# BachiLi/redner

Hardware: AMD Instinct MI355X
Metric: Msamples/s fwd+bwd (higher is better)
Workload: dtype f64; 1 GPU; bunny_box 1024x1024, max_bounces 4, Sobol, 256 spp fwd+bwd per step (vertex gradients, primary+secondary edge sampling), sharded by sample index over 1 GPU(s): 256 spp per GPU; spp=256, spp_per_gpu=256, max_bounces=4, parallelism=sample-sharded x1, world_size=1, pool_cap_mb=32768, samples_per_launch=8, sample_workers=2, schedule=library default: two sample workers, batches as large as the buffer cache holds

## Files before the change

### include/redner_amd.h

```cpp
#ifndef REDNER_AMD_H
#define REDNER_AMD_H

#include <stddef.h>
#include <stdint.h>

#ifdef __cplusplus
extern "C" {
#endif

#define RDR_MAX_MIP_LEVELS 8

enum rdr_camera_type { RDR_CAMERA_PERSPECTIVE = 0, RDR_CAMERA_ORTHOGRAPHIC = 1, RDR_CAMERA_FISHEYE = 2,
                       RDR_CAMERA_PANORAMA = 3 };
enum rdr_sampler_type { RDR_SAMPLER_INDEPENDENT = 0, RDR_SAMPLER_SOBOL = 1 };
enum rdr_channel {
    RDR_CH_RADIANCE = 0, RDR_CH_ALPHA, RDR_CH_DEPTH, RDR_CH_POSITION, RDR_CH_GEOMETRY_NORMAL,
    RDR_CH_SHADING_NORMAL, RDR_CH_UV, RDR_CH_BARYCENTRIC_COORDINATES, RDR_CH_DIFFUSE_REFLECTANCE,
    RDR_CH_SPECULAR_REFLECTANCE, RDR_CH_ROUGHNESS, RDR_CH_GENERIC_TEXTURE, RDR_CH_VERTEX_COLOR,
    RDR_CH_SHAPE_ID, RDR_CH_TRIANGLE_ID, RDR_CH_MATERIAL_ID
};

typedef struct rdr_camera_desc {
    int width, height;
    const float *position, *look, *up;
// ... 38 lines not shown
} rdr_material_desc;

typedef struct rdr_dtexture_desc {
    float *texels[RDR_MAX_MIP_LEVELS];
    int num_levels;
    float *uv_scale;
} rdr_dtexture_desc;
typedef struct rdr_dmaterial_desc {
    rdr_dtexture_desc diffuse_reflectance, specular_reflectance, roughness, generic_texture, normal_map;
} rdr_dmaterial_desc;

typedef struct rdr_area_light_desc {
    int shape_id;
    float intensity[3];
    int two_sided, directly_visible;
} rdr_area_light_desc;
typedef struct rdr_darea_light_desc { float *intensity; } rdr_darea_light_desc;

typedef struct rdr_envmap_desc {
    rdr_texture_desc values;
    const float *env_to_world, *world_to_env;
    const float *sample_cdf_ys, *sample_cdf_xs;
    float pdf_norm;
    int directly_visible;
} rdr_envmap_desc;
typedef struct rdr_denvmap_desc { rdr_dtexture_desc values; float *world_to_env; } rdr_denvmap_desc;

typedef struct rdr_tuning rdr_tuning;
typedef struct rdr_render_options {
    uint64_t seed;
    int num_samples, max_bounces;
    const int *channels; int num_channels;
    int sampler_type;
    int sample_pixel_center;
    int sample_offset, total_samples;
    const rdr_tuning *tuning;
} rdr_render_options;

enum rdr_tune_flags {
    RDR_TUNE_NO_OVERLAP       = 1 << 0,
    RDR_TUNE_FORCE_GENERAL    = 1 << 1,
    RDR_TUNE_PICKN_WALK       = 1 << 2,
    RDR_TUNE_PICKH_FUSED      = 1 << 3,
    RDR_TUNE_PICKH_LAZY       = 1 << 4,
    RDR_TUNE_NO_HOIST         = 1 << 5,
    RDR_TUNE_REFILL_OFF       = 1 << 6,
    RDR_TUNE_REFILL_ALL       = 1 << 7,
    RDR_TUNE_TRACE_BINARY     = 1 << 8,
    RDR_TUNE_TRACE_NO_LDS_TOP = 1 << 9,
    RDR_TUNE_NO_FUSED_BOUNCE  = 1 << 10,
    RDR_TUNE_PICKH_ONE_LAUNCH = 1 << 11,
    RDR_TUNE_NO_NEE_COMPACT   = 1 << 12,
    RDR_TUNE_LARGE_FORMS      = 1 << 13,
    RDR_TUNE_TRACE_EVERY_CONTINUATION = 1 << 14
};
struct rdr_tuning {
    unsigned flags;
    int batch_samples;
    int64_t batch_lanes;
    int workers;
    int refill_rays_per_lane, refill_idle_lanes, refill_steps;
    int wide_max_rays;
    int gather_budget;
    int gather_heavy_cap_plus1, gather_work_cap_plus1;
    int mem_available_mb;
    int refill_order;
    int pickh_slots_per_lane, pickh_idle_lanes, pickh_steps;
    int stale_event_cap_plus1;
};

void rdr_set_stream(void *hip_stream);
void rdr_set_pool_cap_mb(int64_t megabytes);
int64_t rdr_get_pool_cap_mb(void);
enum rdr_build_flags {
    RDR_BUILD_NO_REFIT        = 1 << 0,
    RDR_BUILD_NO_EDGE_CACHE   = 1 << 1,
    RDR_BUILD_SYNC_EDGES      = 1 << 2,
    RDR_BUILD_EDGE_HOST_BUILD = 1 << 3
};
void rdr_set_build_flags(unsigned flags);

typedef struct rdr_dscene_desc {
    rdr_dcamera_desc camera;
    const rdr_dshape_desc *shapes; int num_shapes;
    const rdr_dmaterial_desc *materials; int num_materials;
    const rdr_darea_light_desc *area_lights; int num_area_lights;
    const rdr_denvmap_desc *envmap;
} rdr_dscene_desc;

typedef struct rdr_scene rdr_scene;

rdr_scene *rdr_scene_create(const rdr_camera_desc *camera,
                            const rdr_shape_desc *shapes, int num_shapes,
                            const rdr_material_desc *materials, int num_materials,
                            const rdr_area_light_desc *area_lights, int num_area_lights,
                            const rdr_envmap_desc *envmap,
                            int use_gpu, int gpu_index,
                            int use_primary_edge_sampling, int use_secondary_edge_sampling);
void rdr_scene_destroy(rdr_scene *scene);
int rdr_scene_max_generic_texture_dimension(const rdr_scene *scene);

int rdr_render(const rdr_scene *scene, const rdr_render_options *options,
               float *rendered_image, const float *d_rendered_image,
               const rdr_dscene_desc *d_scene,
               float *screen_gradient_image, float *debug_image);

int rdr_compute_num_channels(const int *channels, int num_channels, int max_generic_texture_dimension);
// ... 109 lines not shown
```

### redner_amd/_capi.py

```python
import ctypes as C
import os

MAX_MIP = 8
_HERE = os.path.dirname(os.path.abspath(__file__))
DEFAULT_LIBRARY = os.path.join(_HERE, 'lib', 'libredner_amd.so')
EXACT_LIBRARY = os.path.join(_HERE, 'lib', 'libredner_amd_exact.so')

c_float_p = C.POINTER(C.c_float)
c_int_p = C.POINTER(C.c_int32)


class CameraDesc(C.Structure):
    _fields_ = [('width', C.c_int), ('height', C.c_int),
                ('position', C.c_void_p), ('look', C.c_void_p), ('up', C.c_void_p),
                ('cam_to_world', C.c_void_p), ('world_to_cam', C.c_void_p),
                ('intrinsic_mat_inv', C.c_void_p), ('intrinsic_mat', C.c_void_p),
                ('distortion_params', C.c_void_p),
                ('clip_near', C.c_float), ('camera_type', C.c_int),
                ('viewport_beg', C.c_int * 2), ('viewport_end', C.c_int * 2)]


class DCameraDesc(C.Structure):
    _fields_ = [(n, C.c_void_p) for n in ('position', 'look', 'up', 'cam_to_world', 'world_to_cam',
                                          'intrinsic_mat_inv', 'intrinsic_mat', 'distortion_params')]
# ... 11 lines not shown
    _fields_ = [(n, C.c_void_p) for n in ('vertices', 'uvs', 'normals', 'colors')]


class TextureDesc(C.Structure):
    _fields_ = [('texels', C.c_void_p * MAX_MIP), ('width', C.c_int * MAX_MIP), ('height', C.c_int * MAX_MIP),
                ('channels', C.c_int), ('num_levels', C.c_int), ('uv_scale', C.c_void_p)]


class MaterialDesc(C.Structure):
    _fields_ = [('diffuse_reflectance', TextureDesc), ('specular_reflectance', TextureDesc),
                ('roughness', TextureDesc), ('generic_texture', TextureDesc), ('normal_map', TextureDesc),
                ('compute_specular_lighting', C.c_int), ('two_sided', C.c_int), ('use_vertex_color', C.c_int)]


class DTextureDesc(C.Structure):
    _fields_ = [('texels', C.c_void_p * MAX_MIP), ('num_levels', C.c_int), ('uv_scale', C.c_void_p)]


class DMaterialDesc(C.Structure):
    _fields_ = [(n, DTextureDesc) for n in ('diffuse_reflectance', 'specular_reflectance', 'roughness',
                                            'generic_texture', 'normal_map')]


class AreaLightDesc(C.Structure):
    _fields_ = [('shape_id', C.c_int), ('intensity', C.c_float * 3), ('two_sided', C.c_int),
                ('directly_visible', C.c_int)]


class DAreaLightDesc(C.Structure):
    _fields_ = [('intensity', C.c_void_p)]


class EnvmapDesc(C.Structure):
    _fields_ = [('values', TextureDesc), ('env_to_world', C.c_void_p), ('world_to_env', C.c_void_p),
                ('sample_cdf_ys', C.c_void_p), ('sample_cdf_xs', C.c_void_p),
                ('pdf_norm', C.c_float), ('directly_visible', C.c_int)]


class DEnvmapDesc(C.Structure):
    _fields_ = [('values', DTextureDesc), ('world_to_env', C.c_void_p)]


class Tuning(C.Structure):
    _fields_ = [('flags', C.c_uint), ('batch_samples', C.c_int), ('batch_lanes', C.c_int64), ('workers', C.c_int),
                ('refill_rays_per_lane', C.c_int), ('refill_idle_lanes', C.c_int), ('refill_steps', C.c_int),
                ('wide_max_rays', C.c_int), ('gather_budget', C.c_int),
                ('gather_heavy_cap_plus1', C.c_int), ('gather_work_cap_plus1', C.c_int), ('mem_available_mb', C.c_int),
                ('refill_order', C.c_int), ('pickh_slots_per_lane', C.c_int), ('pickh_idle_lanes', C.c_int), ('pickh_steps', C.c_int),
                ('stale_event_cap_plus1', C.c_int)]


TUNE_NO_OVERLAP, TUNE_FORCE_GENERAL, TUNE_PICKN_WALK, TUNE_PICKH_FUSED, TUNE_PICKH_LAZY, TUNE_NO_HOIST, TUNE_REFILL_OFF, \
    TUNE_REFILL_ALL, TUNE_TRACE_BINARY, TUNE_TRACE_NO_LDS_TOP, TUNE_NO_FUSED_BOUNCE, TUNE_PICKH_ONE_LAUNCH, TUNE_NO_NEE_COMPACT, \
    TUNE_LARGE_FORMS, TUNE_TRACE_EVERY_CONTINUATION = [1 << k for k in range(15)]
BUILD_NO_REFIT, BUILD_NO_EDGE_CACHE, BUILD_SYNC_EDGES, BUILD_EDGE_HOST_BUILD = [1 << k for k in range(4)]


class RenderOptionsDesc(C.Structure):
    _fields_ = [('seed', C.c_uint64), ('num_samples', C.c_int), ('max_bounces', C.c_int),
                ('channels', C.POINTER(C.c_int)), ('num_channels', C.c_int),
                ('sampler_type', C.c_int), ('sample_pixel_center', C.c_int),
                ('sample_offset', C.c_int), ('total_samples', C.c_int),
                ('tuning', C.POINTER(Tuning))]


class DSceneDesc(C.Structure):
    _fields_ = [('camera', DCameraDesc),
                ('shapes', C.POINTER(DShapeDesc)), ('num_shapes', C.c_int),
                ('materials', C.POINTER(DMaterialDesc)), ('num_materials', C.c_int),
                ('area_lights', C.POINTER(DAreaLightDesc)), ('num_area_lights', C.c_int),
                ('envmap', C.POINTER(DEnvmapDesc))]


class TraceStats(C.Structure):
    _fields_ = [('closest_ms', C.c_double), ('any_ms', C.c_double),
                ('closest_launches', C.c_uint64), ('any_launches', C.c_uint64),
                ('closest_rays', C.c_uint64), ('any_rays', C.c_uint64),
                ('closest_nodes', C.c_uint64), ('closest_tris', C.c_uint64),
                ('any_nodes', C.c_uint64), ('any_tris', C.c_uint64),
                ('closest_wide_nodes', C.c_uint64), ('any_wide_nodes', C.c_uint64),
                ('closest_union_ms', C.c_double), ('any_union_ms', C.c_double)]


class DebugCounters(C.Structure):
    _fields_ = [('device_mallocs', C.c_uint64), ('host_count_reads', C.c_uint64),
                ('last_batch_samples', C.c_uint64), ('last_workers', C.c_uint64)]


class DeferredDesc(C.Structure):
    _fields_ = [('num_images', C.c_int), ('height', C.c_int), ('width', C.c_int),
                ('aa_samples', C.c_int), ('alpha', C.c_int), ('num_lights', C.c_int),
                ('light_type', c_int_p), ('image_light_range', c_int_p), ('gpu_index', C.c_int),
                ('occluders', C.POINTER(C.c_void_p)), ('visibility', C.c_void_p),
                ('ao_occluders', C.POINTER(C.c_void_p)), ('ao_words', C.c_void_p),
                ('ao_rays', C.c_int), ('ao_radius', C.c_float)]


DL_AMBIENT, DL_POINT, DL_DIRECTIONAL, DL_SPOT, DL_SH_R, DL_SH_G, DL_SH_B = range(7)

_p, _i, _i64 = C.c_void_p, C.c_int, C.c_int64
HEADERS = {
    'redner_amd.h': {
        'rdr_last_error': (C.c_char_p, []),
        'rdr_scene_create': (_p, [C.POINTER(CameraDesc), C.POINTER(ShapeDesc), _i, C.POINTER(MaterialDesc), _i,
                                  C.POINTER(AreaLightDesc), _i, C.POINTER(EnvmapDesc), _i, _i, _i, _i]),
        'rdr_scene_destroy': (None, [_p]),
        'rdr_scene_max_generic_texture_dimension': (_i, [_p]),
# ... 124 lines not shown
```

### redner_amd/csrc/bsdf.h

```cpp
#pragma once
#include "surface.h"

namespace rdr {

RDR_FN int imod(int a, int b) { int r = a % b; return r < 0 ? r + b : r; }

struct Bilerp { int i00, i10, i01, i11; double u, v; };
RDR_FN Bilerp bilerp_setup(const TexD &tex, int li, V2 uv) {
    Bilerp b;
    int W = tex.width[li], H = tex.height[li];
    double x = uv.x * W - 0.5f, y = uv.y * H - 0.5f;
    int xf = (int)floor(x), yf = (int)floor(y);
    b.u = x - xf; b.v = y - yf;
    int x0 = imod(xf, W), y0 = imod(yf, H), x1 = imod(xf + 1, W), y1 = imod(yf + 1, H);
    b.i00 = y0 * W + x0; b.i10 = y0 * W + x1; b.i01 = y1 * W + x0; b.i11 = y1 * W + x1;
    return b;
}
RDR_FN double bilerp_eval(const float *texels, int ch, int c, const Bilerp &b) {
    double f00 = texels[ch * b.i00 + c], f10 = texels[ch * b.i10 + c];
    double f01 = texels[ch * b.i01 + c], f11 = texels[ch * b.i11 + c];
    return f00 * (1.f - b.u) * (1.f - b.v) + f01 * (1.f - b.u) * b.v +
           f10 * b.u * (1.f - b.v) + f11 * b.u * b.v;
}

template <class F> RDR_FN void trilinear_each(const TexD &tex, V2 uv, double level, const F &f) {
    int ch = tex.channels;
    if (level <= 0 || level >= tex.num_levels - 1) {
        int li = level <= 0 ? 0 : tex.num_levels - 1;
        Bilerp b = bilerp_setup(tex, li, uv);
        for (int c = 0; c < ch; ++c) f(c, bilerp_eval(tex.texels[li], ch, c, b));
    } else {
        int li = (int)floor(level);
        double ld = level - li;
        Bilerp b0 = bilerp_setup(tex, li, uv), b1 = bilerp_setup(tex, li + 1, uv);
        for (int c = 0; c < ch; ++c) {
            double a0 = bilerp_eval(tex.texels[li], ch, c, b0);
            double a1 = bilerp_eval(tex.texels[li + 1], ch, c, b1);
            f(c, a0 * (1 - ld) + a1 * ld);
        }
    }
}
RDR_FN void trilinear(const TexD &tex, V2 uv, double level, double *out) {
    trilinear_each(tex, uv, level, [out](int c, double x) { out[c] = x; });
}

RDR_FN double tex_level(const TexD &tex, V2 du, V2 dv) {
    double fp = dmax(len(du) * tex.width[0], len(dv) * tex.height[0]);
    return log(dmax(fp, double(1e-8f))) / log(2.0);
}

template <class F> RDR_FN void tex_fetch_each(const TexD &tex, V2 uv_, V2 du_, V2 dv_, const F &f) {
    if (tex.width[0] <= 0 && tex.height[0] <= 0) {
        for (int c = 0; c < tex.channels; ++c) f(c, (double)tex.texels[0][c]);
        return;
// ... 338 lines not shown
}

RDR_FN V3 cos_hemisphere(V2 s) {
    double phi = 2.f * float(M_PI) * s.x;
    double tmp = sqrt(dmax(1.f - s.y, 0.0));
    return V3{cos(phi) * tmp, sin(phi) * tmp, sqrt(s.y)};
}

RDR_FN V3 bsdf_sample_dir(const MaterialD &m, const Surf &sp, V3 wi, V2 s_uv, double s_w, double min_rough,
                          const RayDiff &wi_rd, RayDiff &wo_rd, double &next_min_rough, bool diffs = true) {
    next_min_rough = min_rough;
    ShadeCtx c = shade_ctx(m, sp);
    double gwi = dot(c.gn, wi);
    if (!m.two_sided && gwi < 0) return v3(0);
    LobePmf p = lobe_pmf(m, sp);
    if (s_w <= p.diffuse) {
        next_min_rough = 1.0;
        V3 ld = cos_hemisphere(s_uv);
        if (diffs) {
            wo_rd.org_dx = wi_rd.org_dx; wo_rd.org_dy = wi_rd.org_dy;
            wo_rd.dir_dx = V3{0.03f, 0.03f, 0.03f};
            wo_rd.dir_dy = V3{0.03f, 0.03f, 0.03f};
        }
        V3 d = to_world(c.fr, ld);
        if (dot(c.gn, d) * gwi < 0) d = to_world(c.fr, -ld);
        return d;
    }
    double rough = dmax(dmax(tex1(m.roughness, sp), min_rough), 1e-6);
    next_min_rough = dmax(rough, min_rough);
    double e = roughness_to_phong(rough);
    double phi = 2.f * double(M_PI) * s_uv.y;
    double sphi = sin(phi), cphi = cos(phi);
    double ct = pow(s_uv.x, 1.0 / (e + 2.0));
    double st = sqrt(dmax(1.f - ct * ct, 0.0));
    V3 hl = V3{st * cphi, st * sphi, ct};
    V3 h = to_world(c.fr, hl);
    V3 d = 2.f * dot(wi, h) * h - wi;
    if (dot(c.gn, d) * gwi < 0) {
        hl = -hl;
        h = to_world(c.fr, hl);
        d = 2.f * dot(wi, h) * h - wi;
    }
    if (!diffs) return d;
    V3 dmdx = sp.dn_dx * hl.z, dmdy = sp.dn_dy * hl.z;
    V3 wi_dx = -wi_rd.dir_dx, wi_dy = -wi_rd.dir_dy;
    double wdm_dx = sum(wi_dx * h) + sum(wi * dmdx);
    double wdm_dy = sum(wi_dy * h) + sum(wi * dmdy);
    wo_rd.org_dx = wi_rd.org_dx; wo_rd.org_dy = wi_rd.org_dy;
    wo_rd.dir_dx = 2 * (dot(wi, h) * dmdx + wdm_dx * h) - wi_dx;
    wo_rd.dir_dy = 2 * (dot(wi, h) * dmdy + wdm_dy * h) - wi_dy;
    return d;
}

}
```

### redner_amd/csrc/hip/exec.h

```cpp
#pragma once
#include <hip/hip_runtime.h>
#include "../per_device.h"
#include <stdint.h>
#include <stdio.h>
#include <atomic>
#include <condition_variable>
#include <cstdlib>
#include <exception>
#include <functional>
#include <mutex>
#include <stdexcept>
#include <string>
#include <thread>

#define RDR_FN __host__ __device__ inline
#define RDR_INLINE_CALL [[clang::always_inline]]
#define RDR_DEV_FN __device__ inline
#define RDR_STACK_DECL(T, name, N) __shared__ T name##_lds[(N) * 256]; T *name = name##_lds + threadIdx.x
#define RDR_STACK_AT(name, k) name[(k) * 256]
#define RDR_WALK_STACK_MEMBER(T, name, N)
#define RDR_WALK_STACK(st, T, name, N, TAG) (rdr::lds_column<T, N, TAG>())
#define RDR_WALK_AT(stk, k) stk[(k) * 256]

namespace rdr {
// ... 231 lines not shown
                    if (low && hipDeviceGetStreamPriorityRange(&least, &greatest) == hipSuccess && least != greatest)
                        check(hipStreamCreateWithPriority(&s, hipStreamNonBlocking, least), "hipStreamCreateWithPriority");
                    else check(hipStreamCreateWithFlags(&s, hipStreamNonBlocking), "hipStreamCreate");
                }
                ctx().stream = s;
                job();
                check(hipStreamSynchronize(s), "second stream sync");
            } catch (...) { failure = std::current_exception(); }
            { std::unique_lock<std::mutex> lk(m_); failure_ = failure; state_ = 0; }
            cv_.notify_all();
        }
    }
    std::mutex m_; std::condition_variable cv_;
    std::function<void()> job_; int device_ = 0; int state_ = 0;
    std::exception_ptr failure_;
};

struct Fence {
    hipEvent_t e = nullptr;
    Fence() { check(hipEventCreateWithFlags(&e, hipEventDisableTiming), "hipEventCreate"); }
    ~Fence() { if (e) (void)hipEventDestroy(e); }
    Fence(const Fence &) = delete;
    void after(hipStream_t producer) { check(hipEventRecord(e, producer), "hipEventRecord"); }
    void gate(hipStream_t consumer) { check(hipStreamWaitEvent(consumer, e, 0), "hipStreamWaitEvent"); }
};

inline int choose_replicas(size_t replica_bytes, size_t budget) {
    int r = 256;
    while (r > 1 && replica_bytes * (size_t)r > budget) r >>= 1;
    return r;
}
inline size_t replica_budget(size_t job_samples) {
    static const size_t mb = [] { const char *e = std::getenv("RDR_REPLICA_MB"); return e ? (size_t)std::atoi(e) : (size_t)0; }();
    if (mb) return mb << 20;
    const size_t lo = (size_t)256 << 20, hi = (size_t)1 << 30, want = job_samples * 64;
    return want < lo ? lo : (want > hi ? hi : want);
}
inline void set_replicas(const rdr::ReplicaLayout &layout) {
    check(hipMemcpyToSymbolAsync(HIP_SYMBOL(rdr::g_rep), &layout, sizeof(layout), 0, hipMemcpyHostToDevice, ctx().stream), "set_replicas");
    static const int texel_rounds = [] { const char *e = std::getenv("RDR_TEXEL_ROUNDS"); return e ? std::atoi(e) : 0; }();
    if (texel_rounds > 0) check(hipMemcpyToSymbolAsync(HIP_SYMBOL(rdr::g_texel_rounds), &texel_rounds, sizeof(int), 0, hipMemcpyHostToDevice, ctx().stream), "set_replicas");
    check(hipStreamSynchronize(ctx().stream), "set_replicas sync");
}

struct Count {
    const int *dev; int upper;
    Count(int n) : dev(nullptr), upper(n) {}
    Count(const int *d, int u) : dev(d), upper(u) {}
};

template <class F, class = void> struct MinBlocks { static constexpr int value = 1; };
template <class F> struct MinBlocks<F, decltype((void)F::kMinBlocksPerCU)> { static constexpr int value = F::kMinBlocksPerCU; };

template <class F>
__global__ void __launch_bounds__(256, MinBlocks<F>::value) stage_kernel(F f, int n, const int *count) {
    int i = blockIdx.x * 256 + threadIdx.x;
    if (count) { const int c = *count; n = c < n ? c : n; }
    if (i < n) { RDR_INLINE_CALL f(i); }
}

constexpr int kRefillIdle = 16;
constexpr int kWalkSteps = 16;
template <class W, class = void> struct WalkGate { __device__ static bool closed(const W &) { return false; } };
template <class W> struct WalkGate<W, decltype((void)&W::gate_closed)> { __device__ static bool closed(const W &w) { return w.gate_closed(); } };
template <class W>
__global__ void __launch_bounds__(256) persistent_kernel(W w, int n, const int *count, int *next_item) {
    if (WalkGate<W>::closed(w)) return;
    if (count) { const int c = *count; n = c < n ? c : n; }
    typename W::State st;
    bool busy = false;
    const int lane = threadIdx.x & 63;
    for (;;) {
        const unsigned long long idle = __ballot(!busy);
        const int nidle = __popcll(idle);
        if (nidle >= kRefillIdle) {
            const int leader = __ffsll((long long)idle) - 1;
            int base = 0;
            if (lane == leader) base = atomicAdd(next_item, nidle);
            base = __shfl(base, leader);
            if (!busy) {
                const int item = base + __popcll(idle & ((1ull << lane) - 1ull));
                if (item < n) {
                    if (w.begin(item, st)) busy = true;
                    else w.finish(st);
                }
            }
            if (__ballot(busy) == 0ull && base + nidle >= n) break;
        }
#pragma unroll 1
        for (int it = 0; it < kWalkSteps; ++it) {
            if (busy && w.step(st)) { w.finish(st); busy = false; }
        }
    }
}
#ifndef RDR_CHUNKED_MIN_BLOCKS
#define RDR_CHUNKED_MIN_BLOCKS 1
#endif
template <class W>
__global__ void __launch_bounds__(256, RDR_CHUNKED_MIN_BLOCKS) chunked_kernel(W w, int n, const int *count, int items_per_lane, int idle_min, int steps, int *next_chunk) {
    if (count) { const int c = *count; n = c < n ? c : n; }
    const int chunk = 64 * items_per_lane;
    const int lane = threadIdx.x & 63;
    int next = 0, end = 0;
    bool more = true;
    typename W::State st;
    bool busy = false;
    for (;;) {
        const unsigned long long idle = __ballot(!busy);
        const int nidle = __popcll(idle);
        if (nidle >= idle_min || nidle == 64) {
// ... 221 lines not shown
```

### redner_amd/csrc/render.cpp

```cpp
#include "render.h"
#include "tuning.h"
#include <atomic>
#include <exception>
#include <cstdio>
#include <cstdlib>
#include "stages_fwd.h"
#include "stages_bwd.h"
#include "stages_edge.h"
#include "grad_store.h"
#include <algorithm>
#include <memory>
#include <stdexcept>
#include <type_traits>
#include <vector>

namespace rdr {

namespace {

inline bool overlap_on() { return !tuning().has(RDR_TUNE_NO_OVERLAP); }


VSlice make_slice(Arena &a, int n, bool with_occl, bool with_rdiff = true) {
    VSlice v;
// ... 11 lines not shown
struct Queues {
    rt::RayRec *nee, *bsdf;
    rt::HitRec *h_nee, *h_bsdf;
    int *pos[2];
};

struct BounceChain {
    bool fused = false;
    bool have_rays = false;
    const int *qpos = nullptr;
    exec::Count queue_n{0};
    int flip = 0;
};

struct ChannelLayout { int nd, radiance_dim; ChannelsD ch; };
ChannelLayout layout_of(const rdr_render_options &o, int max_generic) {
    ChannelLayout l;
    l.nd = 0; l.radiance_dim = -1;
    if (o.num_channels > kMaxChannels) throw std::runtime_error("render: too many channels");
    l.ch.n = o.num_channels; l.ch.max_generic = max_generic; l.ch.radiance_off = -1;
    l.ch.id = nullptr;
    l.ch.radiance_only = o.num_channels == 1 && o.channels[0] == RDR_CH_RADIANCE;
    int d = 0;
    for (int i = 0; i < o.num_channels; ++i) {
        if (o.channels[i] == RDR_CH_RADIANCE) {
            if (l.radiance_dim != -1) throw std::runtime_error("Duplicated radiance channel");
            l.radiance_dim = i;
            l.ch.radiance_off = d;
        }
        int one = o.channels[i];
        int w = compute_num_channels(&one, 1, max_generic);
        if (w < 0) throw std::runtime_error("render: unknown channel id");
        d += w;
    }
    l.nd = d;
    l.ch.nd = d; l.ch.radiance_dim = l.radiance_dim;
    return l;
}

void debug_dump(const char *tag, int sample, int depth, const void *dev_ptr, size_t bytes) {
    static const char *dir = std::getenv("RDR_DEBUG_DUMP");
    if (!dir || !dev_ptr) return;
    std::vector<char> host(bytes);
    exec::download(host.data(), dev_ptr, bytes);
    char path[1024];
    std::snprintf(path, sizeof(path), "%s/%s_s%d_d%d.bin", dir, tag, sample, depth);
    if (FILE *f = std::fopen(path, "wb")) { std::fwrite(host.data(), 1, bytes, f); std::fclose(f); }
}

uint64_t pcg_stream_seed(const rdr_render_options &o) {
    return (uint64_t)o.seed + (uint64_t)o.sample_offset * 0x9E3779B97F4A7C15ULL;
}

bool scene_is_lean(const Scene &scene, const ChannelsD &ch) {
    const CameraD &c = scene.d.cam;
    return scene.d.envmap == nullptr && c.kind == kCamPerspective && !c.distortion.defined && ch.radiance_only &&
           !scene.has_mipmaps && !scene.has_textures && !scene.has_vertex_colors;
}

constexpr int kGeneral = 0, kLean = 1, kMid = 2;
int scene_kind(const Scene &scene, const ChannelsD &ch) {
    if (tuning().has(RDR_TUNE_FORCE_GENERAL)) return kGeneral;
    if (scene_is_lean(scene, ch)) return kLean;
    const CameraD &c = scene.d.cam;
    if (scene.d.envmap == nullptr && c.kind == kCamPerspective && !c.distortion.defined && ch.radiance_only) return kMid;
    return kGeneral;
}
template <class F, class Go> void with_kind(int kind, const F &f, Go &&go) {
    if (kind == kLean) go(LeanStage<F>{f});
    else if (kind == kMid) go(MidStage<F>{f});
    else go(f);
}
template <class W, class Go> void with_walk_kind(int kind, const W &w, Go &&go) {
    if (kind == kLean) go(LeanWalk<W>{w});
    else if (kind == kMid) go(MidWalk<W>{w});
    else go(w);
}
template <class F> void launch_v(int kind, exec::Count n, const F &f) {
    with_kind(kind, f, [&](const auto &k) { exec::launch(n, k); });
}

inline int side_index(int k, int lanes) { return lanes >= (1 << 19) ? k + 2 : k; }
struct Fork {
    exec::Fence from, done;
    bool marked = false, pending = false;
    void mark() { from.after(exec::ctx().stream); marked = true; }
    void join() { if (pending) done.gate(exec::ctx().stream); pending = false; }
    template <class Work> void run(hipStream_t side, Work &&work) {
        if (!marked) mark();
        marked = false;
        from.gate(side);
        exec::StreamScope on(side);
        work();
        done.after(side);
        pending = true;
    }
};
template <class Work> void beside(Fork &fork, bool aside, int k, int lanes, Work &&work) {
    if (aside) fork.run(exec::side_stream(side_index(k, lanes)), work);
    else work();
}

inline bool fuse_bounces(bool pcg, int kind, int chain_lanes) {
    return !pcg && kind == kLean && chain_lanes <= (1 << 19) && !tuning().has(RDR_TUNE_NO_FUSED_BOUNCE);
}
constexpr int kEmitterTestMax = 8;
struct Bounce {
    SamplerD rng{}; int dim = 0, rng_shift = 0;
    const int *active = nullptr; exec::Count num_active{0};
    int *next_active = nullptr;
    const VSlice *v = nullptr, *vn = nullptr, *vnn = nullptr;
    const Queues *q = nullptr;
    Sink sink{};
    int *dyn = nullptr; int dyn_inc = 0;
    bool shadow_rays_coherent = false, last_bounce = false, next_is_last = false;
    BounceChain *chain = nullptr;
    Fork *shadow_fork = nullptr;
};
exec::Count run_bounce(const Scene &scene, const SceneD &sd, const Bounce &b) {
    const VSlice &v = *b.v, &vn = *b.vn;
    const Queues &q = *b.q;
    BounceChain *chain = b.chain;
    const int lean = scene_kind(scene, b.sink.ch);
    const bool fused = chain && chain->fused;
    const bool drawn = fused && chain->have_rays;
    const exec::Count queue_n = drawn ? chain->queue_n : b.num_active;
    const int *qpos = drawn ? chain->qpos : nullptr;
    const bool emitter_test = lean == kLean && scene.emitter_triangles > 0 && scene.emitter_triangles <= kEmitterTestMax &&
                              !tuning().has(RDR_TUNE_TRACE_EVERY_CONTINUATION);
    if (!drawn) {
        BounceSample bs{sd, b.rng, b.dim, b.rng_shift, b.active, v, vn, q.nee, q.bsdf};
        bs.last_bounce_emitters = b.last_bounce && emitter_test;
        launch_v(lean, b.num_active, bs);
    }
    beside(*b.shadow_fork, overlap_on(), 1, b.num_active.upper, [&] {
        exec::trace(scene.bvh, q.nee, q.h_nee, queue_n, true, b.shadow_rays_coherent);
    });
    exec::trace(scene.bvh, q.bsdf, q.h_bsdf, queue_n, false);
    b.shadow_fork->join();
    const BounceContrib contrib{sd, b.rng, b.dim, b.rng_shift, b.active, v, vn, q.h_nee, q.h_bsdf, b.sink};
    if (!fused) {
        launch_v(lean, b.num_active, contrib);
        return exec::compact_dev(b.active, b.num_active, b.next_active, KeepHit{vn.shape}, nullptr, b.dyn, b.dyn_inc);
    }
    if (b.vnn) {
        BounceSample next{sd, b.rng, b.dim + 7, b.rng_shift, b.active, vn, *b.vnn, q.nee, q.bsdf};
        next.last_bounce_emitters = b.next_is_last && emitter_test;
        launch_v(lean, b.num_active, BounceContribSample{contrib, next, qpos});
    } else if (qpos) {
        launch_v(lean, b.num_active, BounceContribSample{contrib, BounceSample{sd, b.rng, b.dim + 7, b.rng_shift, b.active, vn, vn, nullptr, nullptr}, qpos, 1});
    } else {
        launch_v(lean, b.num_active, contrib);
    }
    int *pos_out = q.pos[chain->flip];
    chain->flip ^= 1;
    const exec::Count next = exec::compact_dev(b.active, b.num_active, b.next_active, KeepHit{vn.shape}, nullptr, b.dyn, b.dyn_inc, pos_out);
    chain->have_rays = b.vnn != nullptr;
    chain->qpos = pos_out;
    chain->queue_n = b.num_active;
    return next;
}

struct BatchView { int S = 1, P0 = 0, rows = 0; bool on = false; };

struct Worker {
    Arena arena;
    std::vector<VSlice> vs;
    int *active = nullptr;
    Queues q;
    std::vector<exec::Count> num_active;
    int *main_dyn = nullptr;
    int *seg = nullptr;
    float *stage = nullptr;
    Fork shadow_fork;
};

struct Backward {
    const Scene &scene; const rdr_render_options &opt;
    Worker &w;
    int stride, B;
    const float *d_image; float *screen_grad; double weight; int nd, radiance_dim;
// ... 10 lines not shown
    int *edge_dyn = nullptr;
    int *hoist_dyn = nullptr;
    double *multipliers = nullptr;

    VSlice ea, eb;
    int chain_n = 0;
    double *erd_chain = nullptr;
    int *deferred = nullptr, *deferred_seg = nullptr, *deferred_count = nullptr, *prim_dyn = nullptr;
    int *elist[3] = {nullptr, nullptr, nullptr};
    HEntry *h_leaves = nullptr, *h_spill = nullptr;
    int *nee_act = nullptr;
    HDescent *h_descent = nullptr;
    GatherShared gshared{nullptr, nullptr, nullptr, nullptr, 0, 0};
    GatherCand *gather_cands = nullptr;
    int *nee_slots = nullptr;
    double *edge_contrib = nullptr, *edge_tmin = nullptr, *hit_pos = nullptr;
    unsigned char *hp_written = nullptr; int *hp_violations = nullptr;
    HitEvent *hp_events = nullptr; int *hp_event_count = nullptr; int hp_event_cap = 0;
    double *hp_carry = nullptr;
    unsigned char *replay_live = nullptr;
    PrimaryEdgeRec *prim_recs = nullptr;
    SecondaryEdgeRec *sec_recs = nullptr;
    SecPick *sec_picks = nullptr;
    unsigned char *sec_mode = nullptr;
    Sink esink{}, psink{};

    Fork walk_fork;
    Fork pickh_fork;
    Fork adjoint_fork;
    const bool overlap = overlap_on();
    const bool has_lights = sd.num_lights > 0;
    const int dim0 = opt.sample_pixel_center ? 0 : 2;
    bool edges_on() const { return prim_recs != nullptr; }
    bool secondary_on() const { return edges_on() && scene.use_secondary_edges; }

    int sample_id = 0;
    int lanes = 0;
    int cur_S = 1;
    SamplerD rng{}, rng_edge{};
    int edim = 0;
    bool hoisted = false;
    SecEdgeArgs early_sa{};

    Backward(const Scene &scene_, const rdr_render_options &opt_, GradStore &grads_, Worker &w_, int P, int B_,
             const float *d_image_, float *screen_grad_, double weight_, int nd_, int radiance_dim_, const ChannelsD &ch_,
             const BatchView &batch_)
        : scene(scene_), opt(opt_), w(w_), stride(P), B(B_), d_image(d_image_), screen_grad(screen_grad_), weight(weight_),
          nd(nd_), radiance_dim(radiance_dim_), batch(batch_), sd(scene_.d), grads(grads_), ch(ch_) {
        if (batch.on) sd.cam.batch_rows = batch.rows;
        lean = scene_kind(scene, ch);
        adj.n = P; adj.plain = 0;
        adj.thr = arena.get<double>((size_t)3 * P);
        adj.ray_dir = arena.get<double>((size_t)3 * P);
        adj_point_doubles = lean == kLean ? kAdjPointDoublesLean : kAdjPointDoubles;
        adj.point = arena.get<double>((size_t)adj_point_doubles * P);
        adj.carries = scene.d.envmap == nullptr ? arena.get<unsigned char>((size_t)P) : nullptr;
        nee_act = arena.get<int>((size_t)P);
        const bool use_edges = scene.edges && scene.edges->d.num_edges > 0 &&
                              (scene.use_primary_edges || scene.use_secondary_edges);
        if (use_edges) {
            edge_dyn = arena.get<int>(kMaxBatch);
            hoist_dyn = arena.get<int>(kMaxBatch);
            const int L = 2 * P;
            ea = make_slice(arena, L, false, lean != kLean);
            eb = make_slice(arena, L, false, lean != kLean);
            if (scene.has_mipmaps) {
                ea.erd = eb.erd = arena.get<double>((size_t)12 * L);
                exec::zero(ea.erd, sizeof(double) * 12 * L);
                if (batch.on) {
                    chain_n = 2 * batch.P0;
                    ea.erd_touched = eb.erd_touched = arena.get<unsigned char>(L);
                    erd_chain = arena.get<double>((size_t)12 * chain_n);
                    exec::zero(erd_chain, sizeof(double) * 12 * chain_n);
                    deferred = arena.get<int>(L);
                    deferred_seg = arena.get<int>(kMaxBatch + 1);
                    deferred_count = arena.get<int>(kMaxBatch);
                    prim_dyn = arena.get<int>(kMaxBatch);
                }
            }
            for (int k = 0; k < 3; ++k) elist[k] = arena.get<int>(L);
            nee_slots = arena.get<int>(P);
            gather_cands = arena.get<GatherCand>((size_t)kGatherCands * P);
            gshared.book = arena.get<GatherBook>(1);
            gshared.heavy_cap = (int)std::min<long long>(std::max<long long>((long long)P / 256, kGatherHeavyCap), kGatherHeavyMax);
            gshared.work_cap = (int)std::min<long long>(std::max<long long>((long long)P / 32, kGatherWorkCap), kGatherWorkMax);
            gshared.heavy_slot = arena.get<int>(gshared.heavy_cap);
            gshared.work = arena.get<GatherWork>(gshared.work_cap);
            gshared.cands_big = arena.get<GatherCand>((size_t)kGatherCandsBig * gshared.heavy_cap);
            if (tuning().gather_heavy_cap >= 0) gshared.heavy_cap = std::min(tuning().gather_heavy_cap, gshared.heavy_cap);
            if (tuning().gather_work_cap >= 0) gshared.work_cap = std::min(tuning().gather_work_cap, gshared.work_cap);
            h_leaves = arena.get<HEntry>((size_t)kHSamples * P);
            h_spill = arena.get<HEntry>((size_t)(kHSamples - kHStackLds) * P);
            h_descent = arena.get<HDescent>((size_t)P);
            edge_contrib = arena.get<double>(L);
            edge_tmin = arena.get<double>(L);
            hit_pos = arena.get<double>((size_t)3 * L);
            exec::zero(hit_pos, sizeof(double) * 3 * L);
            if (batch.on && scene.d.envmap != nullptr) {
                hp_written = arena.get<unsigned char>(L);
                hp_violations = arena.get<int>(1);
                exec::zero(hp_violations, sizeof(int));
                hp_event_cap = L;
                hp_events = arena.get<HitEvent>((size_t)hp_event_cap);
                if (tuning().stale_event_cap >= 0) hp_event_cap = std::min(tuning().stale_event_cap, hp_event_cap);
                hp_event_count = arena.get<int>(1);
                exec::zero(hp_event_count, sizeof(int));
                hp_carry = arena.get<double>((size_t)3 * 2 * batch.P0);
                exec::zero(hp_carry, sizeof(double) * 3 * 2 * batch.P0);
                replay_live = arena.get<unsigned char>(P);
            }
            prim_recs = arena.get<PrimaryEdgeRec>(P);
            sec_recs = arena.get<SecondaryEdgeRec>(P);
            sec_picks = arena.get<SecPick>(P);
            sec_mode = arena.get<unsigned char>(P);
            if (!ch.radiance_only) multipliers = arena.get<double>((size_t)L * nd);
            if (opt.sampler_type == RDR_SAMPLER_INDEPENDENT) {
                pcg_edge = arena.get<uint64_t>(P);
                exec::launch(P, PcgInit{pcg_edge, pcg_stream_seed(opt) + 131071U});
// ... 300 lines not shown
        for (int d = B - 1; d >= 0; --d) {
            if (w.num_active[d].upper <= 0) continue;
            const AdjBounceArgs ba{sd, grads.g, rng, dim0 + 7 * d, active_of(d), w.vs[d], w.vs[d + 1], d_image, nd, radiance_dim, 0.0, adj};
            launch_v(lean, w.num_active[d], AdjBounceScatterLive{AdjBounceScatter{ba}, replay_live});
            exec::launch(n_events, InjectHitEvents{sd, grads.g, hp_events, d, hit_pos, ea.n, hp_written, hp_carry, 2 * batch.P0, adj, replay_live});
        }
        launch_v(lean, lanes, AdjPrimaryLive{AdjPrimary{sd, grads.g, rng, opt.sample_pixel_center, w.vs[0], d_image, nd, radiance_dim, 0.0,
                                                        adj, screen_grad, ch}, replay_live});
        exec::launch(2 * batch.P0, HitPosCarryAdvance{hp_carry, 2 * batch.P0, cur_S, hit_pos, ea.n, hp_written});
        exec::zero(hp_event_count, sizeof(int));
    }

    void run_sample(int sample_id_, const SamplerD &main_rng, int n_lanes, int S_now) {
        begin_sample(sample_id_, main_rng, n_lanes, S_now);
        hoist_first_vertex_picks();
        for (int d = B - 1; d >= 0 && has_lights; --d) sweep_depth(d);
        camera_vertex_adjoint();
        if (edges_on() && scene.use_primary_edges) primary_edge_pass();
        adjoint_fork.join();
        if (hp_events) replay_stale_hits();
    }
};

struct RestartUnbatched {};
std::atomic<uint64_t> g_unbatchable{0};
uint64_t scene_shape_key(const Scene &scene) {
    uint64_t h = 1469598103934665603ULL;
    auto mix = [&](uint64_t v) { h = (h ^ v) * 1099511628211ULL; };
    mix(scene.shapes.size());
    for (const ShapeD &sh : scene.shapes) { mix((uint64_t)sh.num_vertices); mix((uint64_t)sh.num_triangles); }
    mix(scene.materials.size()); mix(scene.lights.size());
    mix((uint64_t)scene.h_envmap.values.width[0]); mix((uint64_t)scene.h_envmap.values.height[0]);
    return h | 1;
}
BatchView choose_batch(const rdr_render_options &opt, const Tuning &tune, int P, int rows, int lean, int nd,
                       bool samples_independent, bool forward_batches, bool gradient) {
    const int B = opt.max_bounces;
    BatchView batch;
    batch.P0 = P; batch.rows = rows;
    if (!samples_independent && !forward_batches) return batch;
    const int batch_cap = std::min(kMaxBatch, tune.batch_samples);
    const long long total = (long long)opt.num_samples * P;
    int want = opt.num_samples;
    if (total > (1 << 17) && samples_independent) want = (opt.num_samples + 1) / 2;
    long long lane_cap = tune.batch_lanes;
    if (lane_cap == 0) {
        lane_cap = 1LL << 24;
        if (total > (1LL << 22) && exec::memory_held_by_others() > 0.10) lane_cap = 1LL << 22;
    }
    batch.S = std::max(1, std::min(std::min(batch_cap, want), (int)std::max(1LL, lane_cap / P)));
    auto bytes_needed = [&](int S_try) {
        const double lanes = (double)S_try * P;
        const int wk = !samples_independent ? 1 : (tune.workers > 0 ? tune.workers : 2);
        double per_lane = (lean == kLean ? 260.0 * (B + 1) + 660.0 : 400.0 * (B + 1) + 1200.0) * wk;
        if (forward_batches) per_lane += 4.0 * nd * (B + 1);
        if (gradient) per_lane += 4.0 * nd;
        return per_lane * lanes;
    };
    if (tune.batch_lanes == 0 && tune.mem_available_mb < 0) {
        const double cap = (double)exec::pool_cap_bytes();
        while (batch.S > 1 && bytes_needed(batch.S) > cap) --batch.S;
    }
    if (tune.mem_available_mb >= 0 || bytes_needed(batch.S) > 1073741824.0) {
        const double room = 0.8 * (tune.mem_available_mb >= 0 ? tune.mem_available_mb * 1048576.0 : (double)exec::memory_available());
        while (batch.S > 1 && bytes_needed(batch.S) > room) batch.S = (batch.S + 1) / 2;
    }
    batch.on = batch.S > 1;
    return batch;
}

const int *upload_assign_flags(Arena &arena, const rdr_render_options &opt, int max_generic, int nd) {
    std::vector<int> flags((size_t)nd, 0);
    int at = 0;
    bool any_id = false;
    for (int k = 0; k < opt.num_channels; ++k) {
        int one = opt.channels[k];
        const int w = compute_num_channels(&one, 1, max_generic);
        if (one >= RDR_CH_SHAPE_ID) { for (int j = 0; j < w; ++j) flags[at + j] = 1; any_id = true; }
        at += w;
    }
    if (!any_id) return nullptr;
    int *d_flags = arena.get<int>(flags.size());
    exec::upload(d_flags, flags.data(), sizeof(int) * flags.size());
    return d_flags;
}

void render_once(const Scene &scene, const rdr_render_options &opt, float *image, const float *d_image,
                 const rdr_dscene_desc *d_scene, float *screen_gradient_image, const Tuning &tune, bool envmap_batches) {
    if (opt.sampler_type != RDR_SAMPLER_SOBOL && opt.sampler_type != RDR_SAMPLER_INDEPENDENT)
        throw std::runtime_error("render: unknown sampler type");
    if (d_image && !d_scene) throw std::runtime_error("render: d_rendered_image given without d_scene");
    const CameraD &cam = scene.d.cam;
    const int P = (cam.vp_x1 - cam.vp_x0) * (cam.vp_y1 - cam.vp_y0);
    if (P <= 0) return;
    const int B = opt.max_bounces;
    if (B < 0) throw std::runtime_error("render: max_bounces must be >= 0");
    ChannelLayout lay = layout_of(opt, scene.max_generic_texture_dimension);
    if (lay.radiance_dim < 0 && B > 0)
        throw std::runtime_error("render: max_bounces > 0 needs the radiance channel (the reference writes path "
                                 "contributions at the radiance offset, src/path_contribution.cpp:127-129)");
    const int total_spp = opt.total_samples > 0 ? opt.total_samples : opt.num_samples;
    const double weight = 1.0 / total_spp;
    const bool has_lights = scene.d.num_lights > 0;
    if (2 + 7 * B > kSamplerDims) throw std::runtime_error("render: max_bounces exceeds the Sobol' table");

    PhaseTimer timer(d_image ? "render (backward)" : "render (forward)");
    Arena arena;
    {
        int *ids = arena.get<int>(kMaxChannels);
        exec::upload(ids, opt.channels, sizeof(int) * opt.num_channels);
        lay.ch.id = ids;
    }
    std::unique_ptr<GradStore> grads;
    if (d_image) grads.reset(new GradStore(scene, *d_scene, (size_t)P * (size_t)opt.num_samples));

    uint64_t *pcg_main = nullptr;
    if (opt.sampler_type == RDR_SAMPLER_INDEPENDENT) {
        pcg_main = arena.get<uint64_t>(P);
        exec::launch(P, PcgInit{pcg_main, pcg_stream_seed(opt)});
    }
    const int lean = scene_kind(scene, lay.ch);

    const bool sobol_plain = screen_gradient_image == nullptr && opt.sampler_type == RDR_SAMPLER_SOBOL && !timer.on;
    const bool no_edge_passes = !scene.use_primary_edges && !scene.use_secondary_edges;
    const bool chain = (scene.has_mipmaps || scene.d.envmap != nullptr) && !no_edge_passes;
    const bool batchable = sobol_plain && (lean == kLean || no_edge_passes || scene.d.envmap == nullptr || envmap_batches);
    const bool samples_independent = batchable && d_image != nullptr && image == nullptr;
    const bool forward_batches = sobol_plain && d_image == nullptr && image != nullptr;
    const BatchView batch = choose_batch(opt, tune, P, cam.vp_y1 - cam.vp_y0, lean, lay.nd, samples_independent, forward_batches, d_image != nullptr);
    const int S = batch.S;
    const int PL = S * P;
    static const bool tell = std::getenv("RDR_DEBUG_BATCH") != nullptr;
    if (tell) std::fprintf(stderr, "[render] %s: %d samples of %d lanes in batches of %d\n", d_image ? "backward" : "forward", opt.num_samples, P, S);
    const int num_batches = (opt.num_samples + S - 1) / S;
    const float *d_image_lanes = d_image;
    if (batch.on && d_image) {
        float *rep = arena.get<float>((size_t)PL * lay.nd);
        for (int k = 0; k < S; ++k)
            exec::copy_dev(rep + (size_t)k * P * lay.nd, d_image, sizeof(float) * (size_t)P * lay.nd);
        d_image_lanes = rep;
    }
    const int *assign_flags = batch.on && forward_batches && !lay.ch.radiance_only ? upload_assign_flags(arena, opt, scene.max_generic_texture_dimension, lay.nd) : nullptr;
    int workers = 1;
    if (samples_independent) workers = std::max(1, std::min(tune.workers > 0 ? tune.workers : exec::sample_workers(PL, num_batches, batch.on), num_batches));
    if (chain) workers = 1;
    if (d_image != nullptr) { last_schedule()[0].store(S); last_schedule()[1].store(workers); }

    struct SampleWorker : Worker { std::unique_ptr<Backward> bwd; };
    auto make_worker = [&](SampleWorker &w) {
        w.vs.resize(B + 1);
        for (int d = 0; d <= B; ++d) w.vs[d] = make_slice(w.arena, PL, d < B && d_image_lanes != nullptr, lean != kLean);
        w.active = w.arena.get<int>((size_t)(B + 1) * PL);
        w.q.nee = w.arena.get<rt::RayRec>((size_t)2 * PL); w.q.bsdf = w.arena.get<rt::RayRec>((size_t)2 * PL);
        w.q.h_nee = w.arena.get<rt::HitRec>((size_t)2 * PL); w.q.h_bsdf = w.arena.get<rt::HitRec>((size_t)2 * PL);
        w.q.pos[0] = w.arena.get<int>((size_t)2 * PL); w.q.pos[1] = w.arena.get<int>((size_t)2 * PL);
        w.num_active.assign(B + 2, exec::Count(0));
        if (pcg_main) w.main_dyn = w.arena.get<int>(1);
        if (batch.on) w.seg = w.arena.get<int>((size_t)(B + 1) * (kMaxBatch + 1));
        if (batch.on && forward_batches) w.stage = w.arena.get<float>((size_t)(B + 1) * PL * lay.nd);
    };
    auto run_samples = [&](SampleWorker &w, int first, int stride) {
        std::vector<VSlice> &vs = w.vs;
        int *active = w.active;
        const Queues &q = w.q;
        std::vector<exec::Count> &num_active = w.num_active;
        SceneD sd = scene.d;
        if (batch.on) sd.cam.batch_rows = batch.rows;
        for (int b = first; b < num_batches; b += stride) {
            const int s = b * S;
            const int S_now = std::min(S, opt.num_samples - s);
            const int lanes = S_now * P;
            const int sample_id = opt.sample_offset + s;
            SamplerD rng{scene.sobol_table, opt.seed, sample_id, pcg_main, 0};
            if (batch.on) { rng.batch = S_now; rng.batch_lanes = P; }
            Sink sink{image, nullptr, lay.nd, lay.radiance_dim, weight, lay.ch, nullptr};
            const size_t plane = (size_t)PL * lay.nd;
            auto sink_of = [&](int launch) { Sink k = sink; if (w.stage) k.image = w.stage + (size_t)launch * plane; return k; };
            if (w.stage) exec::zero(w.stage, sizeof(float) * plane * (B + 1));
            auto segments = [&](int d) {
                if (batch.on) exec::launch(S_now + 1, SegOffsets{active + (size_t)d * PL, num_active[d].dev, num_active[d].upper, P, S_now,
                                                                 w.seg + (size_t)d * (kMaxBatch + 1)});
            };

            launch_v(lean, lanes, GenPrimary{sd, rng, opt.sample_pixel_center, vs[0], q.bsdf});
            exec::trace(scene.bvh, q.bsdf, q.h_bsdf, lanes, false, true);
            launch_v(lean, lanes, ShadePrimary{sd, nullptr, vs[0], q.h_bsdf, sink_of(0)});
            std::fill(num_active.begin(), num_active.end(), exec::Count(0));
            num_active[0] = exec::compact_dev((const int *)nullptr, lanes, active, KeepHit{vs[0].shape});
            if (d_image) segments(0);
            if (w.main_dyn) exec::zero(w.main_dyn, sizeof(int));

            int dim = opt.sample_pixel_center ? 0 : 2;
            const int dim_first = dim;
            BounceChain chain;
            chain.fused = fuse_bounces(pcg_main != nullptr, lean, 2 * lanes);
            for (int d = 0; d < B && num_active[d].upper > 0 && has_lights; ++d) {
                Bounce bounce;
                bounce.rng = rng; bounce.dim = dim;
                bounce.active = active + (size_t)d * PL; bounce.num_active = num_active[d]; bounce.next_active = active + (size_t)(d + 1) * PL;
                bounce.v = &vs[d]; bounce.vn = &vs[d + 1]; bounce.vnn = d + 1 < B ? &vs[d + 2] : nullptr;
                bounce.q = &q; bounce.sink = sink_of(d + 1);
                bounce.dyn = w.main_dyn; bounce.dyn_inc = 7;
                bounce.shadow_rays_coherent = d == 0;
                bounce.last_bounce = d == B - 1; bounce.next_is_last = d + 2 == B;
// ... 263 lines not shown
```

### redner_amd/csrc/stages_bwd.h

```cpp
#pragma once
#include "stages_fwd.h"

namespace rdr {

constexpr int kAdjPointDoubles = 24;
constexpr int kAdjPointDoublesLean = 6;

struct AdjState {
    double *thr;
    double *ray_dir;
    double *point;
    int n;
    int plain;
    unsigned char *carries;
};

RDR_FN Surf load_adj_point(const AdjState &a, int p) {
    Surf s = surf_zero();
    s.position = ld3(a.point, a.n, p, 0);
    if (a.plain) { s.frame.n = ld3(a.point, a.n, p, 3); return s; }
    s.frame.x = ld3(a.point, a.n, p, 3); s.frame.y = ld3(a.point, a.n, p, 6); s.frame.n = ld3(a.point, a.n, p, 9);
    s.dpdu = ld3(a.point, a.n, p, 12);
    s.uv = v2(a.point[(size_t)15 * a.n + p], a.point[(size_t)16 * a.n + p]);
    s.du_dxy = v2(a.point[(size_t)17 * a.n + p], a.point[(size_t)18 * a.n + p]);
    s.dv_dxy = v2(a.point[(size_t)19 * a.n + p], a.point[(size_t)20 * a.n + p]);
    s.color = ld3(a.point, a.n, p, 21);
    return s;
}
RDR_FN void store_adj_point(const AdjState &a, int p, const Surf &s, bool with_position = true) {
    if (with_position) st3(a.point, a.n, p, 0, s.position);
    if (a.plain) { st3(a.point, a.n, p, 3, s.frame.n); return; }
    st3(a.point, a.n, p, 3, s.frame.x); st3(a.point, a.n, p, 6, s.frame.y); st3(a.point, a.n, p, 9, s.frame.n);
    st3(a.point, a.n, p, 12, s.dpdu);
    a.point[(size_t)15 * a.n + p] = s.uv.x; a.point[(size_t)16 * a.n + p] = s.uv.y;
    a.point[(size_t)17 * a.n + p] = s.du_dxy.x; a.point[(size_t)18 * a.n + p] = s.du_dxy.y;
    a.point[(size_t)19 * a.n + p] = s.dv_dxy.x; a.point[(size_t)20 * a.n + p] = s.dv_dxy.y;
    st3(a.point, a.n, p, 21, s.color);
}

RDR_FN V3 image_grad(const float *d_image, int nd, int radiance_dim, int pixel) {
    if (radiance_dim < 0) return v3(0);
    const float *g = d_image + (size_t)nd * pixel + radiance_dim;
    return V3{(double)g[0], (double)g[1], (double)g[2]};
}

struct AdjBounceArgs {
    SceneD sc; GScene g; SamplerD rng; int dim;
    const int *active; VSlice v, vn;
    const float *d_image; int nd, radiance_dim; double weight;
    AdjState adj;
};

struct AdjBounceScatter {
    AdjBounceArgs a;
    static constexpr int kMidBlocksPerCU = 2;
    static constexpr int kMinBlocksPerCU = 2;
#ifndef RDR_ADJ_SCATTER_LEAN_BLOCKS
#define RDR_ADJ_SCATTER_LEAN_BLOCKS 3
#endif
    static constexpr int kLeanBlocksPerCU = RDR_ADJ_SCATTER_LEAN_BLOCKS;
#ifndef RDR_PARK_ADJ_SCATTER
#define RDR_PARK_ADJ_SCATTER 0
#endif
    static constexpr int kParkDoubles = kSurfParkDoubles + 4;
    static_assert(kParkDoubles <= kMaxParkDoubles, "kMaxParkDoubles must cover every stage");
    RDR_FN void make_lean() { lean_scene(a.sc); lean_slice(a.v); lean_slice(a.vn); a.nd = 3; a.radiance_dim = 0; a.adj.plain = 1; }
    RDR_FN void make_mid() { mid_scene(a.sc); a.nd = 3; a.radiance_dim = 0; }
    RDR_FN void operator()(int idx) const {
        const SceneD &sc = a.sc; const GScene &g = a.g; const VSlice &v = a.v, &vn = a.vn; const AdjState &adj = a.adj;
        int p = a.active[idx];
        VertexCtx c = load_vertex(sc, v, p);
        const GMaterial &gm = g.materials[c.shape->material_id];
        V3 thr = ld3(v.thr, v.n, p, 0);
        V3 pc_bar = a.weight * image_grad(a.d_image, a.nd, a.radiance_dim, p);
        V3 thr_bar = v3(0), in_dir_bar = v3(0);
        Surf sp_bar = surf_zero();
        V3 pos = c.sp.position;
        int bshape = vn.shape[p];
        TriGrad tg = trigrad_zero();
        int tg_shape = -1, tg_tri = -1;
        V3 dir_bar = v3(0);
        bool through_hit = false;
        double d2 = 0;
        V3 wo = v3(0);
        if (bshape >= 0) {
            const ShapeD &bsh = sc.shapes[bshape];
            int btri = vn.tri[p];
            RayDiff wo_rd = load_rdiff(vn, p);
            RayDiff tmp;
            Surf bp = surf_at(bsh, btri, load_ray(vn, p), wo_rd, tmp, !sc.no_diffs);
            V3 next_thr_bar = ld3(adj.thr, adj.n, p, 0);
            V3 next_dir_bar = ld3(adj.ray_dir, adj.n, p, 0);
            V3 dir = bp.position - pos;
            d2 = len_sq(dir);
            wo = dir / sqrt(d2);
            double pdf_b = bsdf_pdf(*c.mat, c.sp, c.wi, wo, c.mrough);
            if (pdf_b > 0) {
                V3 f = bsdf_eval(*c.mat, c.sp, c.wi, wo, c.mrough);
                V3 sb = f / pdf_b;
                thr_bar += next_thr_bar * sb;
                V3 sb_bar = next_thr_bar * thr;
                V3 f_bar = sb_bar / pdf_b;
                if (bsh.light_id >= 0) {
                    const LightD &l = sc.lights[bsh.light_id];
                    if (l.two_sided || dot(-wo, bp.frame.n) > 0) {
                        double geo = fabs(dot(wo, bp.geom_normal)) / d2;
                        V3 Le = v3f(l.intensity);
                        double pdf_nee = (sc.light_pmf[bsh.light_id] * (1 / sc.light_areas[bsh.light_id])) / geo;
                        double mis = 1 / (1 + sq(pdf_nee / pdf_b));
                        V3 sc_contrib = (mis / pdf_b) * f * Le;
                        V3 scb = pc_bar * thr;
                        thr_bar += pc_bar * sc_contrib;
                        double w = mis / pdf_b;
                        f_bar += w * scb * Le;
                        if (g.light_intensity) accum3(g.light_intensity + 3 * bsh.light_id, w * scb * f);
                    }
                }
                V3 wi_bar = v3(0);
                V3 wo_bar = next_dir_bar;
                adj_bsdf_eval(*c.mat, c.sp, c.wi, wo, c.mrough, f_bar, gm, sp_bar, wi_bar, wo_bar);
                dir_bar = wo_bar / sqrt(d2);
                double sd_bar = -sum(wo_bar * dir) / d2;
                double d2_bar = 0.5f * sd_bar / sqrt(d2);
                dir_bar += adj_len_sq(dir, d2_bar);
                in_dir_bar -= wi_bar;
                through_hit = true;
            }
        } else if (sc.envmap != nullptr) {
            V3 wo_e = load_ray(vn, p).dir;
            double pdf_b = bsdf_pdf(*c.mat, c.sp, c.wi, wo_e, c.mrough);
            if (len_sq(wo_e) > 0 && pdf_b > 0) {
                V3 f = bsdf_eval(*c.mat, c.sp, c.wi, wo_e, c.mrough);
                V3 Le = envmap_eval(*sc.envmap, wo_e, raydiff_zero());
                double pdf_nee = envmap_pdf(*sc.envmap, wo_e) * sc.light_pmf[sc.num_lights - 1];
                double mis = 1 / (1 + sq(pdf_nee / pdf_b));
                V3 sc_contrib = (mis / pdf_b) * f * Le;
                V3 scb = pc_bar * thr;
                thr_bar += pc_bar * sc_contrib;
                double w = mis / pdf_b;
                V3 f_bar = w * scb * Le, Le_bar = w * scb * f;
                V3 wo_bar = v3(0), wi_bar = v3(0);
                RayDiff rd_bar = raydiff_zero();
                adj_envmap_eval(*sc.envmap, wo_e, raydiff_zero(), Le_bar, g.envmap, wo_bar, rd_bar);
                adj_bsdf_eval(*c.mat, c.sp, c.wi, wo_e, c.mrough, f_bar, gm, sp_bar, wi_bar, wo_bar);
                in_dir_bar -= wi_bar;
            }
        }
        st3(adj.thr, adj.n, p, 0, thr_bar);
        st3(adj.ray_dir, adj.n, p, 0, in_dir_bar);
        V3 pos_bar = sp_bar.position;
        Surf next_pt_bar = surf_zero();
        if (through_hit) next_pt_bar = load_adj_point(adj, p);
        store_adj_point(adj, p, sp_bar, false);
        if (through_hit) {
            const ShapeD &bsh = sc.shapes[bshape];
            const int btri = vn.tri[p];
            Surf bp_bar = next_pt_bar;
            bp_bar.position += dir_bar;
            DRay r_bar = dray_zero();
            RayDiff rd_bar = raydiff_zero();
            Ray br = make_ray(pos, wo);
#if RDR_PARK_ADJ_SCATTER
            RDR_PARK_DECL(park, kParkDoubles);
            park.put3(kSurfParkDoubles, dir_bar); park.put(kSurfParkDoubles + 3, c.mrough);
            adj_surf_at(bsh, btri, br, load_rdiff(vn, p), bp_bar, raydiff_zero(), r_bar, rd_bar, tg, !sc.no_diffs, sc.plain_materials != 0, park);
            dir_bar = park.get3<V3>(kSurfParkDoubles); c.mrough = park.get(kSurfParkDoubles + 3);
#else
            adj_surf_at(bsh, btri, br, load_rdiff(vn, p), bp_bar, raydiff_zero(), r_bar, rd_bar, tg, !sc.no_diffs, sc.plain_materials != 0);
#endif
            tg_shape = bshape; tg_tri = btri;
            if (c.mrough > 0.01f) {
                pos_bar -= dir_bar;
                pos_bar += r_bar.org;
            }
        }
        st3(adj.point, adj.n, p, 0, pos_bar);
        if (adj.carries) adj.carries[p] = 1;
        scatter_trigrad_wave(sc.shapes, g.shapes, tg_shape, tg_tri, tg, sc.plain_materials != 0);
    }
};

RDR_FN void adj_record_add(const AdjState &adj, int p, V3 thr_bar, V3 in_dir_bar, const Surf &sp_bar) {
    st3(adj.thr, adj.n, p, 0, ld3(adj.thr, adj.n, p, 0) + thr_bar);
    st3(adj.ray_dir, adj.n, p, 0, ld3(adj.ray_dir, adj.n, p, 0) + in_dir_bar);
    Surf cur = load_adj_point(adj, p);
    cur.position += sp_bar.position;
    cur.frame.n += sp_bar.frame.n;
    if (!adj.plain) {
        cur.frame.x += sp_bar.frame.x; cur.frame.y += sp_bar.frame.y;
        cur.dpdu += sp_bar.dpdu; cur.uv += sp_bar.uv; cur.du_dxy += sp_bar.du_dxy; cur.dv_dxy += sp_bar.dv_dxy;
        cur.color += sp_bar.color;
    }
    store_adj_point(adj, p, cur);
    if (adj.carries) adj.carries[p] = 1;
}

struct AdjBounceNee {
    static constexpr int kMinBlocksPerCU = 2;
    static constexpr int kMidBlocksPerCU = 2;
#ifdef RDR_ADJ_NEE_LEAN_BLOCKS
    static constexpr int kLeanBlocksPerCU = RDR_ADJ_NEE_LEAN_BLOCKS;
#endif
#ifndef RDR_PARK_ADJ_NEE
#define RDR_PARK_ADJ_NEE 1
#endif
    static constexpr int kParkDoubles = 22;
    static_assert(kParkDoubles <= kMaxParkDoubles, "kMaxParkDoubles must cover every stage");
    AdjBounceArgs a;
    RDR_FN void make_lean() { lean_scene(a.sc); lean_slice(a.v); lean_slice(a.vn); a.nd = 3; a.radiance_dim = 0; a.adj.plain = 1; }
    RDR_FN void make_mid() { mid_scene(a.sc); a.nd = 3; a.radiance_dim = 0; }
    RDR_FN void envmap_nee(int p, const LightDraw &ld) const {
        const SceneD &sc = a.sc; const GScene &g = a.g; const VSlice &v = a.v;
        V3 wo = envmap_sample(*sc.envmap, ld.uv);
        double pdf_nee = envmap_pdf(*sc.envmap, wo) * sc.light_pmf[sc.num_lights - 1];
        if (!(pdf_nee > 0)) return;
        VertexCtx c = load_vertex(sc, v, p);
        const GMaterial &gm = g.materials[c.shape->material_id];
        V3 thr = ld3(v.thr, v.n, p, 0);
        V3 pc_bar = a.weight * image_grad(a.d_image, a.nd, a.radiance_dim, p);
        V3 f = bsdf_eval(*c.mat, c.sp, c.wi, wo, c.mrough);
        V3 Le = envmap_eval(*sc.envmap, wo, raydiff_zero());
        double pdf_b = bsdf_pdf(*c.mat, c.sp, c.wi, wo, c.mrough);
        double mis = 1 / (1 + sq(pdf_b / pdf_nee));
        V3 nee = (mis / pdf_nee) * f * Le;
        V3 nee_bar = pc_bar * thr;
        V3 thr_bar = pc_bar * nee;
        double w = mis / pdf_nee;
        V3 f_bar = w * nee_bar * Le, Le_bar = w * nee_bar * f;
        V3 wo_bar = v3(0), wi_bar = v3(0);
        RayDiff rd_bar = raydiff_zero();
        adj_envmap_eval(*sc.envmap, wo, raydiff_zero(), Le_bar, g.envmap, wo_bar, rd_bar);
        Surf sp_bar = surf_zero();
        adj_bsdf_eval(*c.mat, c.sp, c.wi, wo, c.mrough, f_bar, gm, sp_bar, wi_bar, wo_bar);
        adj_record_add(a.adj, p, thr_bar, -wi_bar, sp_bar);
    }
    RDR_FN void operator()(int idx) const {
        V3 lv_bar[3] = {v3(0), v3(0), v3(0)};
        int l_shape = -1, l_tri = -1;
        RDR_INLINE_CALL light_vertex(idx, lv_bar, l_shape, l_tri);
        scatter_positions_wave(a.sc.shapes, a.g.shapes, l_shape, l_tri, lv_bar);
    }
    RDR_FN void light_vertex(int idx, V3 (&lv_bar)[3], int &l_shape, int &l_tri) const {
        const SceneD &sc = a.sc; const GScene &g = a.g; const VSlice &v = a.v; const AdjState &adj = a.adj;
        int p = a.active[idx];
        if (v.occl[p]) return;
        LightDraw ld = draw_light(a.rng, p, a.dim);
        LightPick pk = pick_light(sc, ld.light_sel, ld.tri_sel);
        if (pk.shape_id < 0) {
            if (sc.envmap != nullptr) envmap_nee(p, ld);
            return;
        }
        const ShapeD &lsh = sc.shapes[pk.shape_id];
        if (lsh.light_id < 0) return;
        VertexCtx c = load_vertex(sc, v, p);
        V3 pos = c.sp.position;
        Surf lp = sample_tri(lsh, pk.tri_id, ld.uv);
        V3 dir = lp.position - pos;
        double d2 = len_sq(dir);
        V3 wo = dir / sqrt(d2);
        const LightD &l = sc.lights[lsh.light_id];
        if (nee_is_geometrically_zero(sc, c, pk, lp)) return;
        const GMaterial &gm = g.materials[c.shape->material_id];
        V3 thr = ld3(v.thr, v.n, p, 0);
        V3 pc_bar = a.weight * image_grad(a.d_image, a.nd, a.radiance_dim, p);
        V3 thr_bar = v3(0), in_dir_bar = v3(0);
        Surf sp_bar = surf_zero();
        V3 f = bsdf_eval(*c.mat, c.sp, c.wi, wo, c.mrough);
        double cl = dot(wo, lp.geom_normal);
        double geo = fabs(cl) / d2;
        V3 Le = v3f(l.intensity);
        double pdf_nee = sc.light_pmf[lsh.light_id] * (1 / sc.light_areas[lsh.light_id]);
        double pdf_b = bsdf_pdf(*c.mat, c.sp, c.wi, wo, c.mrough) * geo;
        double mis = 1 / (1 + sq(pdf_b / pdf_nee));
        V3 nee = (mis * geo / pdf_nee) * f * Le;
        V3 nee_bar = pc_bar * thr;
        thr_bar += pc_bar * nee;
        double w = mis / pdf_nee;
        double w_bar = geo * sum(nee_bar * f * Le);
        double pdfnee_bar = -w_bar * w / pdf_nee;
        double geo_bar = w * sum(nee_bar * f * Le);
        V3 f_bar = w * nee_bar * geo * Le;
        V3 Le_bar = w * nee_bar * geo * f;
        double area_bar = -pdfnee_bar * pdf_nee / tri_area(lsh, pk.tri_id);
        adj_tri_area(lsh, pk.tri_id, area_bar, lv_bar);
        if (g.light_intensity) accum3(g.light_intensity + 3 * lsh.light_id, Le_bar);
        double cl_bar = cl > 0 ? geo_bar / d2 : -geo_bar / d2;
        double d2_bar = -geo_bar * geo / d2;
        V3 wo_bar = cl_bar * lp.geom_normal;
        Surf lp_bar = surf_zero();
        lp_bar.geom_normal = cl_bar * wo;
        V3 wi_bar = v3(0);
#if RDR_PARK_ADJ_NEE
        RDR_PARK_DECL(park, kParkDoubles);
        park.put3(0, lv_bar[0]); park.put3(3, lv_bar[1]); park.put3(6, lv_bar[2]);
        park.put3(9, thr_bar); park.put3(12, dir); park.put(15, d2); park.put(16, d2_bar);
        park.put3(17, lp_bar.geom_normal); park.put2(20, ld.uv);
#endif
        adj_bsdf_eval(*c.mat, c.sp, c.wi, wo, c.mrough, f_bar, gm, sp_bar, wi_bar, wo_bar);
#if RDR_PARK_ADJ_NEE
        lv_bar[0] = park.get3<V3>(0); lv_bar[1] = park.get3<V3>(3); lv_bar[2] = park.get3<V3>(6);
        thr_bar = park.get3<V3>(9); dir = park.get3<V3>(12); d2 = park.get(15); d2_bar = park.get(16);
        lp_bar.geom_normal = park.get3<V3>(17); ld.uv = park.get2<V2>(20);
#endif
        V3 dir_bar = wo_bar / sqrt(d2);
        double sd_bar = -sum(wo_bar * dir) / d2;
        d2_bar += (0.5f * sd_bar / sqrt(d2));
        dir_bar += adj_len_sq(dir, d2_bar);
        lp_bar.position += dir_bar;
        sp_bar.position -= dir_bar;
        in_dir_bar -= wi_bar;
        adj_sample_tri(lsh, pk.tri_id, ld.uv, lp_bar, lv_bar);
        l_shape = pk.shape_id; l_tri = pk.tri_id;
        adj_record_add(adj, p, thr_bar, in_dir_bar, sp_bar);
    }
};

struct ImageBar {
    const float *gi; double weight;
    RDR_FN double operator()(int c) const { return weight * (double)gi[c]; }
    RDR_FN const double *triple(double *o) const { o[0] = (*this)(0); o[1] = (*this)(1); o[2] = (*this)(2); return o; }
};
RDR_FN void adj_first_hit_channels(const SceneD &sc, const GScene &g, const ChannelsD &ch, const float *d_image,
                                   double weight, int p, int shape, const Surf &sp, const Ray &ray,
                                   Surf &pt_bar, V3 &org_bar) {
    const ShapeD &sh = sc.shapes[shape];
    const MaterialD &m = sc.materials[sh.material_id];
    const GMaterial &gm = g.materials[sh.material_id];
    const float *gi = d_image + (size_t)ch.nd * p;
    int d = 0;
    for (int k = 0; k < ch.n; ++k) {
        int id = ch.id[k];
        int width = channel_width(id, ch.max_generic);
        switch (id) {
            case 2: {
                double dist_bar = (double)gi[d] * weight;
                V3 diff_bar = adj_len(sp.position - ray.org, dist_bar);
                org_bar -= diff_bar; pt_bar.position += diff_bar;
            } break;
            case 3: pt_bar.position += weight * V3{(double)gi[d], (double)gi[d + 1], (double)gi[d + 2]}; break;
            case 4: pt_bar.geom_normal += weight * V3{(double)gi[d], (double)gi[d + 1], (double)gi[d + 2]}; break;
            case 5: pt_bar.frame.n += weight * V3{(double)gi[d], (double)gi[d + 1], (double)gi[d + 2]}; break;
            case 6: pt_bar.uv += weight * V2{(double)gi[d], (double)gi[d + 1]}; break;
            case 7: pt_bar.bary += weight * V2{(double)gi[d], (double)gi[d + 1]}; break;
            case 8: {
                V3 r_bar = weight * V3{(double)gi[d], (double)gi[d + 1], (double)gi[d + 2]};
                if (m.use_vertex_color) pt_bar.color += r_bar; else adj_tex3(m.diffuse, sp, r_bar, gm.diffuse, pt_bar);
            } break;
            case 9: adj_tex3(m.specular, sp, weight * V3{(double)gi[d], (double)gi[d + 1], (double)gi[d + 2]}, gm.specular, pt_bar); break;
            case 10: adj_tex1(m.roughness, sp, weight * (double)gi[d], gm.roughness, pt_bar); break;
            case 11: {
                if (m.generic.num_levels > 0)
// ... 57 lines not shown
            RayDiff mrd_bar = raydiff_zero();
            adj_envmap_eval(*sc.envmap, ray.dir, rd, e_bar, g.envmap, mr_bar.dir, mrd_bar);
            V2 ms = v2(0.5, 0.5);
            if (!sample_center) { const SamplerD::Lane ln = rng.lane(p); ms = v2(rng.draw(ln, 0), rng.draw(ln, 1)); }
            V2 mscr_bar = v2(0, 0);
            RDR_INLINE_CALL adj_primary_ray(sc.cam, pixel_to_screen(sc.cam, p, ms), mr_bar, g.cam, screen_grad != nullptr, mscr_bar);
            if (screen_grad) { screen_grad[2 * p] += (float)mscr_bar.x; screen_grad[2 * p + 1] += (float)mscr_bar.y; }
            return;
        }
        DRay r_bar = dray_zero();
        r_bar.dir = ld3(adj.ray_dir, adj.n, p, 0);
        RayDiff prd_bar = raydiff_zero();
        {
            Surf pt_bar = load_adj_point(adj, p);
            if (!ch.radiance_only) {
                RayDiff tmp;
                Surf sp = surf_at(sc.shapes[shape], v0.tri[p], ray, rd, tmp, !sc.no_diffs);
                adj_first_hit_channels(sc, g, ch, d_image, weight, p, shape, sp, ray, pt_bar, r_bar.org);
            }
            adj_surf_at(sc.shapes[shape], v0.tri[p], ray, rd, pt_bar, raydiff_zero(), r_bar, prd_bar, tg, !sc.no_diffs, sc.plain_materials != 0, park);
#pragma unroll
            for (int k = 0; k < 3; ++k) { park.put3(3 * k, tg.p[k]); park.put3(9 + 3 * k, tg.n[k]); }
            tg_shape = shape; tg_tri = v0.tri[p];
        }
        V2 s = v2(0.5, 0.5);
        if (!sample_center) { const SamplerD::Lane ln = rng.lane(p); s = v2(rng.draw(ln, 0), rng.draw(ln, 1)); }
        V2 screen = pixel_to_screen(sc.cam, p, s);
        double delta = 1e-3;
        double sx = 0.5 / sc.cam.width, sy = 0.5 / sc.cam.height;
        V2 scr_bar = v2(0, 0);
        const bool sb = screen_grad != nullptr;
        if (!sc.no_diffs) {
            DRay rx_bar{prd_bar.org_dx * sx / delta, prd_bar.dir_dx * sx / delta};
            DRay ry_bar{prd_bar.org_dy * sy / delta, prd_bar.dir_dy * sy / delta};
            r_bar.org += (prd_bar.org_dx * -sx + prd_bar.org_dy * -sy) / delta;
            r_bar.dir += (prd_bar.dir_dx * -sx + prd_bar.dir_dy * -sy) / delta;
            RDR_INLINE_CALL adj_primary_ray(sc.cam, screen + v2(delta, 0), rx_bar, g.cam, sb, scr_bar);
            RDR_INLINE_CALL adj_primary_ray(sc.cam, screen + v2(0, delta), ry_bar, g.cam, sb, scr_bar);
        }
        RDR_INLINE_CALL adj_primary_ray(sc.cam, screen, r_bar, g.cam, sb, scr_bar);
        if (screen_grad) {
            screen_grad[2 * p] += (float)scr_bar.x;
            screen_grad[2 * p + 1] += (float)scr_bar.y;
        }
    }
};

struct AdjBounceScatterLive {
    static constexpr int kMidBlocksPerCU = AdjBounceScatter::kMidBlocksPerCU, kMinBlocksPerCU = AdjBounceScatter::kMinBlocksPerCU,
                         kLeanBlocksPerCU = AdjBounceScatter::kLeanBlocksPerCU;
    AdjBounceScatter f; const unsigned char *live;
    RDR_FN void make_lean() { f.make_lean(); }
    RDR_FN void make_mid() { f.make_mid(); }
    RDR_FN void operator()(int idx) const { if (!live[f.a.active[idx]]) return; RDR_INLINE_CALL f(idx); }
};
struct AdjPrimaryLive {
    static constexpr int kMidBlocksPerCU = AdjPrimary::kMidBlocksPerCU, kMinBlocksPerCU = AdjPrimary::kMinBlocksPerCU;
    AdjPrimary f; const unsigned char *live;
    RDR_FN void make_lean() { f.make_lean(); }
    RDR_FN void make_mid() { f.make_mid(); }
    RDR_FN void operator()(int p) const { if (!live[p]) return; RDR_INLINE_CALL f(p); }
};

struct KeepNeeLive {
    const unsigned char *occl;
    RDR_FN bool operator()(int p) const { return occl[p] == 0; }
};

struct KeepLitContinuation {
    const int *next_shape; const ShapeD *shapes; bool envmap;
    RDR_FN bool operator()(int p) const { const int s = next_shape[p]; return s >= 0 ? shapes[s].light_id >= 0 : envmap; }
};
struct KeepCarryingContinuation {
    const unsigned char *carries; const int *next_shape; const ShapeD *shapes;
    RDR_FN bool operator()(int p) const { return carries[p] != 0 || shapes[next_shape[p]].light_id >= 0; }
};

struct FlushSegment { size_t begin, count; float *out; };
struct FlushGrad {
    const double *block; size_t stride; int replicas;
    const FlushSegment *segments; int num_segments;
    RDR_FN void operator()(int i) const {
        int lo = 0, hi = num_segments;
        while (hi - lo > 1) {
            int mid = (lo + hi) >> 1;
            if (segments[mid].begin <= (size_t)i) lo = mid; else hi = mid;
        }
        const FlushSegment sg = segments[lo];
        if ((size_t)i < sg.begin || (size_t)i >= sg.begin + sg.count) return;
        double s = 0;
        for (int r = 0; r < replicas; ++r) s += block[(size_t)r * stride + i];
        sg.out[(size_t)i - sg.begin] += (float)s;
    }
};

}
```

### redner_amd/csrc/stages_edge.h

```cpp
#pragma once
#include "edges.h"
#include "stages_bwd.h"

namespace rdr {

RDR_FN M3 m3_from_frame(const Frame &f) {
    M3 r;
    r.m[0][0] = f.x.x; r.m[0][1] = f.x.y; r.m[0][2] = f.x.z;
    r.m[1][0] = f.y.x; r.m[1][1] = f.y.y; r.m[1][2] = f.y.z;
    r.m[2][0] = f.n.x; r.m[2][1] = f.n.y; r.m[2][2] = f.n.z;
    return r;
}
RDR_FN M3 m3_inverse(const M3 &a) {
    const double (*m)[3] = a.m;
    double det = m[0][0] * (m[1][1] * m[2][2] - m[2][1] * m[1][2]) - m[0][1] * (m[1][0] * m[2][2] - m[1][2] * m[2][0]) +
                 m[0][2] * (m[1][0] * m[2][1] - m[1][1] * m[2][0]);
    double id = 1 / det;
    M3 r;
    r.m[0][0] = (m[1][1] * m[2][2] - m[2][1] * m[1][2]) * id;
    r.m[0][1] = (m[0][2] * m[2][1] - m[0][1] * m[2][2]) * id;
    r.m[0][2] = (m[0][1] * m[1][2] - m[0][2] * m[1][1]) * id;
    r.m[1][0] = (m[1][2] * m[2][0] - m[1][0] * m[2][2]) * id;
    r.m[1][1] = (m[0][0] * m[2][2] - m[0][2] * m[2][0]) * id;
    r.m[1][2] = (m[1][0] * m[0][2] - m[0][0] * m[1][2]) * id;
// ... 529 lines not shown
RDR_FN int finish_edge_nee(const SceneD &sc, const EdgeSceneD &es, const Ray &nee, bool nee_valid, const Surf &nee_pt, int nee_shape,
                           int selected, double edge_w, double wsum, double &weight, V3 &edge_pt, V3 &mwt) {
    double pmf = edge_w / wsum;
    const EdgeD &e = es.edges[selected];
    V3 a = edge_v0(sc.shapes, e), b = edge_v1(sc.shapes, e);
    V3 pn = nee.dir;
    double t = -(dot(nee.org, pn) - dot(a, pn)) / dot(nee.dir, pn);
    if (t < nee.tmin || t > nee.tmax) return -1;
    V3 ip = nee.org + nee.dir * t;
    double jac = 0, pdf_nee = 0;
    if (nee_valid) {
        V3 ln = nee_pt.geom_normal, lpos = nee_pt.position;
        double tau = dot(lpos - nee.org, ln) / dot(ip - nee.org, ln);
        V3 omega = ip - nee.org;
        jac = len(tau * ((b - a) - omega * (dot(b - a, ln) / dot(omega, ln))));
        const ShapeD &lsh = sc.shapes[nee_shape];
        pdf_nee = sc.light_pmf[lsh.light_id] / sc.light_areas[lsh.light_id];
    } else {
        jac = 1 / len_sq(ip - nee.org);
        pdf_nee = envmap_pdf(*sc.envmap, nee.dir);
    }
    if (pmf <= 0 || jac <= 0 || pdf_nee <= 0) return -1;
    weight = 1 / (2 * es.edge_bounds_expand * pmf * jac * pdf_nee);
    V3 ap = a - ip;
    V3 ab = normalize(b - a);
    edge_pt = ip + ap - (dot(ap, ab)) * ab - nee.org;
    mwt = b - a;
    return selected;
}


RDR_FN M3 ltc_matrix(const float *tab, const Surf &sp, V3 wi, double roughness) {
    double ct = dot(wi, sp.frame.n);
    double theta = acos(ct);
    int rid = iclamp(int(roughness * (128 - 1)), 0, 128 - 1);
    int tid = iclamp(int((theta / (M_PI / 2.f)) * (128 - 1)), 0, 128 - 1);
    const float *p = tab + 9 * (rid + tid * 128);
    M3 r;
    for (int i = 0; i < 3; ++i) for (int j = 0; j < 3; ++j) r.m[i][j] = p[3 * i + j];
    return r;
}

struct SecPick { int eid; double ew; V3 sample_p, mwt; };

struct SecPre {
    bool live;
    VertexCtx c;
    LtcCtx lc;
    double pd, ps, m_pmf, roughness, nee_pmf, edge_sel, resample_sel, bsdf_comp, t_sel;
    bool dg, use_nee, nee_valid;
    Ray nee; Surf nee_pt; int nee_shape;
};

RDR_FN SecPre sec_prepare(const SceneD &sc, const EdgeSceneD &es, const SamplerD &rng_main, int dim_main,
                          const SamplerD &rng_edge, int dim_edge, const VSlice &v, int p, int idx) {
    SecPre s;
    s.live = false;
    s.c = load_vertex(sc, v, p);
    if (s.c.mrough > 1e-2f) return s;
    LightDraw ld = draw_light(rng_main, p, dim_main);
    LightPick pk = pick_light(sc, ld.light_sel, ld.tri_sel);
    s.nee_valid = pk.shape_id >= 0;
    s.nee_shape = pk.shape_id;
    s.nee_pt = surf_zero();
    s.nee = make_ray(s.c.sp.position, v3(0));
    if (s.nee_valid) {
        s.nee_pt = sample_tri(sc.shapes[pk.shape_id], pk.tri_id, ld.uv);
        s.nee = shadow_ray_to(s.c.sp.position, s.nee_pt.position);
        s.nee.tmax = len(s.nee_pt.position - s.nee.org);
    } else if (sc.envmap != nullptr) {
        s.nee = make_ray(s.c.sp.position, envmap_sample(*sc.envmap, ld.uv));
    }
    const SamplerD::Lane eln = rng_edge.lane(idx);
    s.edge_sel = rng_edge.draw(eln, dim_edge); s.resample_sel = rng_edge.draw(eln, dim_edge + 1);
    s.bsdf_comp = rng_edge.draw(eln, dim_edge + 2); s.t_sel = rng_edge.draw(eln, dim_edge + 3);
    const MaterialD &mat = *s.c.mat;
    V3 kd = tex3(mat.diffuse, s.c.sp), ks = tex3(mat.specular, s.c.sp);
    double wd = luminance(kd), ws = luminance(ks), wsum = wd + ws;
    if (wsum <= 0.f) return s;
    s.pd = wd / wsum; s.ps = ws / wsum;
    V3 n = s.c.sp.frame.n;
    V3 wi = s.c.wi;
    if (mat.two_sided && dot(wi, n) < 0.f) n = -n;
    V3 fx = normalize(wi - n * dot(wi, n));
    V3 fy = cross(n, fx);
    if (dot(wi, n) > 1 - 1e-6f) onb(n, fx, fy);
    Frame iso{fx, fy, n};
    s.lc.pos = s.c.sp.position;
    s.roughness = dmax(tex1(mat.roughness, s.c.sp), s.c.mrough);
    if (s.bsdf_comp <= s.pd) {
        s.lc.m_inv = m3_from_frame(iso);
        s.lc.m = m3_inverse(s.lc.m_inv);
        s.m_pmf = s.pd;
    } else {
        s.lc.m_inv = m3_mul(m3_inverse(ltc_matrix(es.ltc, s.c.sp, wi, s.roughness)), m3_from_frame(iso));
        s.lc.m = m3_inverse(s.lc.m_inv);
        s.m_pmf = s.ps;
    }
    s.use_nee = false;
    s.nee_pmf = 1;
    s.dg = s.bsdf_comp <= s.pd || s.roughness > 0.1;
    if (s.dg) {
        s.use_nee = s.edge_sel < 0.5;
        if (s.roughness > 0.1) s.nee_pmf = 0.5f;
        else s.nee_pmf = s.use_nee ? s.pd * 0.5f : 1.f - s.pd * 0.5f;
    }
    if (!s.use_nee && s.dg) s.edge_sel = (s.edge_sel - 0.5) * 2;
    s.live = true;
    return s;
}

struct SecEdgeArgs {
    SceneD sc; EdgeSceneD es;
    SamplerD rng_main; int dim_main;
    SamplerD rng_edge; int dim_edge;
    const int *active; VSlice v;
};
RDR_FN SecPick nee_pick_tail(const SecEdgeArgs &a, int idx, int selected, double edge_w, double wsum) {
    SecPick out{-1, 0.0, v3(0), v3(0)};
    if (selected != -1) {
        SecPre s = sec_prepare(a.sc, a.es, a.rng_main, a.dim_main, a.rng_edge, a.dim_edge, a.v, a.active[idx], idx);
        double ew = 0;
        V3 sample_p = v3(0), mwt = v3(0);
        int eid = finish_edge_nee(a.sc, a.es, s.nee, s.nee_valid, s.nee_pt, s.nee_shape, selected, edge_w, wsum, ew, sample_p, mwt);
        out = SecPick{eid, ew, sample_p, mwt};
    }
    return out;
}

constexpr int kDenseShapeTriangles = 512;
struct HDescent { double pos[3], m_inv[9], sample, resample; int nleaf, pad; };
RDR_FN LtcCtx ltc_of(const HDescent &d) {
    LtcCtx c;
    c.pos = V3{d.pos[0], d.pos[1], d.pos[2]};
    for (int r = 0; r < 3; ++r) for (int k = 0; k < 3; ++k) { c.m_inv.m[r][k] = d.m_inv[3 * r + k]; c.m.m[r][k] = 0; }
    return c;
}
struct SecEdgeSetup {
    SecEdgeArgs a; unsigned char *mode; SecondaryEdgeRec *recs; SecPick *picks; VSlice ev; double *edge_tmin;
    HDescent *hd = nullptr;
    RDR_FN void make_lean() { lean_scene(a.sc); lean_slice(a.v); lean_slice(ev); }
    RDR_FN void make_mid() { mid_scene(a.sc); }
    RDR_FN void operator()(int idx) const {
        int p = a.active[idx];
        int l0 = 2 * idx, l1 = 2 * idx + 1;
        SecPre s = sec_prepare(a.sc, a.es, a.rng_main, a.dim_main, a.rng_edge, a.dim_edge, a.v, p, idx);
        SecondaryEdgeRec rec;
        rec.edge = EdgeD{-1, 0, 0, 0, 0};
        rec.edge_pt = rec.mwt = v3(0); rec.sp_pos = s.c.sp.position;
        rec.use_nee_ray = 0; rec.diffuse_or_glossy = 0;
        recs[idx] = rec;
        picks[idx] = SecPick{-1, 0.0, v3(0), v3(0)};
        for (int l = l0; l <= l1; ++l) {
            st3(ev.thr, ev.n, l, 0, v3(0));
            store_ray(ev, l, v3(0), v3(0));
            ev.shape[l] = -1; ev.tri[l] = -1;
            ev.mrough[l] = s.c.mrough;
            edge_tmin[l] = 1e-3f;
            store_rdiff(ev, l, raydiff_zero());
        }
        const bool dense = s.live && s.c.shape->num_triangles >= kDenseShapeTriangles;
        mode[idx] = !s.live ? 0 : (s.use_nee ? (dense ? 3 : 2) : 1);
        if (hd && s.live && !s.use_nee) {
            HDescent d;
            d.pos[0] = s.lc.pos.x; d.pos[1] = s.lc.pos.y; d.pos[2] = s.lc.pos.z;
            for (int r = 0; r < 3; ++r) for (int k = 0; k < 3; ++k) d.m_inv[3 * r + k] = s.lc.m_inv.m[r][k];
            d.sample = s.edge_sel; d.resample = s.resample_sel; d.nleaf = 0; d.pad = 0;
            hd[idx] = d;
        }
    }
};
struct KeepMode {
    const unsigned char *mode; unsigned char want;
    RDR_FN bool operator()(int idx) const { return mode[idx] == want; }
};

struct SecEdgePickH {
    SecEdgeArgs a; const int *slots; SecPick *picks;
    RDR_FN void make_lean() { lean_scene(a.sc); lean_slice(a.v); }
    RDR_FN void make_mid() { mid_scene(a.sc); }
    RDR_FN void operator()(int i) const {
        int idx = slots[i];
        SecPre s = sec_prepare(a.sc, a.es, a.rng_main, a.dim_main, a.rng_edge, a.dim_edge, a.v, a.active[idx], idx);
        double ew = 0;
        int eid = pick_edge_hierarchical(a.sc, a.es, s.lc, s.edge_sel, s.resample_sel, ew);
        picks[idx] = SecPick{eid, ew, v3(0), v3(0)};
    }
};
template <bool PRELOAD> struct SecEdgePickH2 {
    SecEdgeArgs a; const int *slots; SecPick *picks; HEntry *leaves, *spill; int n;
    RDR_FN void make_lean() { lean_scene(a.sc); lean_slice(a.v); }
    RDR_FN void make_mid() { mid_scene(a.sc); }
    RDR_FN void operator()(int i) const {
        int idx = slots[i];
        SecPre s = sec_prepare(a.sc, a.es, a.rng_main, a.dim_main, a.rng_edge, a.dim_edge, a.v, a.active[idx], idx);
        double ew = 0;
        int eid = pick_edge_hierarchical_deferred<PRELOAD>(a.sc, a.es, s.lc, s.edge_sel, s.resample_sel, ew, leaves + i, spill + i, (size_t)n);
        picks[idx] = SecPick{eid, ew, v3(0), v3(0)};
    }
// ... 292 lines not shown
            for (int k = 0; k < sp && !lost; ++k) {
                const int w = atomic_fetch_add(&sh.book->work_count, 1);
                if (w < sh.work_cap) sh.work[w] = GatherWork{heavy, RDR_STACK_AT(stk, k)};
                else lost = true;
            }
            if (lost && heavy < sh.heavy_cap) atomic_fetch_add(&sh.book->cand_count[heavy], kGatherPoison);
            if (lost) sh.book->walk_needed = 1;
        }
        exec::gather_stats_add(h_nodes, h_edges % 1000000, ncand, (int)(h_edges / 1000000));
        if (heavy >= 0) { picks[idx] = SecPick{kPickOverflow, 0.0, v3(0), v3(0)}; return; }
        picks[idx] = gather_replay(a, idx, mine, ncand, c.resample);
    }
};
template <int NS> struct SecEdgeGatherSub {
    SecEdgeArgs a; const int *slots; GatherShared sh;
    RDR_FN void make_lean() { lean_scene(a.sc); lean_slice(a.v); }
    RDR_FN void make_mid() { mid_scene(a.sc); }
    RDR_FN void operator()(int j) const {
        const int n_work = sh.book->work_count < sh.work_cap ? sh.book->work_count : sh.work_cap;
        if (j >= n_work) return;
        const GatherWork wk = sh.work[j];
        const int idx = slots[sh.heavy_slot[wk.heavy]];
        const GatherCtx c = gather_ctx(a, idx);
        RDR_STACK_DECL(int, stk, NS);
        RDR_STACK_DECL(int, lst, kGatherLeafBatch);
        int sp = 0, nl = 0;
        RDR_STACK_AT(stk, sp) = wk.entry; sp++;
        auto emit = [&](const GatherCand &cd) { gather_append_big(sh, wk.heavy, cd); };
        long pops = 0, h_edges = 0;
        gather_walk<NS>(a.sc, a.es, c, stk, sp, lst, nl, (long)1 << 60, emit, pops, h_edges);
    }
};
struct SecEdgeGatherReplay {
    SecEdgeArgs a; const int *slots; SecPick *picks; GatherShared sh;
    RDR_FN void make_lean() { lean_scene(a.sc); lean_slice(a.v); }
    RDR_FN void make_mid() { mid_scene(a.sc); }
    RDR_FN void operator()(int h) const {
        const int n_heavy = sh.book->heavy_count < sh.heavy_cap ? sh.book->heavy_count : sh.heavy_cap;
        if (h >= n_heavy) return;
        const int n = sh.book->cand_count[h];
        if (n < 0 || n > kGatherCandsBig) { sh.book->walk_needed = 1; return; }
        const int idx = slots[sh.heavy_slot[h]];
        SecPre s = sec_prepare(a.sc, a.es, a.rng_main, a.dim_main, a.rng_edge, a.dim_edge, a.v, a.active[idx], idx);
        picks[idx] = gather_replay(a, idx, sh.cands_big + (size_t)h * kGatherCandsBig, n, s.resample_sel);
    }
};

struct SecEdgeFinish {
    SecEdgeArgs a; const unsigned char *mode; const SecPick *picks;
    const float *d_image; int nd, radiance_dim;
    SecondaryEdgeRec *recs; VSlice ev; double *edge_tmin;
    RDR_FN void make_lean() { lean_scene(a.sc); lean_slice(a.v); lean_slice(ev); nd = 3; radiance_dim = 0; }
    RDR_FN void make_mid() { mid_scene(a.sc); nd = 3; radiance_dim = 0; }
    RDR_FN void operator()(int idx) const {
        if (mode[idx] == 0) return;
        SecPick pkd = picks[idx];
        int eid = pkd.eid;
        double ew = pkd.ew;
        if (eid == -1 || ew <= 0) return;
        int p = a.active[idx];
        int l0 = 2 * idx, l1 = 2 * idx + 1;
        const SceneD &sc = a.sc;
        const EdgeSceneD &es = a.es;
        SecPre s = sec_prepare(sc, es, a.rng_main, a.dim_main, a.rng_edge, a.dim_edge, a.v, p, idx);
        const VertexCtx &c = s.c;
        const LtcCtx &lc = s.lc;
        V3 sample_p = pkd.sample_p, mwt = pkd.mwt;
        if (!s.use_nee) {
            const EdgeD &e = es.edges[eid];
            if (!edge_is_silhouette(sc.shapes, lc.pos, e)) return;
            V3 ea = edge_v0(sc.shapes, e), eb = edge_v1(sc.shapes, e);
            V3 ao = m3_apply(lc.m_inv, ea - lc.pos), bo = m3_apply(lc.m_inv, eb - lc.pos);
            if (ao.z <= 0.f && bo.z <= 0.f) return;
            LineSetup ls = line_setup(ao, bo);
            double Il0 = line_I(ls, ls.l0), Il1 = line_I(ls, ls.l1);
            double norm = Il1 - Il0;
            double lb = ls.l0, ub = ls.l1;
            if (lb > ub) { double tt = lb; lb = ub; ub = tt; }
            double l = 0.5f * (lb + ub);
            for (int it = 0; it < 20; ++it) {
                if (!(l >= lb && l <= ub)) l = 0.5f * (lb + ub);
                double value = (line_I(ls, l) - Il0) / norm - s.t_sel;
                if (fabs(value) < 1e-5f || it == 19) break;
                if (value > 0.f) ub = l; else lb = l;
                double dsq = ls.d * ls.d + l * l;
                double deriv = 2.f * ls.d * (ls.vo + l * ls.wt).z / (norm * dsq * dsq);
                l -= value / deriv;
            }
            double dsq = ls.d * ls.d + l * l;
            double lpdf = 2.f * ls.d * (ls.vo + l * ls.wt).z / (norm * dsq * dsq);
            if (lpdf <= 0.f) return;
            sample_p = m3_apply(lc.m, ls.vo + l * ls.wt);
            ew /= (s.m_pmf * lpdf);
            mwt = m3_apply(lc.m, ls.wt);
        }
        const EdgeD &e = es.edges[eid];
        V3 ea = edge_v0(sc.shapes, e), eb = edge_v1(sc.shapes, e);
        V3 hn = normalize(cross(ea - lc.pos, eb - lc.pos));
        double off = 1e-5f / len(sample_p);
        V3 sdir = normalize(sample_p);
        V3 up = normalize(sdir + off * hn), lo = normalize(sdir - off * hn);
        V3 wi = c.wi;
        V3 f = bsdf_eval(*c.mat, c.sp, wi, sdir, c.mrough);
        if (sum(f) < 1e-6f) return;
        V3 dc = image_grad(d_image, nd, radiance_dim, p);
        SecondaryEdgeRec rec = recs[idx];
        rec.edge = e; rec.edge_pt = sample_p; rec.mwt = mwt;
        rec.use_nee_ray = s.use_nee ? 1 : 0; rec.diffuse_or_glossy = s.dg ? 1 : 0;
        recs[idx] = rec;
        store_ray(ev, l0, lc.pos, up);
        store_ray(ev, l1, lc.pos, lo);
        edge_tmin[l0] = edge_tmin[l1] = 1e-3f * len(sample_p);
        RayDiff brd;
        brd.org_dx = c.rd_surf.org_dx; brd.org_dy = c.rd_surf.org_dy;
        if (s.bsdf_comp <= s.pd) {
            brd.dir_dx = V3{0.03f, 0.03f, 0.03f};
            brd.dir_dy = V3{0.03f, 0.03f, 0.03f};
        } else {
            V3 h = normalize(wi + sdir);
            double hz = dot(h, c.sp.frame.n);
            V3 dmdx = c.sp.dn_dx * hz, dmdy = c.sp.dn_dy * hz;
            V3 ddx = c.rd_surf.dir_dx, ddy = c.rd_surf.dir_dy;
            V3 ddn_dx = ddx * h - wi * dmdx, ddn_dy = ddy * h - wi * dmdy;
            brd.dir_dx = ddx - 2 * (-dot(wi, h) * c.sp.dn_dx + ddn_dx * h);
            brd.dir_dy = ddy - 2 * (-dot(wi, h) * c.sp.dn_dy + ddn_dy * h);
        }
        store_rdiff(ev, l0, brd); store_rdiff(ev, l1, brd);
        if (ev.erd) { st_erd(ev, l0, brd); st_erd(ev, l1, brd); }
        V3 nt = ld3(a.v.thr, a.v.n, p, 0) * f * dc * ew / s.nee_pmf;
        st3(ev.thr, ev.n, l0, 0, nt);
        st3(ev.thr, ev.n, l1, 0, -nt);
    }
};

RDR_FN V3 isect_jacobian(V3 org, V3 dir, V3 p, V3 n, V3 l) {
    double dn = dot(dir, n);
    if (fabs(dn) < 1e-10f) return v3(0);
    double d = -dot(p, n);
    double t = -(dot(org, n) + d) / dn;
    if (t <= 0) return v3(0);
    return t * (l - dir * (dot(l, n) / dot(dir, n)));
}

struct HitEvent { int p, entry, shape_id, v0, v1, depth; double contrib; V3 sp_pos; };
struct HitPosView {
    double *pos; int n;
    const int *seg; int S, P0;
    unsigned char *written; int *violations;
    HitEvent *events; int *event_count; int event_cap, depth;
    RDR_FN int index(int lane) const {
        if (!seg) return lane;
        const int idx = lane >> 1;
        int s = 0;
        while (s + 1 < S && seg[s + 1] <= idx) ++s;
        return lane + 2 * (s * P0 - seg[s]);
    }
// ... 132 lines not shown
```

### redner_amd/csrc/stages_fwd.h

```cpp
#pragma once
#include "bsdf.h"
#include "bvh.h"
#include "camera.h"
#include "lights.h"
#include "envmap.h"
#include "sobol.h"

namespace rdr {

struct VSlice {
    double *ray;
    double *rdiff;
    int *shape, *tri;
    double *thr;
    double *mrough;
    unsigned char *occl;
    int n;
    double *erd;
    unsigned char *erd_touched;
    const int *erd_seg; int erd_S, erd_P0;
};
RDR_FN void st_rdiff(double *b, int n, int i, const RayDiff &r);
RDR_FN RayDiff ld_rdiff(const double *b, int n, int i);
RDR_FN int erd_index(const VSlice &v, int p) {
// ... 10 lines not shown
    if (v.erd_touched) v.erd_touched[i] = 1;
}

RDR_FN V3 ld3(const double *b, int n, int i, int k) { return V3{b[(size_t)(k) * n + i], b[(size_t)(k + 1) * n + i], b[(size_t)(k + 2) * n + i]}; }
RDR_FN void st3(double *b, int n, int i, int k, V3 v) { b[(size_t)(k) * n + i] = v.x; b[(size_t)(k + 1) * n + i] = v.y; b[(size_t)(k + 2) * n + i] = v.z; }

RDR_FN Ray load_ray(const VSlice &v, int i) { return make_ray(ld3(v.ray, v.n, i, 0), ld3(v.ray, v.n, i, 3)); }
RDR_FN void store_ray(const VSlice &v, int i, V3 o, V3 d) { st3(v.ray, v.n, i, 0, o); st3(v.ray, v.n, i, 3, d); }
RDR_FN RayDiff load_rdiff(const VSlice &v, int i) {
    if (!v.rdiff) return raydiff_zero();
    return RayDiff{ld3(v.rdiff, v.n, i, 0), ld3(v.rdiff, v.n, i, 3), ld3(v.rdiff, v.n, i, 6), ld3(v.rdiff, v.n, i, 9)};
}
RDR_FN void st_rdiff(double *b, int n, int i, const RayDiff &r) {
    st3(b, n, i, 0, r.org_dx); st3(b, n, i, 3, r.org_dy);
    st3(b, n, i, 6, r.dir_dx); st3(b, n, i, 9, r.dir_dy);
}
RDR_FN RayDiff ld_rdiff(const double *b, int n, int i) {
    return RayDiff{ld3(b, n, i, 0), ld3(b, n, i, 3), ld3(b, n, i, 6), ld3(b, n, i, 9)};
}
RDR_FN void store_rdiff(const VSlice &v, int i, const RayDiff &r) { if (v.rdiff) st_rdiff(v.rdiff, v.n, i, r); }

RDR_FN rt::RayRec ray_rec(const Ray &r, bool dead) {
    rt::RayRec rec;
    rec.ox = (float)r.org.x; rec.oy = (float)r.org.y; rec.oz = (float)r.org.z; rec.tmin = (float)r.tmin;
    rec.dx = (float)r.dir.x; rec.dy = (float)r.dir.y; rec.dz = (float)r.dir.z;
    rec.tmax = dead ? -1.f : (float)r.tmax;
    return rec;
}
RDR_FN void put_ray(rt::RayRec *q, int slot, const Ray &r, bool dead) { q[slot] = ray_rec(r, dead); }

constexpr int kMaxChannels = 16;

struct ChannelsD { int n; const int *id; int radiance_only; int nd, radiance_dim, radiance_off, max_generic; };

struct Sink {
    float *image;
    double *edge_contrib;
    int nd, radiance_dim;
    double weight;
    ChannelsD ch;
    const double *multipliers;
};

RDR_FN void lean_scene(SceneD &sc) { sc.envmap = nullptr; sc.cam.kind = kCamPerspective; sc.cam.distortion.defined = 0; sc.no_diffs = 1; sc.plain_materials = 1; }
RDR_FN void lean_slice(VSlice &v) { v.rdiff = nullptr; v.erd = nullptr; v.erd_touched = nullptr; v.erd_seg = nullptr; }
RDR_FN void mid_scene(SceneD &sc) { sc.envmap = nullptr; sc.cam.kind = kCamPerspective; sc.cam.distortion.defined = 0; }
RDR_FN void lean_channels(ChannelsD &ch) { ch.n = 1; ch.radiance_only = 1; ch.radiance_dim = 0; ch.radiance_off = 0; ch.nd = 3; }
template <class Stage, class = void> struct LeanBlocks { static constexpr int value = 1; };
template <class Stage> struct LeanBlocks<Stage, decltype((void)Stage::kLeanBlocksPerCU)> { static constexpr int value = Stage::kLeanBlocksPerCU; };
template <class Stage> struct LeanStage {
    static constexpr int kMinBlocksPerCU = LeanBlocks<Stage>::value;
    Stage f;
    RDR_FN void operator()(int i) const { Stage g = f; g.make_lean(); RDR_INLINE_CALL g(i); }
};
template <class Stage, class = void> struct MidBlocks { static constexpr int value = 1; };
template <class Stage> struct MidBlocks<Stage, decltype((void)Stage::kMidBlocksPerCU)> { static constexpr int value = Stage::kMidBlocksPerCU; };
template <class Stage> struct MidStage {
    static constexpr int kMinBlocksPerCU = MidBlocks<Stage>::value;
    Stage f;
    RDR_FN void operator()(int i) const { Stage g = f; g.make_mid(); RDR_INLINE_CALL g(i); }
};
template <class Walk> struct LeanWalk {
    Walk w;
    using State = typename Walk::State;
    RDR_DEV_FN bool begin(int i, State &st) const { Walk g = w; g.make_lean(); return g.begin(i, st); }
    RDR_DEV_FN bool step(State &st) const { Walk g = w; g.make_lean(); return g.step(st); }
    RDR_DEV_FN void finish(State &st) const { Walk g = w; g.make_lean(); g.finish(st); }
    RDR_DEV_FN bool gate_closed() const { return w.gate_closed(); }
};
template <class Walk> struct MidWalk {
    Walk w;
    using State = typename Walk::State;
    RDR_DEV_FN bool begin(int i, State &st) const { Walk g = w; g.make_mid(); return g.begin(i, st); }
    RDR_DEV_FN bool step(State &st) const { Walk g = w; g.make_mid(); return g.step(st); }
    RDR_DEV_FN void finish(State &st) const { Walk g = w; g.make_mid(); g.finish(st); }
    RDR_DEV_FN bool gate_closed() const { return w.gate_closed(); }
};

constexpr int kMaxParkDoubles = 22;

struct LightDraw { double light_sel, tri_sel; V2 uv; };
RDR_FN LightDraw draw_light(const SamplerD &rng, const SamplerD::Lane &ln, int dim) {
    return LightDraw{rng.draw(ln, dim), rng.draw(ln, dim + 1), v2(rng.draw(ln, dim + 2), rng.draw(ln, dim + 3))};
}
RDR_FN LightDraw draw_light(const SamplerD &rng, int slot, int dim) { return draw_light(rng, rng.lane(slot), dim); }

struct GenPrimary {
    SceneD sc; SamplerD rng; int sample_center;
    VSlice v0; rt::RayRec *q;
    RDR_FN void make_lean() { lean_scene(sc); lean_slice(v0); }
    RDR_FN void make_mid() { mid_scene(sc); }
    RDR_FN void operator()(int p) const {
        V2 s = v2(0.5, 0.5);
        if (!sample_center) { const SamplerD::Lane ln = rng.lane(p); s = v2(rng.draw(ln, 0), rng.draw(ln, 1)); }
        RayDiff rd = raydiff_zero();
        Ray r = sc.no_diffs ? primary_ray(sc.cam, pixel_to_screen(sc.cam, p, s))
                            : primary_ray_with_diff(sc.cam, pixel_to_screen(sc.cam, p, s), rd);
        store_ray(v0, p, r.org, r.dir);
        store_rdiff(v0, p, rd);
        st3(v0.thr, v0.n, p, 0, v3(1));
        v0.mrough[p] = 0;
        put_ray(q, p, r, false);
    }
};

RDR_FN V3 direct_emission(const SceneD &sc, int shape, int tri, const Ray &ray, const RayDiff &rd) {
// ... 97 lines not shown
        } else if (shape >= 0) {
            double val[3];
            int nv = channel_value(sc, id, sc.shapes[shape], sp, ray, shape, tri, val);
            bool is_id = id >= 13;
            if (sink.image) {
                float *px = sink.image + (size_t)sink.nd * p + d;
                for (int j = 0; j < nv; ++j) {
                    if (is_id) { px[j] = float(val[j]); continue; }
                    double x = val[j] * sink.weight;
                    if (sink.multipliers) x *= sink.multipliers[(size_t)sink.nd * p + d + j];
                    px[j] += float(x);
                }
            }
            if (sink.edge_contrib && sink.multipliers && !is_id) {
                if (id == 5) { val[0] = sp.frame.n.x; val[1] = sp.frame.n.y; val[2] = sp.frame.n.z; }
                double acc = 0;
                for (int j = 0; j < nv; ++j) acc += (val[j] * sink.weight) * sink.multipliers[(size_t)sink.nd * p + d + j];
                sink.edge_contrib[p] += acc;
            }
        }
        d += width;
    }
}

struct ShadePrimary {
    SceneD sc; const int *active; VSlice v; const rt::HitRec *hits; Sink sink;
    RDR_FN void make_lean() { lean_scene(sc); lean_slice(v); lean_channels(sink.ch); sink.multipliers = nullptr; }
    RDR_FN void make_mid() { mid_scene(sc); lean_channels(sink.ch); sink.multipliers = nullptr; }
    RDR_FN void operator()(int idx) const {
        int p = active ? active[idx] : idx;
        rt::HitRec h = hits[idx];
        v.shape[p] = h.shape; v.tri[p] = h.shape >= 0 ? h.prim : -1;
        shade_first_hit(sc, sink, v, p, h.shape, h.shape >= 0 ? h.prim : -1);
    }
};

struct VertexCtx {
    Ray ray; RayDiff rd_in, rd_surf; Surf sp; V3 wi; double mrough;
    const ShapeD *shape; const MaterialD *mat;
};
RDR_FN VertexCtx load_vertex(const SceneD &sc, const VSlice &v, int p) {
    VertexCtx c;
    c.ray = load_ray(v, p);
    c.rd_in = load_rdiff(v, p);
    c.shape = &sc.shapes[v.shape[p]];
    c.mat = &sc.materials[c.shape->material_id];
    c.sp = surf_at(*c.shape, v.tri[p], c.ray, c.rd_in, c.rd_surf, !sc.no_diffs);
    c.sp.plain = sc.plain_materials;
    c.wi = -c.ray.dir;
    c.mrough = v.mrough[p];
    return c;
}

RDR_FN bool ray_meets_emitter_triangle(const SceneD &sc, const rt::RayRec &r) {
    const float o[3] = {r.ox, r.oy, r.oz}, d[3] = {r.dx, r.dy, r.dz};
    for (int l = 0; l < sc.num_area_lights; ++l) {
        const ShapeD &sh = sc.shapes[sc.lights[l].shape_id];
        for (int t = 0; t < sh.num_triangles; ++t) {
            float a[3], b[3], c[3];
            if (sh.geom) {
                const TriGeomD g = load_dev(sh.geom + t);
                for (int k = 0; k < 3; ++k) { a[k] = g.p[k]; b[k] = g.p[3 + k]; c[k] = g.p[6 + k]; }
            } else {
                const int i0 = sh.indices[3 * t], i1 = sh.indices[3 * t + 1], i2 = sh.indices[3 * t + 2];
                for (int k = 0; k < 3; ++k) { a[k] = sh.vertices[3 * i0 + k]; b[k] = sh.vertices[3 * i1 + k]; c[k] = sh.vertices[3 * i2 + k]; }
            }
            float tt;
            if (rt::ray_triangle(o, d, r.tmin, r.tmax, a, b, c, &tt)) return true;
        }
    }
    return false;
}

struct BounceSample {
    static constexpr int kMidBlocksPerCU = 3;
    static constexpr int kMinBlocksPerCU = 3;
    SceneD sc; SamplerD rng; int dim, rng_shift;
    RDR_FN void make_lean() { lean_scene(sc); lean_slice(v); lean_slice(vn); }
    RDR_FN void make_mid() { mid_scene(sc); }
    const int *active; VSlice v, vn;
    rt::RayRec *q_nee, *q_bsdf;
    int last_bounce_emitters = 0;
    RDR_FN void operator()(int idx) const {
        int p = active[idx];
        VertexCtx c = load_vertex(sc, v, p);
        RDR_INLINE_CALL sample_from(c, p, idx);
    }
    RDR_FN void sample_from(const VertexCtx &c, int p, int idx) const {
        int slot = p >> rng_shift;
        const SamplerD::Lane ln = rng.lane(slot);
        LightDraw ld = draw_light(rng, ln, dim);
        LightPick pk = pick_light(sc, ld.light_sel, ld.tri_sel);
        if (pk.shape_id >= 0) {
            const ShapeD &lsh = sc.shapes[pk.shape_id];
            Surf lp = sample_tri(lsh, pk.tri_id, ld.uv);
            bool moot = false;
            {
                V3 dir = lp.position - c.sp.position;
                double d2 = len_sq(dir);
                if (d2 > 1e-20f && lsh.light_id >= 0) {
                    V3 wo = dir / sqrt(d2);
                    const LightD &l = sc.lights[lsh.light_id];
                    if (!(l.two_sided || dot(-wo, lp.frame.n) > 0)) moot = true;
                    ShadeCtx sx = shade_ctx(*c.mat, c.sp);
                    double gwi = dot(sx.gn, c.wi), gwo = dot(sx.gn, wo);
                    double swi = fabs(dot(sx.fr.n, c.wi)), swo = fabs(dot(sx.fr.n, wo));
                    if (gwi * gwo < 0) moot = true;
                    if (!c.mat->two_sided && gwi < 0 && gwo < 0) moot = true;
                    if (swi == 0 || swo <= 1e-3f || fabs(gwo) <= 1e-3f) moot = true;
                }
            }
            put_ray(q_nee, idx, shadow_ray_to(c.sp.position, lp.position), moot);
        } else if (sc.envmap != nullptr) {
            Ray er = make_ray(c.sp.position, envmap_sample(*sc.envmap, ld.uv));
            put_ray(q_nee, idx, er, false);
        } else {
            Ray dead = make_ray(c.sp.position, v3(0));
            put_ray(q_nee, idx, dead, true);
        }
        V2 buv = v2(rng.draw(ln, dim + 4), rng.draw(ln, dim + 5));
        double bw = rng.draw(ln, dim + 6);
        RayDiff wo_rd = vn.erd ? ld_erd(vn, p) : raydiff_zero();
        double next_mr;
        V3 dir = bsdf_sample_dir(*c.mat, c.sp, c.wi, buv, bw, c.mrough, c.rd_surf, wo_rd, next_mr, !sc.no_diffs);
        store_ray(vn, p, c.sp.position, dir);
        store_rdiff(vn, p, wo_rd);
        if (vn.erd) st_erd(vn, p, wo_rd);
        vn.mrough[p] = next_mr;
        Ray nr = make_ray(c.sp.position, dir);
        bool dead = len_sq(dir) <= 1e-3f;
        if (last_bounce_emitters && !dead) dead = !ray_meets_emitter_triangle(sc, ray_rec(nr, false));
        put_ray(q_bsdf, idx, nr, dead);
    }
};

RDR_FN V3 eval_bounce_nee(const SceneD &sc, const VertexCtx &c, bool nee_visible, const LightPick &pk, const Surf &lp, V2 light_uv) {
    V3 nee = v3(0);
    V3 pos = c.sp.position;
    if (nee_visible && pk.shape_id >= 0) {
        const ShapeD &lsh = sc.shapes[pk.shape_id];
        V3 dir = lp.position - pos;
        double d2 = len_sq(dir);
        V3 wo = dir / sqrt(d2);
        if (d2 > 1e-20f && lsh.light_id >= 0) {
            const LightD &l = sc.lights[lsh.light_id];
            if (l.two_sided || dot(-wo, lp.frame.n) > 0) {
                V3 f = bsdf_eval(*c.mat, c.sp, c.wi, wo, c.mrough);
                double g = fabs(dot(wo, lp.geom_normal)) / d2;
                double pdf_nee = sc.light_pmf[lsh.light_id] / sc.light_areas[lsh.light_id];
                double pdf_b = bsdf_pdf(*c.mat, c.sp, c.wi, wo, c.mrough) * g;
                double mis = 1 / (1 + sq(pdf_b / pdf_nee));
                nee = (mis * g / pdf_nee) * f * v3f(l.intensity);
            }
        }
    } else if (nee_visible && sc.envmap != nullptr) {
        V3 wo = envmap_sample(*sc.envmap, light_uv);
        double pdf_nee = envmap_pdf(*sc.envmap, wo) * sc.light_pmf[sc.num_lights - 1];
        if (pdf_nee > 0) {
            V3 f = bsdf_eval(*c.mat, c.sp, c.wi, wo, c.mrough);
            V3 Le = envmap_eval(*sc.envmap, wo, raydiff_zero());
            double pdf_b = bsdf_pdf(*c.mat, c.sp, c.wi, wo, c.mrough);
            double mis = 1 / (1 + sq(pdf_b / pdf_nee));
            nee = (mis / pdf_nee) * f * Le;
        }
    }
    return nee;
}
struct ScatterEval { V3 scatter, thr_factor; bool next_thr_valid, carries; };
RDR_FN ScatterEval eval_bounce_scatter(const SceneD &sc, const VertexCtx &c, int bshape, const Surf &bp, V3 bsdf_dir) {
    ScatterEval r;
    r.scatter = r.thr_factor = v3(0);
    r.next_thr_valid = r.carries = false;
    V3 pos = c.sp.position;
    if (bshape >= 0) {
        const ShapeD &bsh = sc.shapes[bshape];
        V3 dir = bp.position - pos;
        double d2 = len_sq(dir);
        V3 wo = dir / sqrt(d2);
        double pdf_b = bsdf_pdf(*c.mat, c.sp, c.wi, wo, c.mrough);
        r.next_thr_valid = true;
        if (d2 > 1e-20f && pdf_b > 1e-20f) {
            V3 f = bsdf_eval(*c.mat, c.sp, c.wi, wo, c.mrough);
            if (bsh.light_id >= 0) {
                const LightD &l = sc.lights[bsh.light_id];
                if (l.two_sided || dot(-wo, bp.frame.n) > 0) {
                    double inv_area = 1 / sc.light_areas[bsh.light_id];
                    double g = fabs(dot(wo, bp.geom_normal)) / d2;
                    double pdf_nee = (sc.light_pmf[bsh.light_id] * inv_area) / g;
                    double mis = 1 / (1 + sq(pdf_nee / pdf_b));
                    r.scatter = (mis / pdf_b) * f * v3f(l.intensity);
                }
            }
            r.thr_factor = f / pdf_b;
            r.carries = true;
        }
    } else if (sc.envmap != nullptr) {
        V3 wo = bsdf_dir;
        double pdf_b = bsdf_pdf(*c.mat, c.sp, c.wi, wo, c.mrough);
        if (len_sq(wo) > 0 && pdf_b > 1e-20f) {
            V3 f = bsdf_eval(*c.mat, c.sp, c.wi, wo, c.mrough);
            V3 Le = envmap_eval(*sc.envmap, wo, raydiff_zero());
            double pdf_nee = envmap_pdf(*sc.envmap, wo) * sc.light_pmf[sc.num_lights - 1];
            double mis = 1 / (1 + sq(pdf_nee / pdf_b));
            r.scatter = (mis / pdf_b) * f * Le;
        }
    }
    return r;
}
RDR_FN bool nee_is_geometrically_zero(const SceneD &sc, const VertexCtx &c, const LightPick &pk, const Surf &lp) {
    if (pk.shape_id < 0) return sc.envmap == nullptr;
    const ShapeD &lsh = sc.shapes[pk.shape_id];
    if (lsh.light_id < 0) return true;
    const V3 dir = lp.position - c.sp.position;
    const double d2 = len_sq(dir);
    const V3 wo = dir / sqrt(d2);
    const LightD &l = sc.lights[lsh.light_id];
    if (!(l.two_sided || dot(-wo, lp.frame.n) > 0)) return true;
    const ShadeCtx sx = shade_ctx(*c.mat, c.sp);
    const double gwi = dot(sx.gn, c.wi), gwo = dot(sx.gn, wo);
    const double swi = fabs(dot(sx.fr.n, c.wi)), swo = fabs(dot(sx.fr.n, wo));
    if (gwi * gwo < 0) return true;
    if (!c.mat->two_sided && gwi < 0 && gwo < 0) return true;
    if (swi == 0 || swo <= 1e-3f || fabs(gwo) <= 1e-3f) return true;
    return false;
}

struct BounceContrib {
    static constexpr int kMidBlocksPerCU = 3;
    static constexpr int kMinBlocksPerCU = 3;
#ifndef RDR_PARK_BOUNCE_CONTRIB
#define RDR_PARK_BOUNCE_CONTRIB 1
#endif
#if RDR_PARK_BOUNCE_CONTRIB
#ifndef RDR_BOUNCE_CONTRIB_LEAN_BLOCKS
#ifdef RDR_PLATFORM_LIBM
#define RDR_BOUNCE_CONTRIB_LEAN_BLOCKS 4
#else
#define RDR_BOUNCE_CONTRIB_LEAN_BLOCKS 3
#endif
#endif
    static constexpr int kLeanBlocksPerCU = RDR_BOUNCE_CONTRIB_LEAN_BLOCKS;
#endif
    static constexpr int kParkDoubles = 12;
    static_assert(kParkDoubles <= kMaxParkDoubles, "kMaxParkDoubles must cover every stage");
    SceneD sc; SamplerD rng; int dim, rng_shift;
    const int *active; VSlice v, vn;
    const rt::HitRec *h_nee, *h_bsdf;
    Sink sink;
    RDR_FN void make_lean() { lean_scene(sc); lean_slice(v); lean_slice(vn); lean_channels(sink.ch); }
    RDR_FN void make_mid() { mid_scene(sc); lean_channels(sink.ch); }
    RDR_FN void operator()(int idx) const {
        VertexCtx next;
        RDR_INLINE_CALL contrib(active[idx], idx, next);
    }
    RDR_FN bool contrib(int p, int idx, VertexCtx &next) const {
        int slot = p >> rng_shift;
        const rt::HitRec hn = h_nee[idx], hb = h_bsdf[idx];
        const V3 thr = ld3(v.thr, v.n, p, 0);
        VertexCtx c = load_vertex(sc, v, p);
        LightDraw ld = draw_light(rng, slot, dim);
        LightPick pk = pick_light(sc, ld.light_sel, ld.tri_sel);
        Surf lp = surf_zero();
        if (pk.shape_id >= 0) lp = sample_tri(sc.shapes[pk.shape_id], pk.tri_id, ld.uv);
        bool blocked = hn.shape >= 0;
        if (v.occl) v.occl[p] = (blocked || nee_is_geometrically_zero(sc, c, pk, lp)) ? 1 : 0;
        vn.shape[p] = hb.shape; vn.tri[p] = hb.shape >= 0 ? hb.prim : -1;
        Surf bp = surf_zero();
        if (hb.shape >= 0) {
            RayDiff tmp;
            next.ray = load_ray(vn, p);
            next.rd_in = load_rdiff(vn, p);
            bp = surf_at(sc.shapes[hb.shape], hb.prim, next.ray, next.rd_in, tmp, !sc.no_diffs);
            if (vn.erd) st_erd(vn, p, tmp);
            next.rd_surf = tmp;
            next.shape = &sc.shapes[hb.shape];
            next.mat = &sc.materials[next.shape->material_id];
            next.sp = bp; next.sp.plain = sc.plain_materials;
            next.wi = -next.ray.dir;
            next.mrough = vn.mrough[p];
        }
        const bool consumed = sink.image != nullptr || sink.edge_contrib != nullptr;
#if RDR_PARK_BOUNCE_CONTRIB
        RDR_PARK_DECL(park, kParkDoubles);
        park.put3(0, thr); park.put3(3, bp.position); park.put3(6, bp.frame.n); park.put3(9, bp.geom_normal);
        V3 nee = eval_bounce_nee(sc, c, !blocked && consumed, pk, lp, ld.uv);
        bp.position = park.get3<V3>(3); bp.frame.n = park.get3<V3>(6); bp.geom_normal = park.get3<V3>(9);
        park.put3(3, nee);
        const ScatterEval e = eval_bounce_scatter(sc, c, hb.shape, bp, load_ray(vn, p).dir);
        const V3 thr_in = park.get3<V3>(0);
        nee = park.get3<V3>(3);
#else
        const V3 nee = eval_bounce_nee(sc, c, !blocked && consumed, pk, lp, ld.uv);
        const ScatterEval e = eval_bounce_scatter(sc, c, hb.shape, bp, load_ray(vn, p).dir);
        const V3 thr_in = thr;
#endif
        if (e.next_thr_valid) st3(vn.thr, vn.n, p, 0, e.carries ? thr_in * e.thr_factor : v3(0));
        V3 pc = thr_in * (nee + e.scatter);
        if (sink.image) {
            float *px = sink.image + (size_t)sink.nd * p + sink.radiance_dim;
            px[0] += float(sink.weight * pc.x); px[1] += float(sink.weight * pc.y); px[2] += float(sink.weight * pc.z);
        }
        if (sink.edge_contrib) sink.edge_contrib[p] += sum(sink.weight * pc);
        return hb.shape >= 0;
    }
};

struct BounceContribSample {
    static constexpr int kMidBlocksPerCU = 3;
    static constexpr int kMinBlocksPerCU = 3;
    BounceContrib c; BounceSample s;
    const int *qpos;
    int contrib_only = 0;
    RDR_FN void make_lean() { c.make_lean(); s.make_lean(); }
    RDR_FN void make_mid() { c.make_mid(); s.make_mid(); }
    RDR_FN void operator()(int idx) const {
        const int p = c.active[idx];
        VertexCtx next;
        bool hit;
        RDR_INLINE_CALL hit = c.contrib(p, qpos ? qpos[idx] : idx, next);
        if (contrib_only) return;
        if (hit) { RDR_INLINE_CALL s.sample_from(next, p, idx); }
        else {
            Ray dead = make_ray(v3(0), v3(0));
            put_ray(s.q_nee, idx, dead, true);
            put_ray(s.q_bsdf, idx, dead, true);
        }
    }
};

struct KeepHit {
    const int *shape;
    RDR_FN bool operator()(int p) const { return shape[p] >= 0; }
};
struct KeepNonZeroDir {
    const double *ray; int n;
    RDR_FN bool operator()(int p) const { return !all_zero(ld3(ray, n, p, 3)); }
};

}
```

### redner_amd/csrc/tuning.h

```cpp
#pragma once
#include "../../include/redner_amd.h"
#include <atomic>
#include <cstdio>
#include <cstdlib>

namespace rdr {

struct Tuning {
    unsigned flags = 0;
    int batch_samples = 16;
    long long batch_lanes = 0;
    int workers = 0;
    int refill_k = 4, refill_idle = 24, refill_steps = 4;
    int wide_max = 1 << 19;
    int gather_budget = 256;
    int gather_heavy_cap = -1, gather_work_cap = -1;
    double mem_available_mb = -1.0;
    int refill_sort = 1;
    int pickh_k = 1, pickh_idle = 8, pickh_steps = 8;
    int stale_event_cap = -1;
    bool trace_hybrid = true;
    bool has(unsigned f) const { return (flags & f) != 0; }
};

namespace detail {
inline const char *env(const char *name) { return std::getenv(name); }
inline bool env_set(const char *name) { return std::getenv(name) != nullptr; }
struct EnvDefaults {
    unsigned flags = 0;
    int batch_samples = 0; long long batch_lanes = 0; int workers = 0;
    int refill_k = 0, refill_idle = 0, refill_steps = 0, wide_max = 0, gather_budget = 0, heavy_cap = -1, work_cap = -1;
    double mem_mb = -1.0;
    int refill_order = 0, pickh_k = 0, pickh_idle = 0, pickh_steps = 0;
    bool trace_hybrid = true;
    EnvDefaults() {
        if (env_set("RDR_NO_OVERLAP") || env_set("RDR_DEBUG_DUMP")) flags |= RDR_TUNE_NO_OVERLAP;
        if (env_set("RDR_FORCE_GENERAL")) flags |= RDR_TUNE_FORCE_GENERAL;
        if (env_set("RDR_PICKN_WALK")) flags |= RDR_TUNE_PICKN_WALK;
        if (env_set("RDR_PICKH_FUSED")) flags |= RDR_TUNE_PICKH_FUSED;
        if (env_set("RDR_PICKH_LAZY")) flags |= RDR_TUNE_PICKH_LAZY;
        if (env_set("RDR_NO_HOIST")) flags |= RDR_TUNE_NO_HOIST;
        if (env_set("RDR_TRACE_REFILL_ALL")) flags |= RDR_TUNE_REFILL_ALL;
        if (env_set("RDR_TRACE_BINARY")) flags |= RDR_TUNE_TRACE_BINARY;
        if (env_set("RDR_TRACE_NO_LDS_TOP")) flags |= RDR_TUNE_TRACE_NO_LDS_TOP;
        if (env_set("RDR_NO_FUSED_BOUNCE")) flags |= RDR_TUNE_NO_FUSED_BOUNCE;
        if (env_set("RDR_PICKH_ONE_LAUNCH")) flags |= RDR_TUNE_PICKH_ONE_LAUNCH;
        if (env_set("RDR_NO_NEE_COMPACT")) flags |= RDR_TUNE_NO_NEE_COMPACT;
        if (env_set("RDR_LARGE_FRAME_FORMS")) flags |= RDR_TUNE_LARGE_FORMS;
        if (env_set("RDR_TRACE_EVERY_CONTINUATION")) flags |= RDR_TUNE_TRACE_EVERY_CONTINUATION;
        if (const char *e = env("RDR_TRACE_REFILL")) {
            int k = 0, idle = 0, steps = 0;
            const int got = std::sscanf(e, "%d,%d,%d", &k, &idle, &steps);
            if (got >= 1 && k <= 0) flags |= RDR_TUNE_REFILL_OFF;
            if (got >= 1 && k > 0) refill_k = k;
            if (got >= 2 && idle > 0) refill_idle = idle;
            if (got >= 3 && steps > 0) refill_steps = steps;
        }
        if (const char *e = env("RDR_BATCH")) batch_samples = std::atoi(e);
        if (const char *e = env("RDR_BATCH_LANES")) batch_lanes = std::atoll(e);
        if (const char *e = env("RDR_WORKERS")) workers = std::atoi(e);
        if (const char *e = env("RDR_WIDE_MAX")) wide_max = std::atoi(e);
        if (const char *e = env("RDR_GATHER_BUDGET")) gather_budget = std::atoi(e);
        if (const char *e = env("RDR_GATHER_CAPS")) { int h = 0, w = 0; if (std::sscanf(e, "%d,%d", &h, &w) == 2) { heavy_cap = h; work_cap = w; } }
        if (const char *e = env("RDR_MEM_AVAILABLE_MB")) mem_mb = std::atof(e);
        if (const char *e = env("RDR_REFILL_SORT")) refill_order = std::atoi(e) + 1;
        if (const char *e = env("RDR_TRACE_HYBRID")) trace_hybrid = e[0] != '0';
        if (const char *e = env("RDR_PICKH_REFILL")) {
            int k = 0, idle = 0, steps = 0;
            const int got = std::sscanf(e, "%d,%d,%d", &k, &idle, &steps);
            if (got >= 1 && k > 0) pickh_k = k;
            if (got >= 2 && idle > 0) pickh_idle = idle;
            if (got >= 3 && steps > 0) pickh_steps = steps;
        }
    }
};
inline const EnvDefaults &env_defaults() { static const EnvDefaults d; return d; }
inline int clampi(long long v, long long lo, long long hi) { return (int)(v < lo ? lo : (v > hi ? hi : v)); }
}

inline Tuning resolve_tuning(const rdr_tuning *t) {
    const detail::EnvDefaults &e = detail::env_defaults();
    static const rdr_tuning zero{};
    const rdr_tuning &u = t ? *t : zero;
    Tuning r;
    r.flags = u.flags | e.flags;
    auto pick = [](long long field, long long env, long long dflt) { return field != 0 ? field : (env != 0 ? env : dflt); };
    r.batch_samples = detail::clampi(pick(u.batch_samples, e.batch_samples, 16), 1, 16);
    r.batch_lanes = pick(u.batch_lanes, e.batch_lanes, 0);
    if (r.batch_lanes < 0) r.batch_lanes = 1;
    r.workers = detail::clampi(pick(u.workers, e.workers, 0), 0, 4);
    r.refill_k = detail::clampi(pick(u.refill_rays_per_lane, e.refill_k, 4), 1, 64);
    r.refill_idle = detail::clampi(pick(u.refill_idle_lanes, e.refill_idle, 24), 1, 64);
    r.refill_steps = detail::clampi(pick(u.refill_steps, e.refill_steps, 4), 1, 1024);
    r.wide_max = (int)pick(u.wide_max_rays, e.wide_max, 1 << 19);
    r.gather_budget = detail::clampi(pick(u.gather_budget, e.gather_budget, 256), 1, 1 << 20);
    r.gather_heavy_cap = u.gather_heavy_cap_plus1 > 0 ? u.gather_heavy_cap_plus1 - 1 : e.heavy_cap;
    r.gather_work_cap = u.gather_work_cap_plus1 > 0 ? u.gather_work_cap_plus1 - 1 : e.work_cap;
    r.mem_available_mb = u.mem_available_mb > 0 ? (double)u.mem_available_mb : e.mem_mb;
    r.refill_sort = detail::clampi(pick(u.refill_order, e.refill_order, 2), 1, 3) - 1;
    r.pickh_k = detail::clampi(pick(u.pickh_slots_per_lane, e.pickh_k, 1), 1, 64);
    r.pickh_idle = detail::clampi(pick(u.pickh_idle_lanes, e.pickh_idle, 8), 1, 64);
    r.pickh_steps = detail::clampi(pick(u.pickh_steps, e.pickh_steps, 8), 1, 1024);
// ... 29 lines not shown
```

Before: 86.62 Msamples/s.

## Resolve constant materials into an LDS table in a per-block kernel prologue

Adds a per-block prologue that loads each material's constant diffuse, specular and roughness values and its gradient pointers into a shared-memory table. The bounce kernels are then templated to read from this table instead of chasing material and texture pointers through global memory. The path is used only when every material is constant-textured, has no vertex colors and fits in 64 entries, and it can be turned off with a flag. In exchange it adds a __syncthreads and a 4KB LDS footprint per block, which may lower occupancy.

Measured after the change: 89.34 Msamples/s, median of 6. 3.1% higher.

```diff
diff --git a/include/redner_amd.h b/include/redner_amd.h
--- a/include/redner_amd.h
+++ b/include/redner_amd.h
@@ -114,7 +114,8 @@
     RDR_TUNE_PICKH_ONE_LAUNCH = 1 << 11,
     RDR_TUNE_NO_NEE_COMPACT   = 1 << 12,
     RDR_TUNE_LARGE_FORMS      = 1 << 13,
-    RDR_TUNE_TRACE_EVERY_CONTINUATION = 1 << 14
+    RDR_TUNE_TRACE_EVERY_CONTINUATION = 1 << 14,
+    RDR_TUNE_MATERIAL_FROM_MEMORY = 1 << 15
 };
 struct rdr_tuning {
     unsigned flags;
diff --git a/redner_amd/_capi.py b/redner_amd/_capi.py
--- a/redner_amd/_capi.py
+++ b/redner_amd/_capi.py
@@ -87,7 +87,8 @@
 
 TUNE_NO_OVERLAP, TUNE_FORCE_GENERAL, TUNE_PICKN_WALK, TUNE_PICKH_FUSED, TUNE_PICKH_LAZY, TUNE_NO_HOIST, TUNE_REFILL_OFF, \
     TUNE_REFILL_ALL, TUNE_TRACE_BINARY, TUNE_TRACE_NO_LDS_TOP, TUNE_NO_FUSED_BOUNCE, TUNE_PICKH_ONE_LAUNCH, TUNE_NO_NEE_COMPACT, \
-    TUNE_LARGE_FORMS, TUNE_TRACE_EVERY_CONTINUATION = [1 << k for k in range(15)]
+    TUNE_LARGE_FORMS, TUNE_TRACE_EVERY_CONTINUATION, TUNE_MATERIAL_FROM_MEMORY = [1 << k for k in range(16)]
+MATERIAL_TABLE_CAPACITY = 64
 BUILD_NO_REFIT, BUILD_NO_EDGE_CACHE, BUILD_SYNC_EDGES, BUILD_EDGE_HOST_BUILD = [1 << k for k in range(4)]
 
 
diff --git a/redner_amd/csrc/bsdf.h b/redner_amd/csrc/bsdf.h
--- a/redner_amd/csrc/bsdf.h
+++ b/redner_amd/csrc/bsdf.h
@@ -1,5 +1,6 @@
 #pragma once
 #include "surface.h"
+#include "material_table.h"
 
 namespace rdr {
 
@@ -444,4 +445,235 @@
     return d;
 }
 
-}
+RDR_FN const MaterialRec &mat_rec(const TableMat &m) { return material_table()[m.id]; }
+RDR_FN bool mat_two_sided(const TableMat &m) { return (mat_rec(m).flags & kMatTwoSided) != 0; }
+RDR_FN bool mat_specular_lighting(const TableMat &m) { return (mat_rec(m).flags & kMatSpecularLighting) != 0; }
+RDR_FN bool mat_vertex_color(const TableMat &) { return false; }
+RDR_FN V3 mat_diffuse(const TableMat &m, const Surf &) { const MaterialRec &r = mat_rec(m); return V3{(double)r.diffuse[0], (double)r.diffuse[1], (double)r.diffuse[2]}; }
+RDR_FN V3 mat_specular(const TableMat &m, const Surf &) { const MaterialRec &r = mat_rec(m); return V3{(double)r.specular[0], (double)r.specular[1], (double)r.specular[2]}; }
+RDR_FN double mat_roughness(const TableMat &m, const Surf &) { return mat_rec(m).roughness; }
+RDR_FN void adj_mat_diffuse(const TableMat &m, const Surf &, V3 o_bar, const GMaterial &, Surf &) { double *g = mat_rec(m).g_diffuse; if (g) accum3(g, o_bar); }
+RDR_FN void adj_mat_specular(const TableMat &m, const Surf &, V3 o_bar, const GMaterial &, Surf &) { double *g = mat_rec(m).g_specular; if (g) accum3(g, o_bar); }
+RDR_FN void adj_mat_roughness(const TableMat &m, const Surf &, double o_bar, const GMaterial &, Surf &) { double *g = mat_rec(m).g_roughness; if (g) accum(g, o_bar); }
+RDR_FN bool has_normal_map(const TableMat &) { return false; }
+RDR_FN Frame perturbed_frame(const TableMat &, const Surf &sp) { return sp.frame; }
+RDR_FN void adj_perturbed_normal(const TableMat &, const Surf &, V3 n_bar, const GMaterial &, Surf &sp_bar) { sp_bar.frame.n += n_bar; }
+
+RDR_FN ShadeCtx shade_ctx(const TableMat &m, const Surf &sp) {
+    ShadeCtx c;
+    c.fr = sp.frame;
+    if (!sp.plain && has_normal_map(m)) c.fr = perturbed_frame(m, sp);
+    c.gn = sp.geom_normal;
+    if (dot(c.gn, c.fr.n) < 0) c.gn = -c.gn;
+    return c;
+}
+
+RDR_FN V3 bsdf_eval(const TableMat &m, const Surf &sp, V3 wi, V3 wo, double min_rough) {
+    RDR_CONTRACT_FAST
+    ShadeCtx c = shade_ctx(m, sp);
+    double gwi = dot(c.gn, wi), gwo = dot(c.gn, wo);
+    double swi = fabs(dot(c.fr.n, wi)), swo = fabs(dot(c.fr.n, wo));
+    if (gwi * gwo < 0) return v3(0);
+    if (!mat_two_sided(m) && gwi < 0 && gwo < 0) return v3(0);
+    if (swi == 0 || swo <= 1e-3f || fabs(gwo) <= 1e-3f) return v3(0);
+    V3 kd = vmax0(mat_vertex_color(m) ? sp.color : mat_diffuse(m, sp));
+    V3 ks = vmax0(mat_vertex_color(m) ? v3(0) : mat_specular(m, sp));
+    double rough = dmax(mat_roughness(m, sp), min_rough);
+    V3 diffuse = kd * swo / double(M_PI);
+    V3 spec = v3(0);
+    if (mat_specular_lighting(m) && !mat_vertex_color(m)) {
+        V3 h = normalize(wi + wo);
+        V3 hl = to_local(c.fr, h);
+        if (mat_two_sided(m) && hl.z < 0) hl = -hl;
+        if (hl.z > 0.f) {
+            double e = roughness_to_phong(rough);
+            double D = pow(dmax(hl.z, 0.0), e) * (e + 2.f) / double(2 * M_PI);
+            double G = smith_g1(wi, c.fr.n, rough) * smith_g1(wo, c.fr.n, rough);
+            double cd = fabs(dot(h, wo));
+            V3 F = ks + (1.f - ks) * pow(dmax(1.0 - cd, 0.0), 5.0);
+            spec = F * D * G / (4.f * swi);
+        }
+    }
+    return diffuse + spec;
+}
+
+RDR_FN void adj_bsdf_eval(const TableMat &m, const Surf &sp, V3 wi, V3 wo, double min_rough, V3 f_bar,
+                          const GMaterial &gm, Surf &sp_bar, V3 &wi_bar, V3 &wo_bar) {
+    RDR_CONTRACT_FAST
+    ShadeCtx c = shade_ctx(m, sp);
+    V3 n = c.fr.n;
+    V3 n_bar = v3(0);
+    double gwi = dot(c.gn, wi), gwo = dot(c.gn, wo);
+    double swi = fabs(dot(n, wi)), swo = fabs(dot(n, wo));
+    if (gwi * gwo < 0) return;
+    if (!mat_two_sided(m) && gwi < 0 && gwo < 0) return;
+    if (swi == 0 || swo <= 1e-3f || fabs(gwo) <= 1e-3f) return;
+
+    V3 kd_raw = mat_vertex_color(m) ? sp.color : mat_diffuse(m, sp);
+    V3 kd = vmax0(kd_raw);
+    V3 kd_bar = f_bar * (swo / double(M_PI));
+    if (mat_vertex_color(m)) sp_bar.color += kd_bar;
+    else adj_mat_diffuse(m, sp, kd_bar, gm, sp_bar);
+    double swo_bar = sum(f_bar * kd) / double(M_PI);
+    if (dot(n, wo) < 0) swo_bar = -swo_bar;
+    wo_bar += n * swo_bar;
+    n_bar += wo * swo_bar;
+
+    V3 ks = vmax0(mat_vertex_color(m) ? v3(0) : mat_specular(m, sp));
+    double rough = dmax(mat_roughness(m, sp), min_rough);
+    rough = dmax(rough, 1e-6);
+    if (mat_specular_lighting(m) && !mat_vertex_color(m)) {
+        V3 h = normalize(wi + wo);
+        V3 hl = to_local(c.fr, h);
+        bool hflip = false;
+        if (mat_two_sided(m) && hl.z < 0) { hl = -hl; hflip = true; }
+        if (hl.z > 0.f) {
+            double e = roughness_to_phong(rough);
+            double D = pow(hl.z, e) * (e + 2.f) / double(2 * M_PI);
+            double rough_bar = 0;
+            double Gwi = smith_g1(wi, n, rough), Gwo = smith_g1(wo, n, rough);
+            double G = Gwi * Gwo;
+            double cd = dot(h, wo);
+            double c5 = pow(dmax(1.0 - cd, 0.0), 5.0);
+            V3 F = ks + (1.f - ks) * c5;
+            V3 spec = F * D * G / (4.f * swi);
+            V3 F_bar = f_bar * (D * G / (4.f * swi));
+            double D_bar = sum(f_bar * F) * (G / (4.f * swi));
+            double G_bar = sum(f_bar * F) * (D / (4.f * swi));
+            double swi_bar = -sum(f_bar * spec) / swi;
+            wi_bar += swi_bar * n;
+            n_bar += swi_bar * wi;
+            V3 ks_bar = F_bar * (1.f - c5);
+            double c5_bar = sum(F_bar * (1.f - ks));
+            double cd_bar = -5.f * c5_bar * pow(dmax(1.0 - cd, 0.0), 4.0);
+            V3 h_bar = cd_bar * wo;
+            wo_bar += cd_bar * h;
+            double Gwi_bar = G_bar * Gwo, Gwo_bar = G_bar * Gwi;
+            for (int side = 0; side < 2; ++side) {
+                V3 dv = side == 0 ? wi : wo;
+                double g1_bar = side == 0 ? Gwi_bar : Gwo_bar;
+                double ct = dot(dv, n);
+                V3 dv_bar = v3(0);
+                if (!(dot(dv, h) * ct <= 0)) {
+                    double tt = sqrt(dmax(1.f / sq(ct) - 1.f, 0.0));
+                    if (!(tt <= 1e-10f)) {
+                        double alpha = sqrt(rough);
+                        double a = 1.f / (alpha * tt);
+                        if (!(a >= 1.6f)) {
+                            double num = 3.535f * a + 2.181f * sq(a);
+                            double den = 1.f + 2.276f * a + 2.557f * sq(a);
+                            double num_bar = g1_bar / den;
+                            double den_bar = -g1_bar * num / sq(den);
+                            double a_bar = num_bar * (3.535f + 2.181f * 2 * a) + den_bar * (2.276f + 2.557f * 2 * a);
+                            double alpha_bar = -a_bar * a / alpha;
+                            double tt_bar = -a_bar * a / tt;
+                            rough_bar += 0.5f * alpha_bar / alpha;
+                            double tt2_bar = tt_bar * 0.5f / tt;
+                            double ct_bar = -2.f * tt2_bar / (ct * ct * ct);
+                            dv_bar = ct_bar * n;
+                            n_bar += ct_bar * dv;
+                        }
+                    }
+                }
+                if (side == 0) wi_bar += dv_bar; else wo_bar += dv_bar;
+            }
+            double Dpow_bar = D_bar * (e + 2.f) / double(2 * M_PI);
+            double Dfac_bar = D_bar * pow(hl.z, e);
+            double hz_bar = Dpow_bar * pow(dmax(hl.z, 0.0), e - 1) * e;
+            double e_bar = Dpow_bar * pow(dmax(hl.z, 0.0), e) * log(hl.z);
+            e_bar += Dfac_bar / double(2 * M_PI);
+            rough_bar += adj_roughness_to_phong(rough, e_bar);
+            if (hflip) hz_bar = -hz_bar;
+            h_bar += hz_bar * n;
+            n_bar += hz_bar * h;
+            V3 s_bar = adj_normalize(wi + wo, h_bar);
+            wi_bar += s_bar;
+            wo_bar += s_bar;
+            adj_mat_specular(m, sp, ks_bar, gm, sp_bar);
+            if (rough > min_rough) adj_mat_roughness(m, sp, rough_bar, gm, sp_bar);
+        }
+    }
+    if (!sp.plain && has_normal_map(m)) adj_perturbed_normal(m, sp, n_bar, gm, sp_bar);
+    else sp_bar.frame.n += n_bar;
+}
+
+RDR_FN LobePmf lobe_pmf(const TableMat &m, const Surf &sp) {
+    V3 kd = vmax0(mat_vertex_color(m) ? sp.color : mat_diffuse(m, sp));
+    V3 ks = vmax0(mat_vertex_color(m) ? v3(0) : mat_specular(m, sp));
+    double wd = luminance(kd), ws = luminance(ks), wsum = wd + ws;
+    LobePmf p{0.5, 0.5};
+    if (wsum > 0.f) { p.diffuse = wd / wsum; p.specular = ws / wsum; }
+    return p;
+}
+
+RDR_FN double bsdf_pdf(const TableMat &m, const Surf &sp, V3 wi, V3 wo, double min_rough) {
+    RDR_CONTRACT_FAST
+    ShadeCtx c = shade_ctx(m, sp);
+    double gwi = dot(c.gn, wi), gwo = dot(c.gn, wo);
+    double swo = fabs(dot(c.fr.n, wo));
+    if (gwi * gwo < 0) return 0;
+    if (!mat_two_sided(m) && gwi < 0 && gwo < 0) return 0;
+    LobePmf p = lobe_pmf(m, sp);
+    double pd = 0;
+    if (p.diffuse > 0.f) pd = p.diffuse * swo / double(M_PI);
+    double ps = 0;
+    if (p.specular > 0.f) {
+        V3 h = normalize(wi + wo);
+        V3 hl = to_local(sp.frame, h);
+        if (mat_two_sided(m) && hl.z < 0) hl = -hl;
+        if (hl.z > 0.f && fabs(dot(h, wo)) > 0) {
+            double rough = dmax(dmax(mat_roughness(m, sp), min_rough), 1e-6);
+            double e = roughness_to_phong(rough);
+            double D = pow(hl.z, e) * (e + 2.f) / double(2 * M_PI);
+            ps = p.specular * D * hl.z / (4.f * fabs(dot(h, wo)));
+        }
+    }
+    return pd + ps;
+}
+
+RDR_FN V3 bsdf_sample_dir(const TableMat &m, const Surf &sp, V3 wi, V2 s_uv, double s_w, double min_rough,
+                          const RayDiff &wi_rd, RayDiff &wo_rd, double &next_min_rough, bool diffs = true) {
+    next_min_rough = min_rough;
+    ShadeCtx c = shade_ctx(m, sp);
+    double gwi = dot(c.gn, wi);
+    if (!mat_two_sided(m) && gwi < 0) return v3(0);
+    LobePmf p = lobe_pmf(m, sp);
+    if (s_w <= p.diffuse) {
+        next_min_rough = 1.0;
+        V3 ld = cos_hemisphere(s_uv);
+        if (diffs) {
+            wo_rd.org_dx = wi_rd.org_dx; wo_rd.org_dy = wi_rd.org_dy;
+            wo_rd.dir_dx = V3{0.03f, 0.03f, 0.03f};
+            wo_rd.dir_dy = V3{0.03f, 0.03f, 0.03f};
+        }
+        V3 d = to_world(c.fr, ld);
+        if (dot(c.gn, d) * gwi < 0) d = to_world(c.fr, -ld);
+        return d;
+    }
+    double rough = dmax(dmax(mat_roughness(m, sp), min_rough), 1e-6);
+    next_min_rough = dmax(rough, min_rough);
+    double e = roughness_to_phong(rough);
+    double phi = 2.f * double(M_PI) * s_uv.y;
+    double sphi = sin(phi), cphi = cos(phi);
+    double ct = pow(s_uv.x, 1.0 / (e + 2.0));
+    double st = sqrt(dmax(1.f - ct * ct, 0.0));
+    V3 hl = V3{st * cphi, st * sphi, ct};
+    V3 h = to_world(c.fr, hl);
+    V3 d = 2.f * dot(wi, h) * h - wi;
+    if (dot(c.gn, d) * gwi < 0) {
+        hl = -hl;
+        h = to_world(c.fr, hl);
+        d = 2.f * dot(wi, h) * h - wi;
+    }
+    if (!diffs) return d;
+    V3 dmdx = sp.dn_dx * hl.z, dmdy = sp.dn_dy * hl.z;
+    V3 wi_dx = -wi_rd.dir_dx, wi_dy = -wi_rd.dir_dy;
+    double wdm_dx = sum(wi_dx * h) + sum(wi * dmdx);
+    double wdm_dy = sum(wi_dy * h) + sum(wi * dmdy);
+    wo_rd.org_dx = wi_rd.org_dx; wo_rd.org_dy = wi_rd.org_dy;
+    wo_rd.dir_dx = 2 * (dot(wi, h) * dmdx + wdm_dx * h) - wi_dx;
+    wo_rd.dir_dy = 2 * (dot(wi, h) * dmdy + wdm_dy * h) - wi_dy;
+    return d;
+}
+
+}
diff --git a/redner_amd/csrc/hip/exec.h b/redner_amd/csrc/hip/exec.h
--- a/redner_amd/csrc/hip/exec.h
+++ b/redner_amd/csrc/hip/exec.h
@@ -307,10 +307,20 @@
 template <class F, class = void> struct MinBlocks { static constexpr int value = 1; };
 template <class F> struct MinBlocks<F, decltype((void)F::kMinBlocksPerCU)> { static constexpr int value = F::kMinBlocksPerCU; };
 
+template <class F, class = void> struct StagePrologue { __device__ static bool run(const F &, int) { return true; } };
+template <class F> struct StagePrologue<F, decltype((void)&F::prologue)> {
+    __device__ static bool run(const F &f, int n) {
+        if ((int)(blockIdx.x * 256) >= n) return false;
+        f.prologue();
+        return true;
+    }
+};
+
 template <class F>
 __global__ void __launch_bounds__(256, MinBlocks<F>::value) stage_kernel(F f, int n, const int *count) {
     int i = blockIdx.x * 256 + threadIdx.x;
     if (count) { const int c = *count; n = c < n ? c : n; }
+    if (!StagePrologue<F>::run(f, n)) return;
     if (i < n) { RDR_INLINE_CALL f(i); }
 }
 
diff --git a/redner_amd/csrc/material_table.h b/redner_amd/csrc/material_table.h
--- /dev/null
+++ b/redner_amd/csrc/material_table.h
@@ -0,0 +1,66 @@
+#pragma once
+#include "scene_data.h"
+
+namespace rdr {
+
+constexpr int kMaterialTableCap = 64;
+static_assert(kMaterialTableCap == 64, "redner_amd/_capi.py: MATERIAL_TABLE_CAPACITY states the same number (the capacity tests are built around it)");
+
+struct alignas(16) MaterialRec {
+    float diffuse[3], roughness;
+    float specular[3]; int flags;
+    double *g_diffuse, *g_specular, *g_roughness, *g_pad;
+};
+static_assert(sizeof(MaterialRec) == 64, "material record size");
+constexpr int kMatTwoSided = 1, kMatSpecularLighting = 2;
+
+#if defined(__HIP__)
+RDR_FN MaterialRec *material_table() {
+#if defined(__HIP_DEVICE_COMPILE__)
+    __shared__ MaterialRec table[kMaterialTableCap];
+    return table;
+#else
+    return nullptr;
+#endif
+}
+#else
+inline MaterialRec *material_table() { static MaterialRec table[kMaterialTableCap]; return table; }
+#endif
+
+RDR_FN void resolve_material(const SceneD &sc, const GMaterial *gm, int k, MaterialRec &r) {
+    const MaterialD *m = sc.materials + k;
+    const int two_sided = load_dev(&m->two_sided), specular_lighting = load_dev(&m->compute_specular_lighting);
+    const float *kd = load_dev(&m->diffuse.texels[0]), *ks = load_dev(&m->specular.texels[0]), *ro = load_dev(&m->roughness.texels[0]);
+    r.g_diffuse = r.g_specular = r.g_roughness = r.g_pad = nullptr;
+    if (gm) {
+        r.g_diffuse = load_dev(&gm[k].diffuse.texels[0]);
+        r.g_specular = load_dev(&gm[k].specular.texels[0]);
+        r.g_roughness = load_dev(&gm[k].roughness.texels[0]);
+    }
+    const float d0 = load_dev(kd), d1 = load_dev(kd + 1), d2 = load_dev(kd + 2);
+    const float s0 = load_dev(ks), s1 = load_dev(ks + 1), s2 = load_dev(ks + 2);
+    r.roughness = load_dev(ro);
+    r.diffuse[0] = d0; r.diffuse[1] = d1; r.diffuse[2] = d2;
+    r.specular[0] = s0; r.specular[1] = s1; r.specular[2] = s2;
+    r.flags = (two_sided ? kMatTwoSided : 0) | (specular_lighting ? kMatSpecularLighting : 0);
+}
+
+RDR_FN void fill_material_table(const SceneD &sc, const GMaterial *gm) {
+    MaterialRec *table = material_table();
+#if defined(__HIP_DEVICE_COMPILE__)
+    const int k = threadIdx.x;
+    if (k < sc.num_materials) resolve_material(sc, gm, k, table[k]);
+    __syncthreads();
+#elif !defined(__HIP__)
+    for (int k = 0; k < sc.num_materials; ++k) resolve_material(sc, gm, k, table[k]);
+#else
+    (void)table; (void)sc; (void)gm;
+#endif
+}
+
+template <class F, class = void> struct HasPrologue { static constexpr bool value = false; };
+template <class F> struct HasPrologue<F, decltype((void)&F::prologue)> { static constexpr bool value = true; };
+
+struct TableMat { int id; };
+
+}
diff --git a/redner_amd/csrc/render.cpp b/redner_amd/csrc/render.cpp
--- a/redner_amd/csrc/render.cpp
+++ b/redner_amd/csrc/render.cpp
@@ -87,32 +87,53 @@
     return (uint64_t)o.seed + (uint64_t)o.sample_offset * 0x9E3779B97F4A7C15ULL;
 }
 
+bool material_table_ok(const Scene &scene, const Tuning &t) {
+    if (t.has(RDR_TUNE_MATERIAL_FROM_MEMORY) || scene.d.num_materials > kMaterialTableCap) return false;
+    for (const MaterialD &m : scene.materials) {
+        if (m.use_vertex_color) return false;
+        for (const TexD *tex : {&m.diffuse, &m.specular, &m.roughness})
+            if (tex->num_levels <= 0 || tex->texels[0] == nullptr) return false;
+    }
+    return true;
+}
+
 bool scene_is_lean(const Scene &scene, const ChannelsD &ch) {
     const CameraD &c = scene.d.cam;
     return scene.d.envmap == nullptr && c.kind == kCamPerspective && !c.distortion.defined && ch.radiance_only &&
            !scene.has_mipmaps && !scene.has_textures && !scene.has_vertex_colors;
 }
 
-constexpr int kGeneral = 0, kLean = 1, kMid = 2;
+constexpr int kGeneral = 0, kLean = 1, kMid = 2, kLeanTable = 3;
+inline bool is_lean(int kind) { return kind == kLean || kind == kLeanTable; }
 int scene_kind(const Scene &scene, const ChannelsD &ch) {
     if (tuning().has(RDR_TUNE_FORCE_GENERAL)) return kGeneral;
-    if (scene_is_lean(scene, ch)) return kLean;
+    if (scene_is_lean(scene, ch)) return material_table_ok(scene, tuning()) ? kLeanTable : kLean;
     const CameraD &c = scene.d.cam;
     if (scene.d.envmap == nullptr && c.kind == kCamPerspective && !c.distortion.defined && ch.radiance_only) return kMid;
     return kGeneral;
 }
 template <class F, class Go> void with_kind(int kind, const F &f, Go &&go) {
-    if (kind == kLean) go(LeanStage<F>{f});
+    if (is_lean(kind)) {
+        if constexpr (ReadsMaterials<F>::value) { if (kind == kLeanTable) { go(LeanTableStage<F>{f}); return; } }
+        go(LeanStage<F>{f});
+    }
     else if (kind == kMid) go(MidStage<F>{f});
     else go(f);
 }
 template <class W, class Go> void with_walk_kind(int kind, const W &w, Go &&go) {
-    if (kind == kLean) go(LeanWalk<W>{w});
+    if (is_lean(kind)) go(LeanWalk<W>{w});
     else if (kind == kMid) go(MidWalk<W>{w});
     else go(w);
 }
+template <class K> void host_prologue(const K &k) {
+#if defined(RDR_HOSTSIM)
+    if constexpr (HasPrologue<K>::value) k.prologue();
+#else
+    (void)k;
+#endif
+}
 template <class F> void launch_v(int kind, exec::Count n, const F &f) {
-    with_kind(kind, f, [&](const auto &k) { exec::launch(n, k); });
+    with_kind(kind, f, [&](const auto &k) { host_prologue(k); exec::launch(n, k); });
 }
 
 inline int side_index(int k, int lanes) { return lanes >= (1 << 19) ? k + 2 : k; }
@@ -137,7 +158,7 @@
 }
 
 inline bool fuse_bounces(bool pcg, int kind, int chain_lanes) {
-    return !pcg && kind == kLean && chain_lanes <= (1 << 19) && !tuning().has(RDR_TUNE_NO_FUSED_BOUNCE);
+    return !pcg && is_lean(kind) && chain_lanes <= (1 << 19) && !tuning().has(RDR_TUNE_NO_FUSED_BOUNCE);
 }
 constexpr int kEmitterTestMax = 8;
 struct Bounce {
@@ -161,7 +182,7 @@
     const bool drawn = fused && chain->have_rays;
     const exec::Count queue_n = drawn ? chain->queue_n : b.num_active;
     const int *qpos = drawn ? chain->qpos : nullptr;
-    const bool emitter_test = lean == kLean && scene.emitter_triangles > 0 && scene.emitter_triangles <= kEmitterTestMax &&
+    const bool emitter_test = is_lean(lean) && scene.emitter_triangles > 0 && scene.emitter_triangles <= kEmitterTestMax &&
                               !tuning().has(RDR_TUNE_TRACE_EVERY_CONTINUATION);
     if (!drawn) {
         BounceSample bs{sd, b.rng, b.dim, b.rng_shift, b.active, v, vn, q.nee, q.bsdf};
@@ -278,7 +299,7 @@
         adj.n = P; adj.plain = 0;
         adj.thr = arena.get<double>((size_t)3 * P);
         adj.ray_dir = arena.get<double>((size_t)3 * P);
-        adj_point_doubles = lean == kLean ? kAdjPointDoublesLean : kAdjPointDoubles;
+        adj_point_doubles = is_lean(lean) ? kAdjPointDoublesLean : kAdjPointDoubles;
         adj.point = arena.get<double>((size_t)adj_point_doubles * P);
         adj.carries = scene.d.envmap == nullptr ? arena.get<unsigned char>((size_t)P) : nullptr;
         nee_act = arena.get<int>((size_t)P);
@@ -288,8 +309,8 @@
             edge_dyn = arena.get<int>(kMaxBatch);
             hoist_dyn = arena.get<int>(kMaxBatch);
             const int L = 2 * P;
-            ea = make_slice(arena, L, false, lean != kLean);
-            eb = make_slice(arena, L, false, lean != kLean);
+            ea = make_slice(arena, L, false, !is_lean(lean));
+            eb = make_slice(arena, L, false, !is_lean(lean));
             if (scene.has_mipmaps) {
                 ea.erd = eb.erd = arena.get<double>((size_t)12 * L);
                 exec::zero(ea.erd, sizeof(double) * 12 * L);
@@ -696,7 +717,7 @@
     auto bytes_needed = [&](int S_try) {
         const double lanes = (double)S_try * P;
         const int wk = !samples_independent ? 1 : (tune.workers > 0 ? tune.workers : 2);
-        double per_lane = (lean == kLean ? 260.0 * (B + 1) + 660.0 : 400.0 * (B + 1) + 1200.0) * wk;
+        double per_lane = (is_lean(lean) ? 260.0 * (B + 1) + 660.0 : 400.0 * (B + 1) + 1200.0) * wk;
         if (forward_batches) per_lane += 4.0 * nd * (B + 1);
         if (gradient) per_lane += 4.0 * nd;
         return per_lane * lanes;
@@ -768,7 +789,7 @@
     const bool sobol_plain = screen_gradient_image == nullptr && opt.sampler_type == RDR_SAMPLER_SOBOL && !timer.on;
     const bool no_edge_passes = !scene.use_primary_edges && !scene.use_secondary_edges;
     const bool chain = (scene.has_mipmaps || scene.d.envmap != nullptr) && !no_edge_passes;
-    const bool batchable = sobol_plain && (lean == kLean || no_edge_passes || scene.d.envmap == nullptr || envmap_batches);
+    const bool batchable = sobol_plain && (is_lean(lean) || no_edge_passes || scene.d.envmap == nullptr || envmap_batches);
     const bool samples_independent = batchable && d_image != nullptr && image == nullptr;
     const bool forward_batches = sobol_plain && d_image == nullptr && image != nullptr;
     const BatchView batch = choose_batch(opt, tune, P, cam.vp_y1 - cam.vp_y0, lean, lay.nd, samples_independent, forward_batches, d_image != nullptr);
@@ -793,7 +814,7 @@
     struct SampleWorker : Worker { std::unique_ptr<Backward> bwd; };
     auto make_worker = [&](SampleWorker &w) {
         w.vs.resize(B + 1);
-        for (int d = 0; d <= B; ++d) w.vs[d] = make_slice(w.arena, PL, d < B && d_image_lanes != nullptr, lean != kLean);
+        for (int d = 0; d <= B; ++d) w.vs[d] = make_slice(w.arena, PL, d < B && d_image_lanes != nullptr, !is_lean(lean));
         w.active = w.arena.get<int>((size_t)(B + 1) * PL);
         w.q.nee = w.arena.get<rt::RayRec>((size_t)2 * PL); w.q.bsdf = w.arena.get<rt::RayRec>((size_t)2 * PL);
         w.q.h_nee = w.arena.get<rt::HitRec>((size_t)2 * PL); w.q.h_bsdf = w.arena.get<rt::HitRec>((size_t)2 * PL);
diff --git a/redner_amd/csrc/stages_bwd.h b/redner_amd/csrc/stages_bwd.h
--- a/redner_amd/csrc/stages_bwd.h
+++ b/redner_amd/csrc/stages_bwd.h
@@ -66,7 +66,10 @@
     static_assert(kParkDoubles <= kMaxParkDoubles, "kMaxParkDoubles must cover every stage");
     RDR_FN void make_lean() { lean_scene(a.sc); lean_slice(a.v); lean_slice(a.vn); a.nd = 3; a.radiance_dim = 0; a.adj.plain = 1; }
     RDR_FN void make_mid() { mid_scene(a.sc); a.nd = 3; a.radiance_dim = 0; }
-    RDR_FN void operator()(int idx) const {
+    RDR_FN const SceneD &table_scene() const { return a.sc; }
+    RDR_FN const GMaterial *table_grads() const { return a.g.materials; }
+    template <bool kTable> RDR_FN void run(int idx) const { RDR_INLINE_CALL operator()<kTable>(idx); }
+    template <bool kTable = false> RDR_FN void operator()(int idx) const {
         const SceneD &sc = a.sc; const GScene &g = a.g; const VSlice &v = a.v, &vn = a.vn; const AdjState &adj = a.adj;
         int p = a.active[idx];
         VertexCtx c = load_vertex(sc, v, p);
@@ -94,9 +97,9 @@
             V3 dir = bp.position - pos;
             d2 = len_sq(dir);
             wo = dir / sqrt(d2);
-            double pdf_b = bsdf_pdf(*c.mat, c.sp, c.wi, wo, c.mrough);
+            double pdf_b = bsdf_pdf(mat_of<kTable>(sc, c.mat), c.sp, c.wi, wo, c.mrough);
             if (pdf_b > 0) {
-                V3 f = bsdf_eval(*c.mat, c.sp, c.wi, wo, c.mrough);
+                V3 f = bsdf_eval(mat_of<kTable>(sc, c.mat), c.sp, c.wi, wo, c.mrough);
                 V3 sb = f / pdf_b;
                 thr_bar += next_thr_bar * sb;
                 V3 sb_bar = next_thr_bar * thr;
@@ -118,7 +121,7 @@
                 }
                 V3 wi_bar = v3(0);
                 V3 wo_bar = next_dir_bar;
-                adj_bsdf_eval(*c.mat, c.sp, c.wi, wo, c.mrough, f_bar, gm, sp_bar, wi_bar, wo_bar);
+                adj_bsdf_eval(mat_of<kTable>(sc, c.mat), c.sp, c.wi, wo, c.mrough, f_bar, gm, sp_bar, wi_bar, wo_bar);
                 dir_bar = wo_bar / sqrt(d2);
                 double sd_bar = -sum(wo_bar * dir) / d2;
                 double d2_bar = 0.5f * sd_bar / sqrt(d2);
@@ -128,9 +131,9 @@
             }
         } else if (sc.envmap != nullptr) {
             V3 wo_e = load_ray(vn, p).dir;
-            double pdf_b = bsdf_pdf(*c.mat, c.sp, c.wi, wo_e, c.mrough);
+            double pdf_b = bsdf_pdf(mat_of<kTable>(sc, c.mat), c.sp, c.wi, wo_e, c.mrough);
             if (len_sq(wo_e) > 0 && pdf_b > 0) {
-                V3 f = bsdf_eval(*c.mat, c.sp, c.wi, wo_e, c.mrough);
+                V3 f = bsdf_eval(mat_of<kTable>(sc, c.mat), c.sp, c.wi, wo_e, c.mrough);
                 V3 Le = envmap_eval(*sc.envmap, wo_e, raydiff_zero());
                 double pdf_nee = envmap_pdf(*sc.envmap, wo_e) * sc.light_pmf[sc.num_lights - 1];
                 double mis = 1 / (1 + sq(pdf_nee / pdf_b));
@@ -142,7 +145,7 @@
                 V3 wo_bar = v3(0), wi_bar = v3(0);
                 RayDiff rd_bar = raydiff_zero();
                 adj_envmap_eval(*sc.envmap, wo_e, raydiff_zero(), Le_bar, g.envmap, wo_bar, rd_bar);
-                adj_bsdf_eval(*c.mat, c.sp, c.wi, wo_e, c.mrough, f_bar, gm, sp_bar, wi_bar, wo_bar);
+                adj_bsdf_eval(mat_of<kTable>(sc, c.mat), c.sp, c.wi, wo_e, c.mrough, f_bar, gm, sp_bar, wi_bar, wo_bar);
                 in_dir_bar -= wi_bar;
             }
         }
@@ -209,6 +212,8 @@
     AdjBounceArgs a;
     RDR_FN void make_lean() { lean_scene(a.sc); lean_slice(a.v); lean_slice(a.vn); a.nd = 3; a.radiance_dim = 0; a.adj.plain = 1; }
     RDR_FN void make_mid() { mid_scene(a.sc); a.nd = 3; a.radiance_dim = 0; }
+    RDR_FN const SceneD &table_scene() const { return a.sc; }
+    RDR_FN const GMaterial *table_grads() const { return a.g.materials; }
     RDR_FN void envmap_nee(int p, const LightDraw &ld) const {
         const SceneD &sc = a.sc; const GScene &g = a.g; const VSlice &v = a.v;
         V3 wo = envmap_sample(*sc.envmap, ld.uv);
@@ -234,13 +239,14 @@
         adj_bsdf_eval(*c.mat, c.sp, c.wi, wo, c.mrough, f_bar, gm, sp_bar, wi_bar, wo_bar);
         adj_record_add(a.adj, p, thr_bar, -wi_bar, sp_bar);
     }
-    RDR_FN void operator()(int idx) const {
+    RDR_FN void operator()(int idx) const { RDR_INLINE_CALL run<false>(idx); }
+    template <bool kTable> RDR_FN void run(int idx) const {
         V3 lv_bar[3] = {v3(0), v3(0), v3(0)};
         int l_shape = -1, l_tri = -1;
-        RDR_INLINE_CALL light_vertex(idx, lv_bar, l_shape, l_tri);
+        RDR_INLINE_CALL light_vertex<kTable>(idx, lv_bar, l_shape, l_tri);
         scatter_positions_wave(a.sc.shapes, a.g.shapes, l_shape, l_tri, lv_bar);
     }
-    RDR_FN void light_vertex(int idx, V3 (&lv_bar)[3], int &l_shape, int &l_tri) const {
+    template <bool kTable = false> RDR_FN void light_vertex(int idx, V3 (&lv_bar)[3], int &l_shape, int &l_tri) const {
         const SceneD &sc = a.sc; const GScene &g = a.g; const VSlice &v = a.v; const AdjState &adj = a.adj;
         int p = a.active[idx];
         if (v.occl[p]) return;
@@ -259,18 +265,18 @@
         double d2 = len_sq(dir);
         V3 wo = dir / sqrt(d2);
         const LightD &l = sc.lights[lsh.light_id];
-        if (nee_is_geometrically_zero(sc, c, pk, lp)) return;
+        if (nee_is_geometrically_zero<kTable>(sc, c, pk, lp)) return;
         const GMaterial &gm = g.materials[c.shape->material_id];
         V3 thr = ld3(v.thr, v.n, p, 0);
         V3 pc_bar = a.weight * image_grad(a.d_image, a.nd, a.radiance_dim, p);
         V3 thr_bar = v3(0), in_dir_bar = v3(0);
         Surf sp_bar = surf_zero();
-        V3 f = bsdf_eval(*c.mat, c.sp, c.wi, wo, c.mrough);
+        V3 f = bsdf_eval(mat_of<kTable>(sc, c.mat), c.sp, c.wi, wo, c.mrough);
         double cl = dot(wo, lp.geom_normal);
         double geo = fabs(cl) / d2;
         V3 Le = v3f(l.intensity);
         double pdf_nee = sc.light_pmf[lsh.light_id] * (1 / sc.light_areas[lsh.light_id]);
-        double pdf_b = bsdf_pdf(*c.mat, c.sp, c.wi, wo, c.mrough) * geo;
+        double pdf_b = bsdf_pdf(mat_of<kTable>(sc, c.mat), c.sp, c.wi, wo, c.mrough) * geo;
         double mis = 1 / (1 + sq(pdf_b / pdf_nee));
         V3 nee = (mis * geo / pdf_nee) * f * Le;
         V3 nee_bar = pc_bar * thr;
@@ -296,7 +302,7 @@
         park.put3(9, thr_bar); park.put3(12, dir); park.put(15, d2); park.put(16, d2_bar);
         park.put3(17, lp_bar.geom_normal); park.put2(20, ld.uv);
 #endif
-        adj_bsdf_eval(*c.mat, c.sp, c.wi, wo, c.mrough, f_bar, gm, sp_bar, wi_bar, wo_bar);
+        adj_bsdf_eval(mat_of<kTable>(sc, c.mat), c.sp, c.wi, wo, c.mrough, f_bar, gm, sp_bar, wi_bar, wo_bar);
 #if RDR_PARK_ADJ_NEE
         lv_bar[0] = park.get3<V3>(0); lv_bar[1] = park.get3<V3>(3); lv_bar[2] = park.get3<V3>(6);
         thr_bar = park.get3<V3>(9); dir = park.get3<V3>(12); d2 = park.get(15); d2_bar = park.get(16);
@@ -460,7 +466,10 @@
     AdjBounceScatter f; const unsigned char *live;
     RDR_FN void make_lean() { f.make_lean(); }
     RDR_FN void make_mid() { f.make_mid(); }
-    RDR_FN void operator()(int idx) const { if (!live[f.a.active[idx]]) return; RDR_INLINE_CALL f(idx); }
+    RDR_FN const SceneD &table_scene() const { return f.a.sc; }
+    RDR_FN const GMaterial *table_grads() const { return f.a.g.materials; }
+    RDR_FN void operator()(int idx) const { RDR_INLINE_CALL run<false>(idx); }
+    template <bool kTable> RDR_FN void run(int idx) const { if (!live[f.a.active[idx]]) return; RDR_INLINE_CALL f.run<kTable>(idx); }
 };
 struct AdjPrimaryLive {
     static constexpr int kMidBlocksPerCU = AdjPrimary::kMidBlocksPerCU, kMinBlocksPerCU = AdjPrimary::kMinBlocksPerCU;
diff --git a/redner_amd/csrc/stages_edge.h b/redner_amd/csrc/stages_edge.h
--- a/redner_amd/csrc/stages_edge.h
+++ b/redner_amd/csrc/stages_edge.h
@@ -605,7 +605,7 @@
     Ray nee; Surf nee_pt; int nee_shape;
 };
 
-RDR_FN SecPre sec_prepare(const SceneD &sc, const EdgeSceneD &es, const SamplerD &rng_main, int dim_main,
+template <bool kTable = false> RDR_FN SecPre sec_prepare(const SceneD &sc, const EdgeSceneD &es, const SamplerD &rng_main, int dim_main,
                           const SamplerD &rng_edge, int dim_edge, const VSlice &v, int p, int idx) {
     SecPre s;
     s.live = false;
@@ -628,19 +628,19 @@
     s.edge_sel = rng_edge.draw(eln, dim_edge); s.resample_sel = rng_edge.draw(eln, dim_edge + 1);
     s.bsdf_comp = rng_edge.draw(eln, dim_edge + 2); s.t_sel = rng_edge.draw(eln, dim_edge + 3);
     const MaterialD &mat = *s.c.mat;
-    V3 kd = tex3(mat.diffuse, s.c.sp), ks = tex3(mat.specular, s.c.sp);
+    V3 kd = vertex_diffuse<kTable>(sc, mat, s.c.sp), ks = vertex_specular<kTable>(sc, mat, s.c.sp);
     double wd = luminance(kd), ws = luminance(ks), wsum = wd + ws;
     if (wsum <= 0.f) return s;
     s.pd = wd / wsum; s.ps = ws / wsum;
     V3 n = s.c.sp.frame.n;
     V3 wi = s.c.wi;
-    if (mat.two_sided && dot(wi, n) < 0.f) n = -n;
+    if (vertex_two_sided<kTable>(sc, &mat) && dot(wi, n) < 0.f) n = -n;
     V3 fx = normalize(wi - n * dot(wi, n));
     V3 fy = cross(n, fx);
     if (dot(wi, n) > 1 - 1e-6f) onb(n, fx, fy);
     Frame iso{fx, fy, n};
     s.lc.pos = s.c.sp.position;
-    s.roughness = dmax(tex1(mat.roughness, s.c.sp), s.c.mrough);
+    s.roughness = dmax(vertex_roughness<kTable>(sc, mat, s.c.sp), s.c.mrough);
     if (s.bsdf_comp <= s.pd) {
         s.lc.m_inv = m3_from_frame(iso);
         s.lc.m = m3_inverse(s.lc.m_inv);
@@ -694,10 +694,13 @@
     HDescent *hd = nullptr;
     RDR_FN void make_lean() { lean_scene(a.sc); lean_slice(a.v); lean_slice(ev); }
     RDR_FN void make_mid() { mid_scene(a.sc); }
-    RDR_FN void operator()(int idx) const {
+    RDR_FN const SceneD &table_scene() const { return a.sc; }
+    RDR_FN const GMaterial *table_grads() const { return nullptr; }
+    template <bool kTable> RDR_FN void run(int idx) const { RDR_INLINE_CALL operator()<kTable>(idx); }
+    template <bool kTable = false> RDR_FN void operator()(int idx) const {
         int p = a.active[idx];
         int l0 = 2 * idx, l1 = 2 * idx + 1;
-        SecPre s = sec_prepare(a.sc, a.es, a.rng_main, a.dim_main, a.rng_edge, a.dim_edge, a.v, p, idx);
+        SecPre s = sec_prepare<kTable>(a.sc, a.es, a.rng_main, a.dim_main, a.rng_edge, a.dim_edge, a.v, p, idx);
         SecondaryEdgeRec rec;
         rec.edge = EdgeD{-1, 0, 0, 0, 0};
         rec.edge_pt = rec.mwt = v3(0); rec.sp_pos = s.c.sp.position;
@@ -1096,7 +1099,10 @@
     SecondaryEdgeRec *recs; VSlice ev; double *edge_tmin;
     RDR_FN void make_lean() { lean_scene(a.sc); lean_slice(a.v); lean_slice(ev); nd = 3; radiance_dim = 0; }
     RDR_FN void make_mid() { mid_scene(a.sc); nd = 3; radiance_dim = 0; }
-    RDR_FN void operator()(int idx) const {
+    RDR_FN const SceneD &table_scene() const { return a.sc; }
+    RDR_FN const GMaterial *table_grads() const { return nullptr; }
+    template <bool kTable> RDR_FN void run(int idx) const { RDR_INLINE_CALL operator()<kTable>(idx); }
+    template <bool kTable = false> RDR_FN void operator()(int idx) const {
         if (mode[idx] == 0) return;
         SecPick pkd = picks[idx];
         int eid = pkd.eid;
@@ -1106,7 +1112,7 @@
         int l0 = 2 * idx, l1 = 2 * idx + 1;
         const SceneD &sc = a.sc;
         const EdgeSceneD &es = a.es;
-        SecPre s = sec_prepare(sc, es, a.rng_main, a.dim_main, a.rng_edge, a.dim_edge, a.v, p, idx);
+        SecPre s = sec_prepare<kTable>(sc, es, a.rng_main, a.dim_main, a.rng_edge, a.dim_edge, a.v, p, idx);
         const VertexCtx &c = s.c;
         const LtcCtx &lc = s.lc;
         V3 sample_p = pkd.sample_p, mwt = pkd.mwt;
@@ -1145,7 +1151,7 @@
         V3 sdir = normalize(sample_p);
         V3 up = normalize(sdir + off * hn), lo = normalize(sdir - off * hn);
         V3 wi = c.wi;
-        V3 f = bsdf_eval(*c.mat, c.sp, wi, sdir, c.mrough);
+        V3 f = bsdf_eval(mat_of<kTable>(sc, c.mat), c.sp, wi, sdir, c.mrough);
         if (sum(f) < 1e-6f) return;
         V3 dc = image_grad(d_image, nd, radiance_dim, p);
         SecondaryEdgeRec rec = recs[idx];
diff --git a/redner_amd/csrc/stages_fwd.h b/redner_amd/csrc/stages_fwd.h
--- a/redner_amd/csrc/stages_fwd.h
+++ b/redner_amd/csrc/stages_fwd.h
@@ -86,6 +86,14 @@
     static constexpr int kMinBlocksPerCU = LeanBlocks<Stage>::value;
     Stage f;
     RDR_FN void operator()(int i) const { Stage g = f; g.make_lean(); RDR_INLINE_CALL g(i); }
+};
+template <class Stage, class = void> struct ReadsMaterials { static constexpr bool value = false; };
+template <class Stage> struct ReadsMaterials<Stage, decltype((void)&Stage::table_scene)> { static constexpr bool value = true; };
+template <class Stage> struct LeanTableStage {
+    static constexpr int kMinBlocksPerCU = LeanBlocks<Stage>::value;
+    Stage f;
+    RDR_FN void prologue() const { fill_material_table(f.table_scene(), f.table_grads()); }
+    RDR_FN void operator()(int i) const { Stage g = f; g.make_lean(); RDR_INLINE_CALL g.template run<true>(i); }
 };
 template <class Stage, class = void> struct MidBlocks { static constexpr int value = 1; };
 template <class Stage> struct MidBlocks<Stage, decltype((void)Stage::kMidBlocksPerCU)> { static constexpr int value = Stage::kMidBlocksPerCU; };
@@ -289,6 +297,29 @@
     return c;
 }
 
+#define RDR_MAT_FN __attribute__((always_inline)) RDR_FN
+template <bool kTable> RDR_MAT_FN decltype(auto) mat_of(const SceneD &sc, const MaterialD *m) {
+    if constexpr (kTable) return TableMat{(int)(m - sc.materials)};
+    else return (*m);
+}
+template <bool kTable> RDR_MAT_FN bool vertex_two_sided(const SceneD &sc, const MaterialD *m) {
+    if constexpr (kTable) return mat_two_sided(mat_of<true>(sc, m));
+    else return m->two_sided;
+}
+template <bool kTable> RDR_MAT_FN V3 vertex_diffuse(const SceneD &sc, const MaterialD &m, const Surf &sp) {
+    if constexpr (kTable) return mat_diffuse(mat_of<true>(sc, &m), sp);
+    else return tex3(m.diffuse, sp);
+}
+template <bool kTable> RDR_MAT_FN V3 vertex_specular(const SceneD &sc, const MaterialD &m, const Surf &sp) {
+    if constexpr (kTable) return mat_specular(mat_of<true>(sc, &m), sp);
+    else return tex3(m.specular, sp);
+}
+template <bool kTable> RDR_MAT_FN double vertex_roughness(const SceneD &sc, const MaterialD &m, const Surf &sp) {
+    if constexpr (kTable) return mat_roughness(mat_of<true>(sc, &m), sp);
+    else return tex1(m.roughness, sp);
+}
+#undef RDR_MAT_FN
+
 RDR_FN bool ray_meets_emitter_triangle(const SceneD &sc, const rt::RayRec &r) {
     const float o[3] = {r.ox, r.oy, r.oz}, d[3] = {r.dx, r.dy, r.dz};
     for (int l = 0; l < sc.num_area_lights; ++l) {
@@ -315,15 +346,18 @@
     SceneD sc; SamplerD rng; int dim, rng_shift;
     RDR_FN void make_lean() { lean_scene(sc); lean_slice(v); lean_slice(vn); }
     RDR_FN void make_mid() { mid_scene(sc); }
+    RDR_FN const SceneD &table_scene() const { return sc; }
+    RDR_FN const GMaterial *table_grads() const { return nullptr; }
     const int *active; VSlice v, vn;
     rt::RayRec *q_nee, *q_bsdf;
     int last_bounce_emitters = 0;
-    RDR_FN void operator()(int idx) const {
+    RDR_FN void operator()(int idx) const { RDR_INLINE_CALL run<false>(idx); }
+    template <bool kTable> RDR_FN void run(int idx) const {
         int p = active[idx];
         VertexCtx c = load_vertex(sc, v, p);
-        RDR_INLINE_CALL sample_from(c, p, idx);
-    }
-    RDR_FN void sample_from(const VertexCtx &c, int p, int idx) const {
+        RDR_INLINE_CALL sample_from<kTable>(c, p, idx);
+    }
+    template <bool kTable = false> RDR_FN void sample_from(const VertexCtx &c, int p, int idx) const {
         int slot = p >> rng_shift;
         const SamplerD::Lane ln = rng.lane(slot);
         LightDraw ld = draw_light(rng, ln, dim);
@@ -339,11 +373,11 @@
                     V3 wo = dir / sqrt(d2);
                     const LightD &l = sc.lights[lsh.light_id];
                     if (!(l.two_sided || dot(-wo, lp.frame.n) > 0)) moot = true;
-                    ShadeCtx sx = shade_ctx(*c.mat, c.sp);
+                    ShadeCtx sx = shade_ctx(mat_of<kTable>(sc, c.mat), c.sp);
                     double gwi = dot(sx.gn, c.wi), gwo = dot(sx.gn, wo);
                     double swi = fabs(dot(sx.fr.n, c.wi)), swo = fabs(dot(sx.fr.n, wo));
                     if (gwi * gwo < 0) moot = true;
-                    if (!c.mat->two_sided && gwi < 0 && gwo < 0) moot = true;
+                    if (!vertex_two_sided<kTable>(sc, c.mat) && gwi < 0 && gwo < 0) moot = true;
                     if (swi == 0 || swo <= 1e-3f || fabs(gwo) <= 1e-3f) moot = true;
                 }
             }
@@ -359,7 +393,7 @@
         double bw = rng.draw(ln, dim + 6);
         RayDiff wo_rd = vn.erd ? ld_erd(vn, p) : raydiff_zero();
         double next_mr;
-        V3 dir = bsdf_sample_dir(*c.mat, c.sp, c.wi, buv, bw, c.mrough, c.rd_surf, wo_rd, next_mr, !sc.no_diffs);
+        V3 dir = bsdf_sample_dir(mat_of<kTable>(sc, c.mat), c.sp, c.wi, buv, bw, c.mrough, c.rd_surf, wo_rd, next_mr, !sc.no_diffs);
         store_ray(vn, p, c.sp.position, dir);
         store_rdiff(vn, p, wo_rd);
         if (vn.erd) st_erd(vn, p, wo_rd);
@@ -371,7 +405,7 @@
     }
 };
 
-RDR_FN V3 eval_bounce_nee(const SceneD &sc, const VertexCtx &c, bool nee_visible, const LightPick &pk, const Surf &lp, V2 light_uv) {
+template <bool kTable = false> RDR_FN V3 eval_bounce_nee(const SceneD &sc, const VertexCtx &c, bool nee_visible, const LightPick &pk, const Surf &lp, V2 light_uv) {
     V3 nee = v3(0);
     V3 pos = c.sp.position;
     if (nee_visible && pk.shape_id >= 0) {
@@ -382,10 +416,10 @@
         if (d2 > 1e-20f && lsh.light_id >= 0) {
             const LightD &l = sc.lights[lsh.light_id];
             if (l.two_sided || dot(-wo, lp.frame.n) > 0) {
-                V3 f = bsdf_eval(*c.mat, c.sp, c.wi, wo, c.mrough);
+                V3 f = bsdf_eval(mat_of<kTable>(sc, c.mat), c.sp, c.wi, wo, c.mrough);
                 double g = fabs(dot(wo, lp.geom_normal)) / d2;
                 double pdf_nee = sc.light_pmf[lsh.light_id] / sc.light_areas[lsh.light_id];
-                double pdf_b = bsdf_pdf(*c.mat, c.sp, c.wi, wo, c.mrough) * g;
+                double pdf_b = bsdf_pdf(mat_of<kTable>(sc, c.mat), c.sp, c.wi, wo, c.mrough) * g;
                 double mis = 1 / (1 + sq(pdf_b / pdf_nee));
                 nee = (mis * g / pdf_nee) * f * v3f(l.intensity);
             }
@@ -394,9 +428,9 @@
         V3 wo = envmap_sample(*sc.envmap, light_uv);
         double pdf_nee = envmap_pdf(*sc.envmap, wo) * sc.light_pmf[sc.num_lights - 1];
         if (pdf_nee > 0) {
-            V3 f = bsdf_eval(*c.mat, c.sp, c.wi, wo, c.mrough);
+            V3 f = bsdf_eval(mat_of<kTable>(sc, c.mat), c.sp, c.wi, wo, c.mrough);
             V3 Le = envmap_eval(*sc.envmap, wo, raydiff_zero());
-            double pdf_b = bsdf_pdf(*c.mat, c.sp, c.wi, wo, c.mrough);
+            double pdf_b = bsdf_pdf(mat_of<kTable>(sc, c.mat), c.sp, c.wi, wo, c.mrough);
             double mis = 1 / (1 + sq(pdf_b / pdf_nee));
             nee = (mis / pdf_nee) * f * Le;
         }
@@ -404,7 +438,7 @@
     return nee;
 }
 struct ScatterEval { V3 scatter, thr_factor; bool next_thr_valid, carries; };
-RDR_FN ScatterEval eval_bounce_scatter(const SceneD &sc, const VertexCtx &c, int bshape, const Surf &bp, V3 bsdf_dir) {
+template <bool kTable = false> RDR_FN ScatterEval eval_bounce_scatter(const SceneD &sc, const VertexCtx &c, int bshape, const Surf &bp, V3 bsdf_dir) {
     ScatterEval r;
     r.scatter = r.thr_factor = v3(0);
     r.next_thr_valid = r.carries = false;
@@ -414,10 +448,10 @@
         V3 dir = bp.position - pos;
         double d2 = len_sq(dir);
         V3 wo = dir / sqrt(d2);
-        double pdf_b = bsdf_pdf(*c.mat, c.sp, c.wi, wo, c.mrough);
+        double pdf_b = bsdf_pdf(mat_of<kTable>(sc, c.mat), c.sp, c.wi, wo, c.mrough);
         r.next_thr_valid = true;
         if (d2 > 1e-20f && pdf_b > 1e-20f) {
-            V3 f = bsdf_eval(*c.mat, c.sp, c.wi, wo, c.mrough);
+            V3 f = bsdf_eval(mat_of<kTable>(sc, c.mat), c.sp, c.wi, wo, c.mrough);
             if (bsh.light_id >= 0) {
                 const LightD &l = sc.lights[bsh.light_id];
                 if (l.two_sided || dot(-wo, bp.frame.n) > 0) {
@@ -433,9 +467,9 @@
         }
     } else if (sc.envmap != nullptr) {
         V3 wo = bsdf_dir;
-        double pdf_b = bsdf_pdf(*c.mat, c.sp, c.wi, wo, c.mrough);
+        double pdf_b = bsdf_pdf(mat_of<kTable>(sc, c.mat), c.sp, c.wi, wo, c.mrough);
         if (len_sq(wo) > 0 && pdf_b > 1e-20f) {
-            V3 f = bsdf_eval(*c.mat, c.sp, c.wi, wo, c.mrough);
+            V3 f = bsdf_eval(mat_of<kTable>(sc, c.mat), c.sp, c.wi, wo, c.mrough);
             V3 Le = envmap_eval(*sc.envmap, wo, raydiff_zero());
             double pdf_nee = envmap_pdf(*sc.envmap, wo) * sc.light_pmf[sc.num_lights - 1];
             double mis = 1 / (1 + sq(pdf_nee / pdf_b));
@@ -444,7 +478,7 @@
     }
     return r;
 }
-RDR_FN bool nee_is_geometrically_zero(const SceneD &sc, const VertexCtx &c, const LightPick &pk, const Surf &lp) {
+template <bool kTable = false> RDR_FN bool nee_is_geometrically_zero(const SceneD &sc, const VertexCtx &c, const LightPick &pk, const Surf &lp) {
     if (pk.shape_id < 0) return sc.envmap == nullptr;
     const ShapeD &lsh = sc.shapes[pk.shape_id];
     if (lsh.light_id < 0) return true;
@@ -453,11 +487,11 @@
     const V3 wo = dir / sqrt(d2);
     const LightD &l = sc.lights[lsh.light_id];
     if (!(l.two_sided || dot(-wo, lp.frame.n) > 0)) return true;
-    const ShadeCtx sx = shade_ctx(*c.mat, c.sp);
+    const ShadeCtx sx = shade_ctx(mat_of<kTable>(sc, c.mat), c.sp);
     const double gwi = dot(sx.gn, c.wi), gwo = dot(sx.gn, wo);
     const double swi = fabs(dot(sx.fr.n, c.wi)), swo = fabs(dot(sx.fr.n, wo));
     if (gwi * gwo < 0) return true;
-    if (!c.mat->two_sided && gwi < 0 && gwo < 0) return true;
+    if (!vertex_two_sided<kTable>(sc, c.mat) && gwi < 0 && gwo < 0) return true;
     if (swi == 0 || swo <= 1e-3f || fabs(gwo) <= 1e-3f) return true;
     return false;
 }
@@ -486,11 +520,14 @@
     Sink sink;
     RDR_FN void make_lean() { lean_scene(sc); lean_slice(v); lean_slice(vn); lean_channels(sink.ch); }
     RDR_FN void make_mid() { mid_scene(sc); lean_channels(sink.ch); }
-    RDR_FN void operator()(int idx) const {
+    RDR_FN const SceneD &table_scene() const { return sc; }
+    RDR_FN const GMaterial *table_grads() const { return nullptr; }
+    RDR_FN void operator()(int idx) const { RDR_INLINE_CALL run<false>(idx); }
+    template <bool kTable> RDR_FN void run(int idx) const {
         VertexCtx next;
-        RDR_INLINE_CALL contrib(active[idx], idx, next);
-    }
-    RDR_FN bool contrib(int p, int idx, VertexCtx &next) const {
+        RDR_INLINE_CALL contrib<kTable>(active[idx], idx, next);
+    }
+    template <bool kTable = false> RDR_FN bool contrib(int p, int idx, VertexCtx &next) const {
         int slot = p >> rng_shift;
         const rt::HitRec hn = h_nee[idx], hb = h_bsdf[idx];
         const V3 thr = ld3(v.thr, v.n, p, 0);
@@ -500,7 +537,7 @@
         Surf lp = surf_zero();
         if (pk.shape_id >= 0) lp = sample_tri(sc.shapes[pk.shape_id], pk.tri_id, ld.uv);
         bool blocked = hn.shape >= 0;
-        if (v.occl) v.occl[p] = (blocked || nee_is_geometrically_zero(sc, c, pk, lp)) ? 1 : 0;
+        if (v.occl) v.occl[p] = (blocked || nee_is_geometrically_zero<kTable>(sc, c, pk, lp)) ? 1 : 0;
         vn.shape[p] = hb.shape; vn.tri[p] = hb.shape >= 0 ? hb.prim : -1;
         Surf bp = surf_zero();
         if (hb.shape >= 0) {
@@ -520,15 +557,15 @@
 #if RDR_PARK_BOUNCE_CONTRIB
         RDR_PARK_DECL(park, kParkDoubles);
         park.put3(0, thr); park.put3(3, bp.position); park.put3(6, bp.frame.n); park.put3(9, bp.geom_normal);
-        V3 nee = eval_bounce_nee(sc, c, !blocked && consumed, pk, lp, ld.uv);
+        V3 nee = eval_bounce_nee<kTable>(sc, c, !blocked && consumed, pk, lp, ld.uv);
         bp.position = park.get3<V3>(3); bp.frame.n = park.get3<V3>(6); bp.geom_normal = park.get3<V3>(9);
         park.put3(3, nee);
-        const ScatterEval e = eval_bounce_scatter(sc, c, hb.shape, bp, load_ray(vn, p).dir);
+        const ScatterEval e = eval_bounce_scatter<kTable>(sc, c, hb.shape, bp, load_ray(vn, p).dir);
         const V3 thr_in = park.get3<V3>(0);
         nee = park.get3<V3>(3);
 #else
-        const V3 nee = eval_bounce_nee(sc, c, !blocked && consumed, pk, lp, ld.uv);
-        const ScatterEval e = eval_bounce_scatter(sc, c, hb.shape, bp, load_ray(vn, p).dir);
+        const V3 nee = eval_bounce_nee<kTable>(sc, c, !blocked && consumed, pk, lp, ld.uv);
+        const ScatterEval e = eval_bounce_scatter<kTable>(sc, c, hb.shape, bp, load_ray(vn, p).dir);
         const V3 thr_in = thr;
 #endif
         if (e.next_thr_valid) st3(vn.thr, vn.n, p, 0, e.carries ? thr_in * e.thr_factor : v3(0));
@@ -550,13 +587,16 @@
     int contrib_only = 0;
     RDR_FN void make_lean() { c.make_lean(); s.make_lean(); }
     RDR_FN void make_mid() { c.make_mid(); s.make_mid(); }
-    RDR_FN void operator()(int idx) const {
+    RDR_FN const SceneD &table_scene() const { return c.sc; }
+    RDR_FN const GMaterial *table_grads() const { return nullptr; }
+    RDR_FN void operator()(int idx) const { RDR_INLINE_CALL run<false>(idx); }
+    template <bool kTable> RDR_FN void run(int idx) const {
         const int p = c.active[idx];
         VertexCtx next;
         bool hit;
-        RDR_INLINE_CALL hit = c.contrib(p, qpos ? qpos[idx] : idx, next);
+        RDR_INLINE_CALL hit = c.contrib<kTable>(p, qpos ? qpos[idx] : idx, next);
         if (contrib_only) return;
-        if (hit) { RDR_INLINE_CALL s.sample_from(next, p, idx); }
+        if (hit) { RDR_INLINE_CALL s.sample_from<kTable>(next, p, idx); }
         else {
             Ray dead = make_ray(v3(0), v3(0));
             put_ray(s.q_nee, idx, dead, true);
diff --git a/redner_amd/csrc/tuning.h b/redner_amd/csrc/tuning.h
--- a/redner_amd/csrc/tuning.h
+++ b/redner_amd/csrc/tuning.h
@@ -48,6 +48,7 @@
         if (env_set("RDR_NO_NEE_COMPACT")) flags |= RDR_TUNE_NO_NEE_COMPACT;
         if (env_set("RDR_LARGE_FRAME_FORMS")) flags |= RDR_TUNE_LARGE_FORMS;
         if (env_set("RDR_TRACE_EVERY_CONTINUATION")) flags |= RDR_TUNE_TRACE_EVERY_CONTINUATION;
+        if (env_set("RDR_MATERIAL_FROM_MEMORY")) flags |= RDR_TUNE_MATERIAL_FROM_MEMORY;
         if (const char *e = env("RDR_TRACE_REFILL")) {
             int k = 0, idle = 0, steps = 0;
             const int got = std::sscanf(e, "%d,%d,%d", &k, &idle, &steps);
```
